# smdogroup/paropt

Hardware: AMD Instinct MI355X
Metric: IP iterations/sec (KKT solve+line search), n=50M vars m=32, 1/2/4/8 GPUs (higher is better)
Workload: dtype f64

## Files before the change

### paropt_amd/csrc/context.cpp

```cpp
#include <dlfcn.h>
#include <math.h>
#include <stdarg.h>
#include <execinfo.h>
#include <stdio.h>
#include <stdlib.h>
#include <string.h>
#include <time.h>

#include <algorithm>
#include <mutex>
#include <unordered_map>

#include "core.hpp"

namespace po {

static thread_local char g_err[1024] = "";
thread_local int g_last_code = 0;

void set_error(const char *fmt, ...) {
  va_list ap;
  va_start(ap, fmt);
  vsnprintf(g_err, sizeof(g_err), fmt, ap);
  va_end(ap);
  fprintf(stderr, "paropt_amd: %s\n", g_err);
}
const char *last_error() { return g_err; }

double host_now() {
  struct timespec t;
  clock_gettime(CLOCK_MONOTONIC, &t);
  return (double)t.tv_sec + 1e-9 * (double)t.tv_nsec;
}

struct SwitchDef {
  DbgSwitch id;
  const char *env;
  int dflt;
  bool presence;
};
static const SwitchDef kSwitches[] = {
    {SW_PERTURB_W, nullptr, 0, false},
    {SW_MPC_FUSE, "PAROPT_AMD_MPC_FUSE", 1, false},
    {SW_MPC_POLY, "PAROPT_AMD_MPC_POLY", 1, false},
    {SW_SPEC_DT, "PAROPT_AMD_SPEC_DT", 1, false},
    {SW_UNIFORM_BOUNDS, nullptr, 1, false},
    {SW_WGRAM_PRIO, "PAROPT_AMD_WGRAM_PRIO", 2, false},
    {SW_WGRAM_ABLATE, "PAROPT_AMD_WGRAM_ABLATE", 0, false},
    {SW_EXPLICIT_DOTS, "PAROPT_AMD_EXPLICIT_DOTS", 0, true},
    {SW_NO_RECOMPUTE, "PAROPT_AMD_NO_RECOMPUTE", 0, true},
    {SW_NO_RECOMPUTE_RHS, "PAROPT_AMD_NO_RECOMPUTE_RHS", 0, true},
    {SW_NO_FUSED_MERIT, "PAROPT_AMD_NO_FUSED_MERIT", 0, true},
    {SW_NO_LEAN_STEP, "PAROPT_AMD_NO_LEAN_STEP", 0, true},
    {SW_NO_RECOMPUTE_DT, "PAROPT_AMD_NO_RECOMPUTE_DT", 0, true},
    {SW_NO_FUSED_UPDATE, "PAROPT_AMD_NO_FUSED_UPDATE", 0, true},
    {SW_NO_CSR_GROUPS, "PAROPT_AMD_NO_CSR_GROUPS", 0, true},
    {SW_NO_FRONTS, "PAROPT_AMD_NO_FRONTS", 0, false},
    {SW_FORCE_RCCL, "PAROPT_AMD_FORCE_RCCL", 0, true},
    {SW_RCCL_ALLGATHER, "PAROPT_AMD_RCCL_ALLGATHER", 0, true},
    {SW_NO_DIRECT_RED, "PAROPT_AMD_NO_DIRECT_RED", 0, true},
    {SW_NO_FLAG_POLL, "PAROPT_AMD_NO_FLAG_POLL", 0, true},
    {SW_NO_BATCH, "PAROPT_AMD_NO_BATCH", 0, true},
    {SW_HOST_TRACE, "PAROPT_AMD_HOST_TRACE", 0, true},
    {SW_SYNC_TRACE, "PAROPT_AMD_SYNC_TRACE", 0, true},
    {SW_USER_TIMING, "PAROPT_AMD_USER_TIMING", 0, true},
    {SW_DUMP_LONG_SOLVES, "PAROPT_AMD_DUMP_LONG_SOLVES", -1, false},
};
static struct {
  int value = -1;
} g_dbg_switch[SW_COUNT];

int dbg_switch(DbgSwitch id) {
  if (g_dbg_switch[id].value >= 0) return g_dbg_switch[id].value;
  for (const SwitchDef &s : kSwitches) {
    if (s.id != id) continue;
    const char *e = s.env ? getenv(s.env) : nullptr;
    return e ? (s.presence ? 1 : atoi(e)) : s.dflt;
  }
  return 0;
}
void dbg_switch_set(int id, int value) {
  if (id >= 0 && id < SW_COUNT) g_dbg_switch[id].value = value;
}

int launch_reduce_final(Ctx *c, int nblocks, int nslots, int nsum, int nmin, int dst_off);
int launch_reduce_final_multi(Ctx *c, const Ctx::PendingRed *pend, int count);
int launch_red_publish(Ctx *c, const double *src, int count);
static int alloc_h_red(Ctx *c, size_t doubles) {
  if (c->h_red) (void)hipHostFree(c->h_red);
  c->h_red = nullptr;
  c->h_red_dev = nullptr;
  if (hipHostMalloc((void **)&c->h_red, sizeof(double) * doubles, hipHostMallocMapped | hipHostMallocCoherent) !=
      hipSuccess) {
    (void)hipGetLastError();
    c->h_red = nullptr;
    PO_HIP(hipHostMalloc((void **)&c->h_red, sizeof(double) * doubles, hipHostMallocDefault));
    c->h_red_coherent = 0;
  } else {
    c->h_red_coherent = 1;
  }
  if (dbg_switch(SW_NO_DIRECT_RED) ||
      hipHostGetDevicePointer((void **)&c->h_red_dev, c->h_red, 0) != hipSuccess) {
    (void)hipGetLastError();
    c->h_red_dev = nullptr;
  }
  if (c->h_flag && (!c->h_red_coherent || !c->h_red_dev)) {
    (void)hipHostFree(c->h_flag);
    c->h_flag = c->h_flag_dev = nullptr;
    if (c->d_ticket) (void)hipFree(c->d_ticket);
    c->d_ticket = nullptr;
  }
  if (c->h_red_dev && !c->h_flag && c->h_red_coherent && !dbg_switch(SW_NO_FLAG_POLL)) {
    if (hipHostMalloc((void **)&c->h_flag, 64, hipHostMallocMapped | hipHostMallocCoherent) == hipSuccess &&
        hipHostGetDevicePointer((void **)&c->h_flag_dev, c->h_flag, 0) == hipSuccess &&
        hipMalloc((void **)&c->d_ticket, sizeof(unsigned)) == hipSuccess &&
        hipMemset(c->d_ticket, 0, sizeof(unsigned)) == hipSuccess) {
      *c->h_flag = 0;
    } else {
      (void)hipGetLastError();
      if (c->h_flag) (void)hipHostFree(c->h_flag);
      if (c->d_ticket) (void)hipFree(c->d_ticket);
      c->h_flag = c->h_flag_dev = nullptr;
      c->d_ticket = nullptr;
    }
  }
  return PO_OK;
}


static int comm_self_test(Ctx *c);
static void free_overflow(Ctx *c, const double *keep);

struct Id128 {
  char b[PO_RCCL_ID_BYTES];
};
struct RcclApi {
  void *handle = nullptr;
  int (*GetUniqueId)(void *) = nullptr;
  int (*CommInitRank)(void **, int, Id128, int) = nullptr;
  int (*AllGather)(const void *, void *, size_t, int, void *, hipStream_t) = nullptr;
  int (*AllReduce)(const void *, void *, size_t, int, int, void *, hipStream_t) = nullptr;
  int (*CommDestroy)(void *) = nullptr;
  const char *(*GetErrorString)(int) = nullptr;
  int (*GetVersion)(int *) = nullptr;
  int version = 0;
};
static RcclApi g_rccl;

static int load_rccl() {
// ... 578 lines not shown
```

### paropt_amd/csrc/core.hpp

```cpp
#pragma once
#include <hip/hip_runtime.h>
#include <stdint.h>

#include <functional>
#include <string>
#include <vector>

#include "../../include/paropt_amd.h"

namespace po {

void set_error(const char *fmt, ...);
extern thread_local int g_last_code;

#define PO_HIP(expr)                                                                     \
  do {                                                                                   \
    hipError_t _e = (expr);                                                              \
    if (_e != hipSuccess) {                                                              \
      po::set_error("%s failed: %s (%s:%d)", #expr, hipGetErrorString(_e), __FILE__,     \
                    __LINE__);                                                           \
      return PO_ERR_HIP;                                                                 \
    }                                                                                    \
  } while (0)

// ... 75 lines not shown
};

struct Vec {
  Ctx *ctx;
  int64_t n;
  double *d;
  int ref;
  double *h;
  int h_live = 0;
};

struct PtrTable {
  const double *p[kMaxPanel];
};
struct CoefTable {
  double a[kMaxPanel];
};
int reduce_finish(Ctx *c, int nblocks, int nsum, int nmin, int nmax, double *host_out, bool now = false,
                  double *local_out = nullptr);
bool red_direct(const Ctx *c);
int batch_flush(Ctx *c, const double *keep_partials = nullptr, size_t keep_len = 0);
void batch_abort(Ctx *c);
template <class F>
inline void after_reduce(Ctx *c, F &&f) {
  if (c->batch_depth > 0 && !c->batch_pend.empty()) {
    c->batch_after.emplace_back(std::forward<F>(f));
  } else {
    f();
  }
}
struct BatchScope {
  Ctx *c;
  bool open;
  explicit BatchScope(Ctx *c_, bool on = true) : c(c_), open(on && c_->batch_enabled) {
    if (open) c->batch_depth++;
  }
  void begin() {
    if (!open && c->batch_enabled) {
      open = true;
      c->batch_depth++;
    }
  }
  int end() {
    if (!open) return PO_OK;
    open = false;
    c->batch_depth--;
    return batch_flush(c);
  }
  int end_nested() {
    if (!open) return PO_OK;
    open = false;
    c->batch_depth--;
    return c->batch_depth > 0 ? PO_OK : batch_flush(c);
  }
  template <class F>
  int end_then(F &&post) {
    if (open) {
      open = false;
      c->batch_depth--;
      if (c->batch_depth > 0) {
        after_reduce(c, std::forward<F>(post));
        return PO_OK;
      }
      PO_TRY(batch_flush(c));
    }
    post();
    return PO_OK;
  }
  ~BatchScope() {
    if (open) {
      c->batch_depth--;
      batch_abort(c);
    }
  }
  BatchScope(const BatchScope &) = delete;
  BatchScope &operator=(const BatchScope &) = delete;
};
enum DbgSwitch {
  SW_PERTURB_W = 11, SW_MPC_FUSE = 14, SW_MPC_POLY = 15, SW_SPEC_DT = 16, SW_UNIFORM_BOUNDS = 17,
  SW_WGRAM_PRIO = 18, SW_WGRAM_ABLATE = 19, SW_EXPLICIT_DOTS = 20, SW_NO_RECOMPUTE = 21, SW_NO_RECOMPUTE_RHS = 22,
  SW_NO_FUSED_MERIT = 23, SW_NO_LEAN_STEP = 24, SW_NO_RECOMPUTE_DT = 25, SW_NO_FUSED_UPDATE = 26,
  SW_NO_CSR_GROUPS = 27, SW_NO_FRONTS = 28, SW_FORCE_RCCL = 29, SW_RCCL_ALLGATHER = 30, SW_NO_DIRECT_RED = 31,
  SW_NO_FLAG_POLL = 32, SW_NO_BATCH = 33, SW_HOST_TRACE = 34, SW_SYNC_TRACE = 35, SW_USER_TIMING = 36,
  SW_DUMP_LONG_SOLVES = 37, SW_COUNT = 38
};
int dbg_switch(DbgSwitch id);
void dbg_switch_set(int id, int value);
double host_now();
inline double host_trace_begin(Ctx *c);
inline void host_trace_end(Ctx *c, double t0);
int ensure_partials(Ctx *c, size_t doubles);
bool ctx_alive(const Ctx *c, unsigned long long serial);
inline double host_trace_begin(Ctx *c) {
  if (!c->host_trace) return 0.0;
  const double t = host_now();
  if (!c->host_gap_open && c->host_t_launch_end > 0.0) {
    const double g = t - c->host_t_launch_end;
    if (g < 500e-6) {
      c->host_inter_s += g;
      c->host_inter_n++;
      if (g > 30e-6) {
        c->host_inter_n30++;
        c->host_inter_s30 += g;
      }
    }
  }
  if (c->host_gap_open) {
    const double g = t - c->host_t_sync;
    if (g < 500e-6) {
      c->host_gap_s += g;
      c->host_gap_n++;
      if (g > 20e-6) c->host_gap_n20++;
    } else {
      c->host_gap_long_s += g;
      c->host_gap_long_n++;
    }
    c->host_gap_open = false;
  }
  return t;
}
inline void host_trace_end(Ctx *c, double t0) {
  if (!c->host_trace) return;
  c->host_t_launch_end = host_now();
  c->host_launch_s += c->host_t_launch_end - t0;
  c->host_launch_n++;
}
inline void count_bytes(Ctx *c, double streams, int64_t n) {
  const double b = 8.0 * streams * (double)n;
  c->alg_bytes += b;
  if (c->in_user) c->alg_bytes_user += b;
}
constexpr int kBpcPanel = 2;
constexpr int kBpcStream = 4;
int grid_for(Ctx *c, int64_t n);
int grid_for(Ctx *c, int64_t n, int bpc);

struct GroupCol {
  const double *w = nullptr;
  double scale = 0.0;
  unsigned period = 1, nw = 0;
  long long nwcon = 0;
};

struct GroupCols2 {
  GroupCol g[2];
  double ca[2] = {0.0, 0.0}, cb[2] = {0.0, 0.0};
  int count = 0;
};

int k_fill(Ctx *c, double *y, int64_t n, double alpha);
int k_fill_hash(Ctx *c, double *y, int64_t n, uint64_t seed, uint64_t aid, int64_t offset,
                double scale, double shift);
int k_copy(Ctx *c, double *y, const double *x, int64_t n);
int k_sign(Ctx *c, double *y, const double *x, int64_t n);
int k_scale(Ctx *c, double *y, int64_t n, double alpha);
int k_axpy(Ctx *c, double *y, double alpha, const double *x, int64_t n);
int k_panel_axpy(Ctx *c, double *y, double a, const double *x, double b, const double *alpha,
                 const double *const *V, int nv, int64_t n, const GroupCol *ybase = nullptr);
int k_panel_axpy2(Ctx *c, double *y1, double a1, const double *x1, const double *c1, double *y2, double a2,
                  const double *x2, const double *c2, const double *const *V, int nv, int64_t n);
int k_panel_lincomb(Ctx *c, double *const *dst, double a, const double *const *X, double b,
                    const double *const *Y, int nv, int64_t n);
enum Red1 { RED_DOT = 0, RED_SUMSQ = 1, RED_ASUM = 2, RED_AMAX = 3 };
int k_reduce1(Ctx *c, int kind, const double *x, const double *y, int64_t n, double *out);
int k_mdot(Ctx *c, const double *x, const double *const *V, int nv, int64_t n, double *out);
int k_minmax(Ctx *c, const double *x, int64_t n, double out[2]);
int k_stream_launch(Ctx *c, int kind, double *x, double *y, int64_t n);
int k_mdot_launch(Ctx *c, const double *x, const double *const *V, int nv, int64_t n, int *nblocks);
struct GramGroups {
  int64_t nwcon = 0, start = 0;
  int nw = 0, skip = 0;
  double alpha = 1.0;
  int ncols = 0;
  double *const *U = nullptr;
};
int k_wgram(Ctx *c, const double *d, const double *const *V, int nv, int64_t n, double *W,
            const double *const *S = nullptr, double *const *Zout = nullptr, int kpend = 0,
            double b0 = 0.0, int preweighted_last = 0, bool may_defer = false,
            const GramGroups *groups = nullptr, bool *groups_done = nullptr);
int wgram_debug_stamps(double out[8]);
int k_xgram(Ctx *c, const double *const *U, const double *const *Z, int m, int64_t w, double *out,
            bool may_defer = false);
int k_wgram_launch(Ctx *c, const double *d, const double *const *V, int nv, int64_t n,
                   int *nblocks, int *nslots, const double *const *S = nullptr,
                   double *const *Zout = nullptr, int kpend = 0, double b0 = 0.0,
                   int preweighted_last = 0, const GramGroups *groups = nullptr, bool *groups_done = nullptr);

struct Bounds {
  const double *x, *lb, *ub, *zl, *zu;
  double max_bound;
  int use_lower, use_upper;
  int lb_uni = 0, ub_uni = 0;
  double lb_c = 0.0, ub_c = 0.0;
};
inline int uniform_bound_streams(const Bounds &b) { return (b.lb_uni ? 1 : 0) + (b.ub_uni ? 1 : 0); }
int k_kkt_res(Ctx *c, const Bounds &b, const double *g, const double *const *A, const double *z,
              int nc, double beta_mu, int64_t n, double *rx, double *out, double *yqn = nullptr,
              double beta_mu2 = -1.0, const GroupCol *gcol = nullptr, double gcoef = 0.0);
int k_kkt_res_update(Ctx *c, const Bounds &b, const double *g, const double *const *A, const double *z, int nc,
                     double beta_mu, int64_t n, double *rx, double *out, double *yqn, double *zl,
                     const double *pzl, double *zu, const double *pzu, double a, double eps, const double *va,
                     double az, double *acz, double az_acz,
                     const double *pxs = nullptr, const double *xold = nullptr, double beta_mu_step = 0.0,
                     double beta_mu2 = -1.0,
                     const GroupCol *gcol = nullptr, double gcoef = 0.0,
                     double *dinv_out = nullptr, double *t_out = nullptr, double spec_diag = 0.0,
                     double spec_beta_mu = 0.0);
int k_res_norms(Ctx *c, const Bounds &b, double beta_mu, int64_t n, double out[11]);
int k_dinv(Ctx *c, const Bounds &b, double diag, int64_t n, double *dinv,
           const double *hdiag = nullptr);
int k_d1s(Ctx *c, const Bounds &b, const double *bx, const double *dinv, double alpha, double beta_mu,
          int64_t n, double *t);
int k_solve2s(Ctx *c, const Bounds &b, const double *t, const double *dinv, const double *coef,
              const double *const *P, int nv, double alpha, double beta_mu, int full, double tau, int64_t n,
              double *px, double *pzl, double *pzu, double out[2]);
int k_d1(Ctx *c, const Bounds &b, const double *rx, const double *dinv, double beta_mu, int64_t n,
         double *t, const double *cl = nullptr, const double *cu = nullptr);
int k_dinv_d1(Ctx *c, const Bounds &b, double diag, const double *hdiag, const double *rx, double beta_mu,
              int64_t n, double *dinv, double *t, int raw = 0);
int k_corrector(Ctx *c, const Bounds &b, const double *px, const double *pzl, const double *pzu,
                int64_t n, double *cl, double *cu);
constexpr int kCorrDotsMax = 15;
int k_corr_d1_dots(Ctx *c, const Bounds &b, const double *px, const double *pzl, const double *pzu, const double *rx,
                   const double *dinv, double beta_mu, const double *const *V, int nv, int64_t n, double *t,
                   double *out);
int k_solve2c(Ctx *c, const Bounds &b, const double *t, const double *dinv, const double *alpha,
              const double *const *P, int nv, double beta_mu, double tau, int64_t n, double *px, double *pzl,
              double *pzu, double *va, int nca, const double *g, int want_logs, double out[12]);
int k_solve2(Ctx *c, const Bounds &b, const double *t, const double *dinv, const double *alpha,
             const double *const *P, int nv, double beta_mu, int refine, double tau, int64_t n,
             double *px, double *pzl, double *pzu, double out[2], const double *coef2 = nullptr,
             const double *rx = nullptr, double diag = 0.0, double *tout = nullptr,
             double *va = nullptr, int nca = 0, const double *cl = nullptr,
             const double *cu = nullptr);
int k_solve2_dots(Ctx *c, const Bounds &b, const double *t, const double *dinv, const double *alpha,
                  const double *coef2, const double *const *P, int nv, double beta_mu, double tau,
                  const double *rx, double diag, int64_t n, double *px, double *pzl, double *pzu,
                  double *tout, double *va, int nca, double *out, double *traw = nullptr,
                  int store_step = 1,
                  int ca0 = 0,
                  double dinv_diag = 0.0,
                  const GroupCols2 *gcols = nullptr);
int k_solve2r(Ctx *c, const Bounds &b, const double *t1, const double *t2, const double *dinv, const double *a1,
              const double *a2, const double *const *P, int nv, double beta_mu, double tau, int64_t n, double *px,
              double *pzl, double *pzu, double *va, int nca, double out[2], const double *ar = nullptr,
              const double *rx = nullptr, double diag = 0.0,
              int ca0 = 0,
              const double *g = nullptr, double *merit_out = nullptr,
              double dinv_diag = 0.0,
              const GroupCol *gcol = nullptr, double gc1 = 0.0, double gc2 = 0.0);
int k_form_pz(Ctx *c, const Bounds &b, const double *px, double beta_mu, int64_t n, double *pzl, double *pzu);
int k_update_mult_yqn(Ctx *c, double *zl, const double *pzl, double *zu, const double *pzu, double a,
                      double eps, int use_lower, int use_upper, const double *rx, const double *va,
                      double az, int64_t n, double *yqn, double *acz = nullptr);
int k_res_step(Ctx *c, const Bounds &b, const double *rx, const double *px, const double *pzl,
               const double *pzu, const double *dinv, const double *coef, const double *const *P,
               int nv, double diag, double beta_mu, int64_t n, double *tprime);
int k_step_check(Ctx *c, const Bounds &b, const double *rx, const double *px, const double *pzl, const double *pzu,
                 const double *coef, const double *const *P, int nv, double diag, double beta_mu, int64_t n,
                 double out[3]);
int k_comp_step(Ctx *c, const Bounds &b, const double *px, const double *pzl, const double *pzu,
                double ax, double az, int64_t n, double out[2]);
int k_comp_merit(Ctx *c, const Bounds &b, const double *px, const double *pzl, const double *pzu, double ax,
                 double az, const double *g, int64_t n, double out[9]);
int k_merit0(Ctx *c, const Bounds &b, const double *px, double sx, const double *g, int64_t n,
             double out[6]);
int k_trial(Ctx *c, const Bounds &b, const double *px, double a, double eps, int64_t n, double *xt,
            double out[2], double *sout = nullptr);
int k_update_mult(Ctx *c, double *zl, const double *pzl, double *zu, const double *pzu, double a,
                  double eps, int use_lower, int use_upper, int64_t n);
int k_affine_mult(Ctx *c, const Bounds &b, double *zl, const double *pzl, double *zu,
                  const double *pzu, double amin, int64_t n);
int k_check_bounds(Ctx *c, double *x, double *lb, double *ub, double *zl, double *zu,
                   double max_bound, double rel_bound, int both, int64_t n, int *flag, int uni[2] = nullptr,
                   double val[2] = nullptr);
int k_bounds_mode(Ctx *c, double *x, double *lb, double *ub, int mode, int64_t offset, int64_t n);
int k_clamp_count(Ctx *c, const double *x, const double *lb, const double *ub, const double *zl, const double *zu,
                  double eps, int64_t n, double out[4]);
// ... 24 lines not shown
```

### paropt_amd/csrc/ip.cpp

```cpp
#include "ip.hpp"

#include <math.h>
#include <stdio.h>
#include <stdlib.h>
#include <string.h>

#include <algorithm>
#include <chrono>

namespace po {

static const int LS_SUCCESS = 1, LS_FAILURE = 2, LS_MIN_STEP = 4, LS_MAX_ITERS = 8,
                 LS_NO_IMPROVEMENT = 16, LS_SHORT_STEP = 32;

InteriorPoint::InteriorPoint(Problem *p)
    : prob(p), ctx(p->ctx), n(p->nlocal), c(p->ncon), qn(nullptr), x(nullptr), zl(nullptr),
      zu(nullptr), lb(nullptr), ub(nullptr), g(nullptr), fobj(0.0), barrier_param(0.1),
      rho_penalty_search(0.0), niter(0), neval(0), ngeval(0),
      iter_cb(nullptr),
      iter_cb_user(nullptr), px(nullptr), pzl(nullptr), pzu(nullptr), Dinv(nullptr), rx(nullptr),
      tvec(nullptr), xt(nullptr), y_qn(nullptr), s_qn(nullptr), vA(nullptr), qn_created(false), qn_owned(true),
      comp_prod(0), comp_count(0), max_rx(0), max_rzl(0), max_rzu(0), sx(1.0), sz(1.0),
      corrector_active(false), norm_type(0), phase_t0(0) {
  qn_handle.qn = nullptr;
// ... 247 lines not shown
  (void)hipEventRecord(user_ev[2 * user_pending], ctx->stream);
}
void InteriorPoint::userEnd() {
  ctx->in_user = 0;
  if (!user_timing || !user_events_ready) return;
  (void)hipEventRecord(user_ev[2 * user_pending + 1], ctx->stream);
  user_pending++;
}
void InteriorPoint::userHarvest() {
  for (int i = 0; i < user_pending; i++) {
    float ms = 0.0f;
    if (hipEventSynchronize(user_ev[2 * i + 1]) == hipSuccess &&
        hipEventElapsedTime(&ms, user_ev[2 * i], user_ev[2 * i + 1]) == hipSuccess)
      user_seconds += 1e-3 * ms;
  }
  user_pending = 0;
}

int InteriorPoint::initAndCheckDesignAndBounds() {
  bounds_uni[0] = bounds_uni[1] = 0;
  int rc = prob->getVarsAndBounds(x, lb, ub);
  if (rc != 0) {
    set_error("getVarsAndBounds failed with code %d", rc);
    return PO_ERR_USER;
  }
  const double rel_bound = 0.001 * barrier_param;
  int flag = 0;
  PO_TRY(k_check_bounds(ctx, x->d, lb->d, ub->d, zl->d, zu->d, options.real("max_bound_value"),
                        rel_bound, use_lower && use_upper, n, &flag, bounds_uni, bounds_val));
  check_flag |= flag;
  if (ctx->rank == 0) {
    if (flag & 1) history += "ParOpt Warning: Variable bounds are inconsistent\n";
    if (flag & 2) history += "ParOpt Warning: Variables may be too close to lower bound\n";
    if (flag & 4) history += "ParOpt Warning: Variables may be too close to upper bound\n";
  }
  return PO_OK;
}

int InteriorPoint::clampCounts(double out[8]) {
  const double eps = options.real("design_precision");
  PO_TRY(k_clamp_count(ctx, x->d, lb->d, ub->d, use_lower ? zl->d : nullptr, use_upper ? zu->d : nullptr, eps, n,
                       out));
  for (int j = 4; j < 8; j++) out[j] = 0.0;
  for (int i = 0; i < c; i++) {
    if (vars.s[i] == eps) out[4] += 1.0;
    if (vars.t[i] == eps) out[5] += 1.0;
    if (vars.zs[i] == eps) out[6] += 1.0;
    if (vars.zt[i] == eps) out[7] += 1.0;
  }
  return PO_OK;
}

static int refreshLiveMirror(Vec *v) {
  if (!v || !v->h_live || !v->h || v->n <= 0) return PO_OK;
  PO_HIP(hipMemcpyAsync(v->h, v->d, sizeof(double) * (size_t)v->n, hipMemcpyDeviceToHost, v->ctx->stream));
  PO_HIP(hipStreamSynchronize(v->ctx->stream));
  return PO_OK;
}

int InteriorPoint::resetDesignAndBounds() {
  stateReplaced();
  bounds_uni[0] = bounds_uni[1] = 0;
  int rc = prob->getVarsAndBounds(x, lb, ub);
  if (rc != 0) return PO_ERR_USER;
  PO_TRY(refreshLiveMirror(x));
  PO_TRY(refreshLiveMirror(lb));
  return refreshLiveMirror(ub);
}

void InteriorPoint::resetQuasiNewtonHessian() {
  if (qn) qn->reset();
}

int InteriorPoint::initLeastSquaresMultipliers() {
  iterate_flags.acz_valid = false;
  const double mu0 = options.real("init_barrier_param");
  PO_TRY(k_fill(ctx, zl->d, n, mu0));
  PO_TRY(k_fill(ctx, zu->d, n, mu0));
  for (int i = 0; i < c; i++) vars.z[i] = vars.s[i] = vars.t[i] = vars.zs[i] = vars.zt[i] = mu0;
  PO_TRY(k_zero_inactive(ctx, lb->d, ub->d, zl->d, zu->d, options.real("max_bound_value"), n));
  if (has_w) return initLeastSquaresMultipliersW();
  if (c == 0) return PO_OK;
  const double small = 1e-4;
  PO_TRY(k_fill(ctx, Dinv->d, n, 1.0));
  int k = 0;
  std::vector<const double *> A = panel(false, &k);
  std::vector<double> G((size_t)c * c, 0.0);
  PO_TRY(k_wgram(ctx, Dinv->d, A.data(), c, n, G.data()));
  for (int i = 0; i < c; i++) G[(size_t)i * (c + 1)] += small;
  std::vector<int> piv(c);
  lu_factor(c, G.data(), c, piv.data());
  const double al[2] = {1.0, -1.0};
  const double *vv[2] = {zl->d, zu->d};
  PO_TRY(k_panel_axpy(ctx, tvec->d, -1.0, g->d, 0.0, al, vv, 2, n));
  std::vector<double> z(c, 0.0);
  PO_TRY(k_mdot(ctx, tvec->d, A.data(), c, n, z.data()));
  for (int i = 0; i < c; i++) z[i] = -z[i];
  lu_solve(c, G.data(), c, piv.data(), z.data());
  for (int i = 0; i < c; i++) {
    const double gam = 10.0 * std::max(gamma_s[i], gamma_t[i]);
    vars.z[i] = (z[i] < -gam || z[i] > gam) ? 0.0 : z[i];
  }
  return PO_OK;
}

int InteriorPoint::initAffineStepMultipliers() {
  const double amin = options.real("start_affine_multiplier_min");
  PO_TRY(initLeastSquaresMultipliers());
  PO_TRY(k_zero_inactive(ctx, lb->d, ub->d, zl->d, zu->d, options.real("max_bound_value"), n));
  PO_TRY(computeResidual(0.0, true));
  bool use_qn = !(options.integer("sequential_linear_method") ||
                  !options.integer("use_qn_gmres_precon") || options.integer("use_diag_hessian"));
  if (options.integer("use_diag_hessian")) PO_TRY(ensureHdiag());
  PO_TRY(setUpKKTSystem(use_qn));
  denseResidual(0.0, res);
  if (has_w) {
    PO_TRY(solveKKTW(res, 0.0, use_qn, false, 1.0, step));
    PO_TRY(k_w_affine(ctx, wv(), wp(), amin, nw));
  } else {
    PO_TRY(solveKKT(res, 0.0, use_qn, false, 1.0, step));
  }
  iterate_flags.acz_valid = false;
  for (int i = 0; i < c; i++) {
    vars.z[i] = vars.z[i] + step.z[i];
    vars.s[i] = std::max(amin, fabs(vars.s[i] + step.s[i]));
    vars.t[i] = std::max(amin, fabs(vars.t[i] + step.t[i]));
    vars.zs[i] = std::max(amin, fabs(vars.zs[i] + step.zs[i]));
    vars.zt[i] = std::max(amin, fabs(vars.zt[i] + step.zt[i]));
  }
  PO_TRY(k_affine_mult(ctx, bounds(), zl->d, pzl->d, zu->d, pzu->d, amin, n));
  double comp = 0.0;
  PO_TRY(getComplementarity(&comp));
  barrier_param = comp;
  return PO_OK;
}

void InteriorPoint::denseResidual(double mu, Dense &r) const {
  for (int i = 0; i < c; i++) {
    r.z[i] = -(cvals[i] - vars.s[i] + vars.t[i]);
    r.s[i] = -(gamma_s[i] - vars.zs[i] + vars.z[i]);
    r.t[i] = -(gamma_t[i] - vars.zt[i] - vars.z[i]);
    r.zs[i] = -(vars.s[i] * vars.zs[i] - mu);
    r.zt[i] = -(vars.t[i] * vars.zt[i] - mu);
  }
}

double InteriorPoint::nextMonotoneMu() const {
  const double abs_res_tol = options.real("abs_res_tol");
  const double mu_frac = options.real("monotone_barrier_fraction") * barrier_param;
  const double mu_pow = pow(barrier_param, options.real("monotone_barrier_power"));
  double new_mu = mu_frac;
  if (mu_pow < mu_frac) new_mu = mu_pow;
  if (new_mu < 0.1 * abs_res_tol) new_mu = 0.09999 * abs_res_tol;
  return new_mu;
}

int InteriorPoint::computeResidual(double mu, bool vectors, Vec *yqn_complete, const MultUpdate *upd) {
  const double beta_mu = options.real("rel_bound_barrier") * mu;
  double *out = res_out;
  const bool spec = vectors && spec_enabled && !has_w && mu == barrier_param;
  const double mu2 = spec ? nextMonotoneMu() : 0.0;
  const double beta_mu2 = spec ? options.real("rel_bound_barrier") * mu2 : -1.0;
  iterate_flags.spec_valid = false;
  scratch_flags.spec_dt_valid = false;
  BatchScope wbatch(ctx, has_w && prob->reductionsBatchable());
  if (has_w) PO_TRY(computeResidualW(mu));
  bool acz_mode = false, acz_rebuilt = false;
  if (vectors) {
    std::vector<const double *> A;
    std::vector<double> zc;
    if (prob->linear_constraints && iterate_flags.ac_valid && c > 0) {
      if (!acz) acz = vec_new(ctx, n);
      if (!acz) return PO_ERR_HIP;
      if (!iterate_flags.acz_valid || acz_age >= kAczRefresh) {
        std::vector<const double *> Ap;
        for (Vec *a : Ac) Ap.push_back(a->d);
        PO_TRY(k_panel_axpy(ctx, acz->d, 0.0, nullptr, 0.0, vars.z.data(), Ap.data(), c, n));
        iterate_flags.acz_valid = true;
        acz_age = 0;
        acz_rebuilt = true;
      }
      acz_age++;
      A.push_back(acz->d);
      zc.push_back(1.0);
      acz_mode = true;
    } else {
      for (Vec *a : Ac) A.push_back(a->d);
      zc = vars.z;
    }
    GroupCol gcol;
    const bool have_gcol = has_w && !acz_mode && prob->sparseTransposeColumn(1.0, x, wvar[0], &gcol);
    if (has_w && !have_gcol) {
      if (prob->setSparseJacobianTranspose(1.0, x, wvar[0], tvec) != 0) return PO_ERR_USER;
      A.push_back(tvec->d);
      zc.push_back(1.0);
    }
    if (upd) {
      const double az_acz = (acz_mode && upd->acz_follow && !acz_rebuilt) ? upd->az : 0.0;
      const bool spec_dt = spec_dt_want && !has_w && !options.integer("use_diag_hessian") &&
                           dbg_switch(SW_SPEC_DT) != 0;
      const double sdiag = spec_dt ? options.real("qn_sigma") + ((qn && !options.integer("sequential_linear_method"))
                                                                    ? qn->diag() : 0.0) : 0.0;
      const double sbmu = spec_dt ? options.real("rel_bound_barrier") * spec_dt_mu : 0.0;
      PO_TRY(k_kkt_res_update(ctx, bounds(), g->d, A.data(), zc.data(), acz_mode ? 0 : (int)A.size(), beta_mu, n,
                              rx->d, out, yqn_complete ? yqn_complete->d : nullptr, zl->d, pzl->d, zu->d, pzu->d,
                              upd->a, upd->eps, (yqn_complete || az_acz != 0.0) ? vA->d : nullptr,
                              upd->az, acz_mode ? acz->d : nullptr, az_acz, step_flags.pz_stored ? nullptr : px->d,
                              step_flags.pz_stored ? nullptr : xt->d, step_beta_mu, beta_mu2,
                              have_gcol ? &gcol : nullptr, 1.0,
                              spec_dt ? Dinv->d : nullptr, spec_dt ? tvec->d : nullptr, sdiag, sbmu));
      if (spec_dt) {
        scratch_flags.spec_dt_valid = true;
        spec_dt_diag = sdiag;
        spec_dt_bmu = sbmu;
      }
    } else {
      PO_TRY(k_kkt_res(ctx, bounds(), g->d, A.data(), zc.data(), (int)A.size(), beta_mu, n, rx->d, out,
                       yqn_complete ? yqn_complete->d : nullptr, beta_mu2, have_gcol ? &gcol : nullptr, 1.0));
    }
  } else {
    PO_TRY(k_res_norms(ctx, bounds(), beta_mu, n, out));
  }
  after_reduce(ctx, [this, vectors, spec, mu2] {
    const double *o = res_out;
    if (vectors) {
      l1_rx = o[2];
      l2_rx = o[5];
      max_rx = o[8];
    }
    if (spec) {
      spec_mu = mu2;
      spec_max[0] = o[11];
      spec_max[1] = o[12];
      iterate_flags.spec_valid = true;
    }
    comp_prod = o[0];
    comp_count = o[1];
    l1_rzl = o[3];
    l1_rzu = o[4];
    l2_rzl = o[6];
    l2_rzu = o[7];
    max_rzl = o[9];
    max_rzu = o[10];
  });
  return wbatch.end_nested();
}

void InteriorPoint::resNorms(const Dense &r, double *max_prime, double *max_dual,
                             double *max_infeas, double *res_norm) const {
  double mp = 0.0, md = 0.0, mi = 0.0;
  if (norm_type == 0) {
    mp = max_rx;
    for (int i = 0; i < c; i++) {
      mp = std::max(mp, std::max(fabs(r.s[i]), fabs(r.t[i])));
      mi = std::max(mi, fabs(r.z[i]));
      md = std::max(md, std::max(fabs(r.zs[i]), fabs(r.zt[i])));
    }
    if (use_lower) md = std::max(md, max_rzl);
    if (use_upper) md = std::max(md, max_rzu);
    if (has_w) {
      mi = std::max(mi, w_maxs[0]);
      md = std::max(md, std::max(std::max(w_maxs[1], w_maxs[2]), std::max(w_maxs[3], w_maxs[4])));
    }
  } else if (norm_type == 1) {
    mp = l1_rx;
    for (int i = 0; i < c; i++) {
      mp += fabs(r.s[i]);
      mp += fabs(r.t[i]);
      mi += fabs(r.z[i]);
      md += fabs(r.zs[i]);
      md += fabs(r.zt[i]);
    }
    if (use_lower) md += l1_rzl;
    if (use_upper) md += l1_rzu;
    if (has_w) {
      mi += w_sums[1];
      md += w_sums[3] + w_sums[4] + w_sums[5] + w_sums[6];
    }
  } else {
    double prime = 0.0, infeas = 0.0, dual = 0.0;
    for (int i = 0; i < c; i++) {
      prime += r.s[i] * r.s[i] + r.t[i] * r.t[i];
      infeas += r.z[i] * r.z[i];
      dual += r.zs[i] * r.zs[i] + r.zt[i] * r.zt[i];
    }
    mp = l2_rx + prime;
    mi = infeas;
    md = dual;
    if (use_lower) md += l2_rzl;
    if (use_upper) md += l2_rzu;
    if (has_w) {
      mi += w_sums[2];
      md += w_sums[3] * w_sums[3] + w_sums[4] * w_sums[4] + w_sums[5] * w_sums[5] +
            w_sums[6] * w_sums[6];
    }
    mp = sqrt(mp);
    mi = sqrt(mi);
    md = sqrt(md);
  }
  *max_prime = mp;
  *max_dual = md;
  *max_infeas = mi;
  *res_norm = std::max(mp, std::max(md, mi));
}

double InteriorPoint::compFromSums(double prod, double count, const Dense &v,
                                   double wprod) const {
  prod = prod / options.real("rel_bound_barrier");
  if (has_w) {
    prod += wprod;
    count += 2.0 * nw_global;
  }
  for (int i = 0; i < c; i++) {
    prod += v.s[i] * v.zs[i] + v.t[i] * v.zt[i];
    count += 2.0;
  }
  return count != 0.0 ? prod / count : 0.0;
}

int InteriorPoint::getComplementarity(double *comp) {
  double out[11];
  PO_TRY(k_res_norms(ctx, bounds(), 0.0, n, out));
  double wprod = 0.0;
  if (has_w) PO_TRY(wCompStep(0.0, 0.0, &wprod));
  *comp = compFromSums(out[0], out[1], vars, wprod);
  return PO_OK;
}

int InteriorPoint::setUpKKTSystem(bool use_qn, bool diag_only, const double *rhs_mu) {
  if (qn) PO_TRY(refreshQuasiNewton());
  step_flags.ptpx_valid = false;
  scratch_flags.t0_valid = false;
  const double sigma = options.real("qn_sigma");
  const bool use_hdiag = options.integer("use_diag_hessian") && hdiag;
  const double b0 = (!use_hdiag && qn && (use_qn || diag_only)) ? qn->diag() : 0.0;
  const bool fuse_t = rhs_mu && !has_w && c + (qn && use_qn && !diag_only ? qn->size() : 0) > 0;
  scratch_flags.t_is_plain_dinv_d1 = false;
  const bool raw_d1_w = has_w && rhs_mu && !corrector_active;
  const bool have_spec_dt = scratch_flags.spec_dt_valid;
  scratch_flags.spec_dt_valid = false;
  if (fuse_t && have_spec_dt && !use_hdiag && spec_dt_diag == b0 + sigma &&
      spec_dt_bmu == options.real("rel_bound_barrier") * (*rhs_mu)) {
    scratch_flags.t_is_plain_dinv_d1 = true;
    t0_diag = b0 + sigma;
  } else if (fuse_t) {
    PO_TRY(k_dinv_d1(ctx, bounds(), b0 + sigma, use_hdiag ? hdiag->d : nullptr, rx->d,
                     options.real("rel_bound_barrier") * (*rhs_mu), n, Dinv->d, tvec->d));
    scratch_flags.t_is_plain_dinv_d1 = !use_hdiag;
    t0_diag = b0 + sigma;
  } else if (raw_d1_w) {
    PO_TRY(k_dinv_d1(ctx, bounds(), b0 + sigma, use_hdiag ? hdiag->d : nullptr, rx->d,
                     options.real("rel_bound_barrier") * (*rhs_mu), n, Dinv->d, d1v->d, 1));
  } else {
    PO_TRY(k_dinv(ctx, bounds(), b0 + sigma, n, Dinv->d, use_hdiag ? hdiag->d : nullptr));
  }
  int k = 0;
  std::vector<const double *> Yp, Sp;
  std::vector<double *> Zo;
  double b0z = 0.0;
  const bool fuse_z = qn && use_qn && !diag_only && !has_w && qn->pendingZ(&Yp, &Sp, &Zo, &b0z) &&
                      !Yp.empty() && Yp.size() <= 12 && c + (int)Yp.size() + (fuse_t ? 1 : 0) <= kWgramMaxVecs;
  if (fuse_z) {
    k = (int)Yp.size();
    const int m2 = c + k, mt = m2 + (fuse_t ? 1 : 0);
    std::vector<const double *> P2(Yp);
    for (Vec *a : Ac) P2.push_back(a->d);
    if (fuse_t) P2.push_back(tvec->d);
    std::vector<double> W2((size_t)mt * mt, 0.0);
    PO_TRY(k_wgram(ctx, Dinv->d, P2.data(), mt, n, W2.data(), Sp.data(), Zo.data(), k, b0z, fuse_t ? 1 : 0));
    qn->pendingZDone();
    kkt.W.assign((size_t)m2 * m2, 0.0);
    auto perm = [&](int i) { return i < c ? k + i : i - c; };
    for (int j = 0; j < m2; j++)
      for (int i = 0; i < m2; i++) kkt.W[i + (size_t)m2 * j] = W2[perm(i) + (size_t)mt * perm(j)];
    if (fuse_t) {
      t0dots.assign(m2, 0.0);
      for (int i = 0; i < m2; i++) t0dots[i] = W2[perm(i) + (size_t)mt * m2];
    }
  }
  std::vector<const double *> P;
  if (!fuse_z) {
    P = panel(use_qn && !diag_only, &k);
  } else if (has_w) {
    int k2 = 0;
    P = panel(use_qn && !diag_only, &k2);
  }
  const int m = c + k;
  kkt.k = k;
  bool fuse_tw = false;
  BatchScope wbatch(ctx, has_w && prob->reductionsBatchable());
  bool t0_ready = fuse_z && fuse_t;
  if (has_w) {
    PO_TRY(prob->sparseFactorFromSlacks(x, Dinv, wv(), Cw));
    fuse_tw = rhs_mu && m > 0 && m + 1 <= kWgramMaxVecs && !corrector_active;
    if (fuse_tw) {
      PO_TRY(computeResidualW(*rhs_mu, true, true));
      if (!raw_d1_w)
        PO_TRY(k_d1(ctx, bounds(), rx->d, nullptr, options.real("rel_bound_barrier") * (*rhs_mu), n, d1v->d));
      PO_TRY(applyK0(d1v->d, wd2->d, tvec, wyw));
    }
  }
  GramGroups gram_groups;
  std::vector<double *> Ugs;
  const GramGroups *ggp = nullptr;
  bool panel_done = false;
  if (has_w && !fuse_z && m > 0 && prob->sparseGramGroups(x, &gram_groups)) {
    PO_TRY(panelImageVectors(m, Ugs));
    gram_groups.ncols = m;
    gram_groups.U = Ugs.data();
    ggp = &gram_groups;
  }
  if (!fuse_z) {
    kkt.W.assign((size_t)m * m, 0.0);
    if (m > 0 && (fuse_t || fuse_tw) && m + 1 <= kWgramMaxVecs) {
      std::vector<const double *> Pt(P);
      Pt.push_back(tvec->d);
      const int mt = m + 1;
      Wt_buf.assign((size_t)mt * mt, 0.0);
      PO_TRY(k_wgram(ctx, Dinv->d, Pt.data(), mt, n, Wt_buf.data(), nullptr, nullptr, 0, 0.0, 1, wbatch.open, ggp,
                     &panel_done));
      t0dots.assign(m, 0.0);
      after_reduce(ctx, [this, m, mt] {
        for (int j = 0; j < m; j++)
          for (int i = 0; i < m; i++) kkt.W[i + (size_t)m * j] = Wt_buf[i + (size_t)mt * j];
        for (int i = 0; i < m; i++) t0dots[i] = Wt_buf[i + (size_t)mt * m];
      });
      t0_ready = true;
    } else {
      if (m > 0)
        PO_TRY(k_wgram(ctx, Dinv->d, P.data(), m, n, kkt.W.data(), nullptr, nullptr, 0, 0.0, 0, wbatch.open, ggp,
                       &panel_done));
      t0dots.clear();
    }
  }
  if ((fuse_t || fuse_tw) && m > 0 && t0_ready && (int)t0dots.size() == m) {
    scratch_flags.t0_valid = true;
    t0_mu = *rhs_mu;
  }
  if (has_w) PO_TRY(sparseGramCorrection(P, m, fuse_tw ? d1v : tvec, wbatch.open, panel_done));
  PO_TRY(wbatch.end());
  if (m > 1 && debug_keep_schur && dbg_switch(SW_PERTURB_W) != 0) {
    kkt.W[1] *= 1.0 + 1e-9;
    kkt.W[m] = kkt.W[1];
  }
  const double *d0 = nullptr, *M = nullptr;
  if (k > 0) {
    double b0_;
    qn->getCompactMat(&b0_, &d0, &M, nullptr);
  }
  kkt.factor(vars, d0, M, debug_keep_schur ? &Gmat0 : nullptr, debug_keep_schur ? &Ce0 : nullptr);
  if (k == 0) Ce0.clear();
  return PO_OK;
}

int InteriorPoint::solveKKT(const Dense &b, double mu, bool use_qn, bool refine_pass, double tau,
                            Dense &out, bool fuse_residual) {
  const double beta_mu = options.real("rel_bound_barrier") * mu;
  const int k = (qn && use_qn) ? qn->size() : 0;
  PO_TRY(kkt.checkWidth(k));
  const int m = c + k;
  std::vector<const double *> P;
  bool have_panel = false;
  auto need_panel = [&]() {
    if (!have_panel) {
      int k2 = 0;
      P = panel(use_qn, &k2);
      have_panel = true;
    }
  };
  const bool corr = corrector_active && !refine_pass;
  const bool corr_fused = corr && corrector_fused && m >= 1 && m <= kCorrDotsMax;
  const double *cl = (corr && !corr_fused) ? s_qn->d : nullptr;
  const double *cu = (corr && !corr_fused) ? y_qn->d : nullptr;
  if (corr && corrector_fused && !corr_fused) {
    set_error("internal: fused corrector solve with a panel of %d columns", m);
    return PO_ERR_ARG;
  }
  const bool have_t0 = !refine_pass && scratch_flags.t0_valid && t0_mu == mu && !corr && (int)t0dots.size() == m;
  std::vector<double> dots(m > 0 ? m : 1, 0.0);
  if (corr_fused) {
    need_panel();
    PO_TRY(k_corr_d1_dots(ctx, bounds(), px->d, pzl->d, pzu->d, rx->d, Dinv->d, beta_mu, P.data(), m, n, tvec->d,
                          dots.data()));
  } else {
    if (!refine_pass && !have_t0) PO_TRY(k_d1(ctx, bounds(), rx->d, Dinv->d, beta_mu, n, tvec->d, cl, cu));
    if (have_t0) {
      for (int i = 0; i < m; i++) dots[i] = t0dots[i];
    } else if (refine_pass && step_flags.tdots_valid && (int)tdots.size() == m) {
      dots = tdots;
    } else if (m > 0) {
      need_panel();
      PO_TRY(k_mdot(ctx, tvec->d, P.data(), m, n, dots.data()));
    }
  }
  if (!refine_pass) scratch_flags.first_t_recomputable = have_t0 && scratch_flags.t_is_plain_dinv_d1;
  if (!refine_pass) scratch_flags.t0_valid = false;
  const bool deferred = refine_pass && step_flags.step_deferred;
  stepWillChange();
  Bordered::Sol sol;
  kkt.solve(1.0, b, vars, dots.data(), &sol);
  const std::vector<double> &alpha = sol.coef;
  kkt.panelDots(dots.data(), sol, refine_pass, &ptpx);
  step_flags.ptpx_valid = true;
  const bool seq_lin = options.integer("sequential_linear_method");
  const int kq = (qn && !seq_lin) ? qn->size() : 0;
  const bool fuse = fuse_residual && !refine_pass && forms.analytic_panel_dots && kq == k &&
                    !options.integer("use_diag_hessian") && !inexact_newton_step && m <= kMaxPanel;
  step_flags.vA_valid = true;
  std::vector<double> coef(m > 0 ? m : 1, 0.0);
  double diag = options.real("qn_sigma");
  if (fuse) PO_TRY(residualCoefs(qn && !seq_lin ? RES_QN : RES_SIGMA, alpha.data(), ptpx.data() + c, k, coef, &diag));
  const bool first_fused = fuse && m > 0 && !corr;
  need_panel();
  if (first_fused) {
    std::vector<double> out(m + 2, 0.0);
    const bool defer = forms.recompute_first_step;
    double *tp_out = !defer ? tvec->d : (forms.recompute_rhs ? nullptr : xt->d);
    const bool redo_dt1 = forms.recompute_dt && defer && forms.recompute_rhs && scratch_flags.first_t_recomputable;
    const double *t_in = redo_dt1 ? nullptr : tvec->d;
    PO_TRY(k_solve2_dots(ctx, bounds(), t_in, Dinv->d, alpha.data(), coef.data(), P.data(), m, beta_mu, tau, rx->d,
                         diag, n, px->d, pzl->d, pzu->d, tp_out, vA->d, c, out.data(), nullptr, defer ? 0 : 1, 0,
                         t0_diag));
    tdots.assign(out.begin(), out.begin() + m);
    step_flags.tdots_valid = true;
    step_mins[0] = out[m];
    step_mins[1] = out[m + 1];
    step_flags.step_deferred = defer;
    if (defer) {
      alpha_first = alpha;
      coef_first = coef;
      diag_first = diag;
    }
  } else if (deferred) {
    const bool take_merit = forms.fuse_merit && forms.recompute_rhs && !corr;
    const double *gm = take_merit ? g->d : nullptr;
    double *mo = take_merit ? fused_merit : nullptr;
    const bool lean = forms.lean_step && lean_step_allowed && take_merit && iterate_flags.iterate_logs_valid;
    double *pzl_out = lean ? nullptr : pzl->d, *pzu_out = lean ? nullptr : pzu->d;
    const bool redo_dt = forms.recompute_dt && forms.recompute_rhs && scratch_flags.first_t_recomputable;
    const double *t1p = redo_dt ? nullptr : tvec->d;
    if (lean) {
      step_flags.pz_stored = false;
      step_beta_mu = beta_mu;
    }
    PO_TRY(k_solve2r(ctx, bounds(), t1p, forms.recompute_rhs ? nullptr : xt->d, Dinv->d, alpha_first.data(),
                     alpha.data(), P.data(), m, beta_mu, tau, n, px->d, pzl_out, pzu_out, vA->d, c, step_mins,
                     coef_first.data(), rx->d, diag_first, 0, gm, mo, t0_diag));
    if (take_merit) {
      after_reduce(ctx, [this] {
        step_mins[0] = fused_merit[7];
        step_mins[1] = fused_merit[8];
        step_flags.fused_merit_valid = true;
      });
    }
  } else if (corr_fused) {
    const bool want_logs = !iterate_flags.iterate_logs_valid;
    PO_TRY(k_solve2c(ctx, bounds(), tvec->d, Dinv->d, alpha.data(), P.data(), m, beta_mu, tau, n, px->d, pzl->d,
                     pzu->d, vA->d, c, g->d, want_logs ? 1 : 0, corr_out));
    after_reduce(ctx, [this, want_logs] {
      for (int i = 0; i < 7; i++) fused_merit[i] = corr_out[i];
      fused_merit[7] = step_mins[0] = corr_out[9];
      fused_merit[8] = step_mins[1] = corr_out[10];
      fused_merit[9] = corr_out[11];
      if (want_logs) {
        iterate_logs[0] = corr_out[7];
        iterate_logs[1] = corr_out[8];
        iterate_flags.iterate_logs_valid = true;
      }
      step_flags.fused_merit_valid = true;
    });
  } else {
    PO_TRY(k_solve2(ctx, bounds(), tvec->d, Dinv->d, alpha.data(), P.data(), m, beta_mu,
                    refine_pass ? 1 : 0, tau, n, px->d, pzl->d, pzu->d, step_mins,
                    fuse ? coef.data() : nullptr, rx->d, diag, tvec->d, vA->d, c, cl, cu));
  }
  step_flags.residual_fused = fuse;
  kkt.backSubstitute(1.0, b, vars, sol, true, out);
  return PO_OK;
}

int InteriorPoint::computeKKTStepWithRefinement(double mu, bool use_qn, double tau) {
  const int nref = options.integer("iterative_refinement_steps");
  const double beta_mu = options.real("rel_bound_barrier") * mu;
  const bool with_qn = qn && !options.integer("sequential_linear_method");
  const int mq = c + (with_qn ? qn->size() : 0);
  const bool diag_hess = options.integer("use_diag_hessian") && (!has_w || hdiag);
  const ResTerm term = (!has_w && inexact_newton_step) ? RES_HVEC
                       : diag_hess                     ? RES_HDIAG
                       : with_qn                       ? RES_QN
                                                       : RES_SIGMA;
  if (has_w && !(scratch_flags.t0_valid && t0_mu == mu)) PO_TRY(computeResidualW(mu));
  denseResidual(mu, res);
  PO_TRY(has_w ? solveKKTW(res, mu, use_qn, false, tau, step, nref > 0)
               : solveKKT(res, mu, use_qn, false, tau, step, nref > 0));
  for (int it = 0; it < nref; it++) {
    LazyPanel Pq{this, with_qn};
    if (has_w) Pq.get();
    std::vector<double> dots;
    PO_TRY(stepPanelDots(Pq, dots));
    std::vector<double> coef(mq + 2, 0.0);
    double diag = 0.0;
    PO_TRY(residualCoefs(term, step.z.data(), dots.data() + c, mq - c, coef, &diag));
    int mres = mq;
    if (term == RES_HVEC || term == RES_HDIAG) {
      Pq.get().push_back(xt->d);
      mres++;
    }
    if (!(it == 0 && step_flags.residual_fused)) {
      if (has_w) {
        if (prob->setSparseJacobianTranspose(1.0, x, wstepv[0], tvec) != 0) return PO_ERR_USER;
        Pq.get().push_back(tvec->d);
        coef[mres++] = 1.0;
      }
      PO_TRY(k_res_step(ctx, bounds(), rx->d, px->d, pzl->d, pzu->d, has_w ? nullptr : Dinv->d, coef.data(),
                        Pq.get().data(), mres, diag, beta_mu, n, has_w ? d1v->d : tvec->d));
    }
    if (has_w) {
      PO_TRY(computeResidualW(mu, false));
      if (prob->addSparseJacobian(-1.0, x, px, wresv[0]) != 0) return PO_ERR_USER;
      PO_TRY(k_w_res_step(ctx, wv(), wp(), wr(), nw, wd2->d));
      scratch_flags.wd2_ready = true;
    }
    Dense r2;
    r2.resize(c);
    denseResidual(mu, r2);
    denseResStep(vars, step, dots.data(), r2);
    PO_TRY(has_w ? solveKKTW(r2, mu, use_qn, true, tau, refine) : solveKKT(r2, mu, use_qn, true, tau, refine));
    for (int i = 0; i < c; i++) {
      step.z[i] += refine.z[i];
      step.s[i] += refine.s[i];
      step.t[i] += refine.t[i];
      step.zs[i] += refine.zs[i];
      step.zt[i] += refine.zt[i];
    }
  }
  sx = sz = 1.0;
  return PO_OK;
}

int InteriorPoint::checkKKTStep(int iteration, double mu) {
  const double beta_mu = options.real("rel_bound_barrier") * mu;
  if (!step_flags.pz_stored) {
    PO_TRY(k_form_pz(ctx, bounds(), px->d, step_beta_mu, n, pzl->d, pzu->d));
    step_flags.pz_stored = true;
  }
  const bool seq_lin = options.integer("sequential_linear_method");
  int kq = 0;
  std::vector<const double *> Pq = panel(qn && !seq_lin, &kq);
  const int mq = c + kq;
  std::vector<double> dots(mq > 0 ? mq : 1, 0.0), coef(mq > 0 ? mq : 1, 0.0);
  if (mq > 0) PO_TRY(k_mdot(ctx, px->d, Pq.data(), mq, n, dots.data()));
  double diag = 0.0;
  const bool with_qn = qn && !seq_lin && !options.integer("use_diag_hessian");
  PO_TRY(residualCoefs(with_qn ? RES_QN : RES_SIGMA, step.z.data(), dots.data() + c, kq, coef, &diag));
  if (has_w) {
    if (prob->setSparseJacobianTranspose(1.0, x, wstepv[0], xt) != 0) return PO_ERR_USER;
    Pq.push_back(xt->d);
    coef.push_back(1.0);
  }
  double mx[3];
  PO_TRY(computeResidual(mu, true));
  PO_TRY(k_step_check(ctx, bounds(), rx->d, px->d, pzl->d, pzu->d, coef.data(), Pq.data(), (int)Pq.size(), diag,
                      beta_mu, n, mx));
  Dense r;
  r.resize(c);
  denseResidual(mu, r);
  denseResStep(vars, step, dots.data(), r);
  double mz = 0.0, ms = 0.0, mt = 0.0, mzs = 0.0, mzt = 0.0;
  for (int i = 0; i < c; i++) {
    mz = std::max(mz, fabs(r.z[i]));
    ms = std::max(ms, fabs(r.s[i]));
    mt = std::max(mt, fabs(r.t[i]));
    mzs = std::max(mzs, fabs(r.zs[i]));
    mzt = std::max(mzt, fabs(r.zt[i]));
  }
  if (ctx->rank == 0) {
    char line[640];
    snprintf(line, sizeof(line),
             "\nResidual step check for iteration %d:\n"
             "max |stationarity (x block)|:             %10.4e\n"
             "max |dense constraints (z block)|:        %10.4e\n"
             "max |slack duals (s block)|:              %10.4e\n"
             "max |slack duals (t block)|:              %10.4e\n"
             "max |slack complementarity (zs block)|:   %10.4e\n"
             "max |slack complementarity (zt block)|:   %10.4e\n"
             "max |lower-bound complementarity (zl)|:   %10.4e\n"
             "max |upper-bound complementarity (zu)|:   %10.4e\n",
             iteration, mx[0], mz, ms, mt, mzs, mzt, mx[1], mx[2]);
    history += line;
  }
  return PO_OK;
}

int InteriorPoint::checkGradients(double dh, std::string *report) {
  scratchLent();
  return prob->checkGradients(dh, x, options.integer("use_hvec_product"), xt, tvec, report);
}

int InteriorPoint::checkMeritFuncGradient(Vec *xpt, double dh, double out[2]) {
  if (xpt) PO_TRY(k_copy(ctx, x->d, xpt->d, n));
  iterateReplaced();
  if (prob->evalObjCon(x, &fobj, cvals.data()) != 0) {
    fprintf(stderr, "ParOpt: Function and constraint evaluation failed\n");
    return PO_ERR_USER;
  }
  neval++;
  if (prob->evalObjConGradient(x, g, Ac.data()) != 0) {
    fprintf(stderr, "ParOpt: Gradient evaluation failed\n");
    return PO_ERR_USER;
  }
  ngeval++;
  iterate_flags.ac_valid = true;
  if (xpt) {
    double g2 = 0.0;
    PO_TRY(k_reduce1(ctx, RED_SUMSQ, g->d, nullptr, n, &g2));
    PO_TRY(k_panel_axpy(ctx, px->d, g2 > 0.0 ? -1.0 / sqrt(g2) : 0.0, g->d, 0.0, nullptr, nullptr, 0, n));
    for (int i = 0; i < c; i++) {
      step.s[i] = -0.259 * (1 + (i % 3));
      step.t[i] = -0.349 * (4 - (i % 2));
    }
    if (has_w && nw > 0) {
      std::vector<double> hs((size_t)nw), ht((size_t)nw);
      for (int64_t i = 0; i < nw; i++) {
        hs[i] = -0.419 * (1 + (i % 5));
        ht[i] = -0.7513 * (1 + (i % 19));
      }
      PO_HIP(hipMemcpyAsync(wstepv[1]->d, hs.data(), sizeof(double) * (size_t)nw, hipMemcpyHostToDevice, ctx->stream));
      PO_HIP(hipMemcpyAsync(wstepv[2]->d, ht.data(), sizeof(double) * (size_t)nw, hipMemcpyHostToDevice, ctx->stream));
      PO_HIP(hipStreamSynchronize(ctx->stream));
    }
  }
  sx = sz = 1.0;
  stepWillChange();
  double m0 = 0.0, dm0 = 0.0;
  PO_TRY(evalMeritInitDeriv(1.0, &m0, &dm0));
  const double eps = 0.0;
  double sums[2], wsums[5];
  std::vector<double> rs(c), rt(c), cs(cvals);
  for (int i = 0; i < c; i++) {
    rs[i] = vars.s[i] + dh * step.s[i];
    rt[i] = vars.t[i] + dh * step.t[i];
  }
  {
    PO_TRY(k_trial(ctx, bounds(), px->d, dh, eps, n, xt->d, sums));
  }
  double ftemp = 0.0;
  if (prob->evalObjCon(xt, &ftemp, cs.data()) != 0) {
    fprintf(stderr, "ParOpt: Function and constraint evaluation failed\n");
    return PO_ERR_USER;
  }
  neval++;
  if (has_w) {
    if (prob->evalSparseCon(xt, wtmp) != 0) return PO_ERR_USER;
    PO_TRY(k_w_trial(ctx, wv(), wp(), dh, eps, gsw->d, gtw->d, wtmp->d, nw, wsums));
  }
  const double m1 = evalMeritFromSums(ftemp, cs.data(), rs.data(), rt.data(), sums[0], sums[1], has_w ? wsums : nullptr);
  const double fd = (m1 - m0) / dh;
  if (ctx->rank == 0) {
    fprintf(stdout, "Merit function test\n");
    fprintf(stdout, "dm FD: %15.8e  Actual: %15.8e  Err: %8.2e  Rel err: %8.2e\n", fd, dm0, fabs(fd - dm0),
            fabs((fd - dm0) / fd));
    fflush(stdout);
  }
  if (out) {
    out[0] = fd;
    out[1] = dm0;
  }
  return PO_OK;
}

int InteriorPoint::debugKKTStep(double mu) {
  PO_TRY(createQuasiNewton());
  PO_TRY(computeResidual(mu, true));
  PO_TRY(setUpKKTSystem(true));
  denseResidual(mu, res);
  if (has_w) {
    PO_TRY(solveKKTW(res, mu, true, false, 0.95, step));
  } else {
    PO_TRY(solveKKT(res, mu, true, false, 0.95, step));
  }
  sx = sz = 1.0;
  return PO_OK;
}

int InteriorPoint::debugSetState(const double *z, const double *s, const double *t, const double *zs,
                                 const double *zt, double mu) {
  PO_TRY(createQuasiNewton());
  for (int i = 0; i < c; i++) {
    vars.z[i] = z[i];
    vars.s[i] = s[i];
    vars.t[i] = t[i];
    vars.zs[i] = zs[i];
    vars.zt[i] = zt[i];
  }
  barrier_param = mu;
  {
    const std::string nt = options.str("norm_type");
    norm_type = nt == "infinity" ? 0 : (nt == "l1" ? 1 : 2);
  }
  stateReplaced();
  spec_enabled = false;
  corrector_active = false;
  inexact_newton_step = false;
  if (prob->evalObjCon(x, &fobj, cvals.data()) != 0) return PO_ERR_USER;
  if (prob->evalObjConGradient(x, g, Ac.data()) != 0) return PO_ERR_USER;
  iterate_flags.ac_valid = true;
  return PO_OK;
}

int InteriorPoint::debugKKT(double mu, int mode, double tau) {
  struct KeepSchur {
    bool &f;
    explicit KeepSchur(bool &f_) : f(f_) { f = true; }
    ~KeepSchur() { f = false; }
  } keep(debug_keep_schur);
  if (mode == 0) {
    PO_TRY(debugKKTStep(mu));
  } else if (mode == 2) {
    PO_TRY(createQuasiNewton());
    const bool use_qn = !options.integer("sequential_linear_method");
    barrier_param = mu;
    PO_TRY(computeResidual(mu, true));
    const double comp = compFromSums(comp_prod, comp_count, vars, w_sums[0]);
    const double rhs_mu = 0.0;
    PO_TRY(setUpKKTSystem(use_qn, false, &rhs_mu));
    double tau_new = tau;
    PO_TRY(mehrotraStep(use_qn, comp, true, options.real("min_fraction_to_boundary"), options.real("abs_res_tol"),
                        &tau_new));
    (void)tau_new;
    PO_TRY(batch_flush(ctx));
  } else {
    PO_TRY(createQuasiNewton());
    PO_TRY(computeResidual(mu, true));
    PO_TRY(setUpKKTSystem(true, false, &mu));
    lean_step_allowed = false;
    PO_TRY(computeKKTStepWithRefinement(mu, true, tau));
    PO_TRY(batch_flush(ctx));
  }
  denseResidual(mu, res);
  resNorms(res, &debug_norms[0], &debug_norms[1], &debug_norms[2], &debug_norms[3]);
  return PO_OK;
}

int InteriorPoint::mehrotraStep(bool use_qn, double comp, bool corrector, double min_frac, double abs_res_tol,
                                double *tau_out) {
  PO_TRY(computeKKTStepWithRefinement(0.0, use_qn, 1.0));
  double max_x = std::min(1.0, step_mins[0]), max_z = std::min(1.0, step_mins[1]);
  for (int i = 0; i < c; i++) {
    if (step.s[i] < 0.0) max_x = std::min(max_x, -vars.s[i] / step.s[i]);
    if (step.t[i] < 0.0) max_x = std::min(max_x, -vars.t[i] / step.t[i]);
    if (step.zs[i] < 0.0) max_z = std::min(max_z, -vars.zs[i] / step.zs[i]);
    if (step.zt[i] < 0.0) max_z = std::min(max_z, -vars.zt[i] / step.zt[i]);
  }
  double cs[2];
  if (step_flags.fused_merit_valid && !has_w && dbg_switch(SW_MPC_POLY) != 0) {
    cs[0] = comp_prod + max_x * fused_merit[0] + max_z * fused_merit[1] + max_x * max_z * fused_merit[2];
    cs[1] = comp_count;
  } else {
    PO_TRY(k_comp_step(ctx, bounds(), px->d, pzl->d, pzu->d, max_x, max_z, n, cs));
  }
  double prod = cs[0] / options.real("rel_bound_barrier"), count = cs[1];
  if (has_w) {
    double wprod = 0.0;
    PO_TRY(wCompStep(max_x, max_z, &wprod));
    prod += wprod;
    count += 2.0 * nw_global;
  }
  for (int i = 0; i < c; i++) {
    prod += ((vars.s[i] + max_x * step.s[i]) * (vars.zs[i] + max_z * step.zs[i]) +
             (vars.t[i] + max_x * step.t[i]) * (vars.zt[i] + max_z * step.zt[i]));
    count += 2.0;
  }
  const double comp_affine = count != 0.0 ? prod / count : 0.0;
  const double s1 = comp_affine / comp;
  double sigma = s1 * s1 * s1;
  if (sigma < 0.01) sigma = 0.01;
  barrier_param = sigma * comp;
  if (barrier_param < 0.09999 * abs_res_tol) barrier_param = 0.09999 * abs_res_tol;
  double tau = min_frac;
  if (1.0 - barrier_param >= tau) tau = 1.0 - barrier_param;
  *tau_out = tau;
  if (corrector) {
    corrector_fused = !has_w && c + kkt.k >= 1 && c + kkt.k <= kCorrDotsMax &&
                      dbg_switch(SW_MPC_FUSE) != 0;
    if (!corrector_fused) PO_TRY(k_corrector(ctx, bounds(), px->d, pzl->d, pzu->d, n, s_qn->d, y_qn->d));
    denseResidual(barrier_param, res);
    for (int i = 0; i < c; i++) {
      res.zs[i] -= step.s[i] * step.zs[i];
      res.zt[i] -= step.t[i] * step.zt[i];
    }
    if (has_w) {
      PO_TRY(computeResidualW(barrier_param));
      PO_TRY(k_w_corrector(ctx, wp(), wr(), nw));
    }
    corrector_active = true;
    int rcs = has_w ? solveKKTW(res, barrier_param, use_qn, false, tau, step)
                    : solveKKT(res, barrier_param, use_qn, false, tau, step);
    corrector_active = false;
    corrector_fused = false;
    PO_TRY(rcs);
    sx = sz = 1.0;
  } else {
    PO_TRY(computeKKTStepWithRefinement(barrier_param, use_qn, tau));
  }
  return PO_OK;
}

int InteriorPoint::scaleKKTStep(double tau, double comp, double *alpha_x, double *alpha_z, int *ceq,
// ... 743 lines not shown
                 "nobj", "ngrd", "nhvc", "alpha", "alphx", "alphz", "fobj", "|opt|", "|infes|",
                 "|dual|", "mu", "comp", "dmerit", "rho");
        history += line;
      }
      if (k == 0) {
        snprintf(line, sizeof(line),
                 "%4d %4d %4d %4d %7s %7s %7s %12.5e %7.1e %7.1e %7.1e %7.1e %7.1e %8s %7s %s\n", k,
                 neval, ngeval, nhvec, "--", "--", "--", fobj, max_prime, max_infeas, max_dual,
                 barrier_param, comp, "--", "--", info);
      } else {
        snprintf(line, sizeof(line),
                 "%4d %4d %4d %4d %7.1e %7.1e %7.1e %12.5e %7.1e %7.1e %7.1e %7.1e %7.1e %8.1e %7.1e %s\n",
                 k, neval, ngeval, nhvec, alpha_prev, alpha_xprev, alpha_zprev, fobj, max_prime,
                 max_infeas, max_dual, barrier_param, comp, dm0_prev, rho_penalty_search, info);
      }
      history += line;
    }

    int converged = 0;
    if (k > 0 && (barrier_param <= 0.1 * abs_res_tol) &&
        (res_norm < abs_res_tol || rel_function_test || (line_search_test >= 2))) {
      if (ctx->rank == 0) {
        if (rel_function_test) {
          history += "\nParOpt: Successfully converged on relative function test\n";
        } else if (line_search_test >= 2) {
          history +=
              "\nParOpt Warning: Current design point could not be improved. No barrier function "
              "decrease in previous two iterations\n";
        } else {
          history += "\nParOpt: Successfully converged to requested tolerance\n";
        }
      }
      converged = 1;
    }
    if (converged) {
      flushHistory();
      return 0;
    }

    const bool mehrotra = (barrier_strategy == B_MEHROTRA || barrier_strategy == B_MPC);
    spec_dt_mu = mehrotra ? 0.0 : barrier_param;
    double tau = min_frac;
    if (1.0 - barrier_param >= tau) tau = 1.0 - barrier_param;

    int gmres_iters = 0;
    inexact_newton_step = false;
    if (use_hvec_product) {
      const double gmres_rtol =
          res_norm_prev == 0.0 ? 1e300
                               : options.real("eisenstat_walker_gamma") *
                                     pow(res_norm / res_norm_prev, options.real("eisenstat_walker_alpha"));
      const double nk = options.real("nk_switch_tol");
      if (max_prime < nk && max_dual < nk && max_infeas < nk && gmres_rtol < options.real("max_gmres_rtol")) {
        const bool precon_qn = !(seq_lin || !options.integer("use_qn_gmres_precon"));
        PO_TRY(setUpKKTSystem(precon_qn));
        PO_TRY(computeKKTGMRESStep(gmres_rtol, options.real("gmres_atol"), precon_qn, tau, &gmres_iters));
        phaseEnd("gmres_step");
        if (gmres_iters > 0) inexact_newton_step = true;
      }
    }
    fobj_prev = fobj;
    res_norm_prev = res_norm;
    int seq_linear_step = 0, diagonal_quasi_newton_step = 0;
    bool use_qn = !seq_lin;
    if (inexact_newton_step) {
    } else if (!seq_lin && line_search_failed && !use_qnu) {
      use_qn = false;
      seq_linear_step = 1;
      if (qn && qn->diag() > 0.0) {
        seq_linear_step = 0;
        diagonal_quasi_newton_step = 1;
      }
    } else if (use_diag_hessian && !seq_lin) {
      use_qn = false;
      if (prob->evalHessianDiag(x, vars.z.data(), has_w ? wvar[0] : nullptr, hdiag) != 0) {
        fprintf(stderr, "ParOpt: Hessian diagonal evaluation failed\n");
        return PO_ERR_USER;
      }
    }

    if (inexact_newton_step) {
    } else {
    const double rhs_mu = mehrotra ? 0.0 : barrier_param;
    PO_TRY(setUpKKTSystem(use_qn, diagonal_quasi_newton_step != 0, &rhs_mu));
    phaseEnd("setup_kkt");
    if (!mehrotra) {
      lean_step_allowed = qn && use_qnu && use_qn && !diagonal_quasi_newton_step && forms.analytic_panel_dots &&
                          forms.fuse_mult_update && !use_hvec_product && !use_diag_hessian && !seq_lin;
      const int step_rc = computeKKTStepWithRefinement(barrier_param, use_qn, tau);
      lean_step_allowed = false;
      PO_TRY(step_rc);
    } else {
      PO_TRY(mehrotraStep(use_qn, comp, barrier_strategy == B_MPC, min_frac, abs_res_tol, &tau));
    }
    }
    phaseEnd("kkt_step");
    if (step_verification_frequency > 0 && (k % step_verification_frequency) == 0 && !inexact_newton_step) {
      if (barrier_strategy == B_MPC && ctx->rank == 0)
        history += "Note: the step check is inconsistent with the predictor-corrector step (corrector terms)\n";
      PO_TRY(checkKKTStep(k, barrier_param));
    }

    double alpha_x = 1.0, alpha_z = 1.0;
    int ceq_step = 0;
    PO_TRY(scaleKKTStep(tau, comp, &alpha_x, &alpha_z, &ceq_step, inexact_newton_step));
    phaseEnd("scale_step");

    double alpha = 1.0;
    int line_fail = LS_FAILURE;
    int update_type = 0;
    int line_search_skipped = 0;
    no_merit_function_improvement = 0;

    if (use_line_search) {
      double m0 = 0.0, dm0 = 0.0;
      PO_TRY(evalMeritInitDeriv(alpha_x, &m0, &dm0));
      phaseEnd("merit_deriv");
      dm0_prev = dm0;
      if (dm0 >= 0.0 && dm0 <= fprec) {
        line_search_skipped = 1;
        PO_TRY(computeStepAndUpdate(alpha, 1, 1, &update_type));
        phaseEnd("step_update");
        if ((fobj_prev + fprec <= fobj) && (fobj + fprec <= fobj_prev)) line_fail = LS_NO_IMPROVEMENT;
      } else {
        if (dm0 >= 0.0) {
          if (qn) {
            qn_hessian_reset = 1;
            qn->reset();
          }
          diagonal_quasi_newton_step = 1;
          PO_TRY(computeResidual(barrier_param, true));
          denseResidual(barrier_param, res);
          resNorms(res, &max_prime, &max_dual, &max_infeas, &res_norm);
          PO_TRY(setUpKKTSystem(true, false, &barrier_param));
          PO_TRY(computeKKTStepWithRefinement(barrier_param, true, tau));
          PO_TRY(scaleKKTStep(tau, comp, &alpha_x, &alpha_z, &ceq_step));
          PO_TRY(evalMeritInitDeriv(alpha_x, &m0, &dm0));
          dm0_prev = dm0;
          phaseEnd("qn_reset_step");
        }
        if (dm0 >= 0.0) {
          line_fail = LS_FAILURE;
        } else {
          double px_norm = 0.0;
          if (step_flags.merit_cache_valid) {
            px_norm = merit_cache[6];
          } else if (step_flags.px_amax_valid) {
            px_norm = px_amax_w;
          } else {
            PO_TRY(k_reduce1(ctx, RED_AMAX, px->d, nullptr, n, &px_norm));
          }
          px_norm *= fabs(sx);
          double alpha_min = 1.0;
          if (px_norm != 0.0) alpha_min = fprec / px_norm;
          if (alpha_min > 0.5) alpha_min = 0.5;
          PO_TRY(lineSearch(alpha_min, &alpha, m0, dm0, &line_fail));
          phaseEnd("line_search");
          if (px_norm < design_precision) line_fail |= LS_SHORT_STEP;
          if (!(line_fail & LS_FAILURE)) {
            PO_TRY(computeStepAndUpdate(alpha, 0, 1, &update_type));
            phaseEnd("step_update");
          }
        }
      }
    } else {
      double m0 = 0.0, dm0 = 0.0;
      PO_TRY(evalMeritInitDeriv(alpha_x, &m0, &dm0));
// ... 231 lines not shown
```

### paropt_amd/csrc/ip.hpp

```cpp
#pragma once
#include <stdlib.h>
#include <map>
#include <string>
#include <vector>

#include "bordered.hpp"
#include "problem.hpp"
#include "qn.hpp"

namespace po {

class Options {
 public:
  enum Type { STR = 1, BOOL = 2, INT = 3, FLOAT = 4, ENUM = 5 };
  struct Entry {
    Type type;
    std::string s;
    int i = 0, ilo = 0, ihi = 0;
    double f = 0, flo = 0, fhi = 0;
    std::vector<std::string> choices;
  };
  Options();
  void addTrustRegionDefaults();
  void addMMADefaults();
  int set(const char *name, const char *value);
  int set(const char *name, int value);
  int set(const char *name, double value);
  const char *str(const char *name) const;
  int integer(const char *name) const;
  double real(const char *name) const;
  bool has(const char *name) const { return e.count(name) > 0; }
  int visit(const Options *skip, po_option_visitor fn, void *user) const;
  void adoptExtras(const Options &src, const Options &base);

 private:
  std::map<std::string, Entry> e;
};

class InteriorPoint {
 public:
  InteriorPoint(Problem *prob);
  ~InteriorPoint();
  int allocate();
  const std::vector<int> &gPivots() const { return kkt.gpiv; }
  Vec *lowerBounds() { return lb; }
  Vec *upperBounds() { return ub; }
  void clearUniformBounds() { bounds_uni[0] = bounds_uni[1] = 0; }
  int checkFlag() const { return check_flag; }
  int clampCounts(double out[8]);
  int checkKKTStep(int iteration, double mu);

  Options options;
  int optimize(const char *checkpoint);
  void getOptimizedPoint(Vec **x, const double **z, Vec **zl, Vec **zu);
  void getOptimizedSlacks(const double **s, const double **t, const double **zs, const double **zt);
  void getOptimizedSparse(Vec *v[5]);
  void getIterationCounters(int *niter_, int *neval_, int *ngeval_);
  double getBarrierParameter() const { return barrier_param; }
  int getComplementarity(double *comp);
  void setPenaltyGamma(double gamma);
  void setPenaltyGammaArray(const double *gamma);
  int resetDesignAndBounds();
  void resetQuasiNewtonHessian();
  int setQuasiNewton(CompactQuasiNewton *qn_);
  int resetProblemInstance(Problem *p);
  int writeSolutionFile(const char *filename);
  int readSolutionFile(const char *filename);
  int debugKKTStep(double mu);
  int debugSetState(const double *z, const double *s, const double *t, const double *zs, const double *zt, double mu);
  int debugKKT(double mu, int mode, double tau);
  std::vector<double> Gmat0, Ce0;
  bool debug_keep_schur = false;
  double debug_norms[4] = {0, 0, 0, 0};
  const std::vector<double> &gramMatrix() const { return kkt.W; }
  const std::vector<int> &cPivots() const { return kkt.cpiv; }
  const double *stepMins() const { return step_mins; }
  Vec *dinvVec() { return Dinv; }
  Vec *rxVec() { return rx; }
  void flushHistory();
  int checkGradients(double dh, std::string *report);
  int checkMeritFuncGradient(Vec *xpt, double dh, double out[2]);
  int setHvecFiniteDifference(int mode, int central, double rel_step);
  void getHvecFiniteDifferenceCount(int *products, int *evaluations) const;
  double hvecFiniteDifferenceStep() const { return hvec_fd_h; }
  int evalHvec(const double *z, Vec *zw, Vec *p, Vec *hvec);

  Problem *prob;
  Ctx *ctx;
  int64_t n;
  int c;
  CompactQuasiNewton *qn;
  po_qn_s qn_handle;

  Vec *x, *zl, *zu, *lb, *ub, *g;
  std::vector<Vec *> Ac;
  Dense vars, res, step, refine;
  double fobj, barrier_param, rho_penalty_search;
  std::vector<double> cvals;
  int niter, neval, ngeval, nhvec;

  po_ip_iteration_fn iter_cb;
  void *iter_cb_user;
  std::string history;
  std::vector<std::string> phase_names;
  std::vector<double> phase_seconds;
  std::string phase_names_joined;
  bool user_timing = dbg_switch(SW_USER_TIMING) != 0;

  Vec *px, *pzl, *pzu;

  int64_t nw;
  bool has_w;
  double nw_global;
  Vec *wvar[5], *wresv[5], *wstepv[5];

 private:
  Vec *Dinv, *rx, *tvec, *xt, *y_qn, *s_qn;
  Vec *vA;
  std::vector<double> gamma_s, gamma_t;
  int use_lower, use_upper;
  bool qn_created;
  bool qn_owned;

  Bordered kkt;

  struct StepFlags {
    bool ptpx_valid = false;
    bool tdots_valid = false;
    bool merit_cache_valid = false;
    bool fused_merit_valid = false;
    bool px_amax_valid = false;
    bool w_comp_valid = false;
    bool w_merit_cache_valid = false;
    bool vA_valid = false;
    bool residual_fused = false;
    bool pz_stored = true;
    bool step_deferred = false;
    bool px_first_only = false;
  } step_flags;
  struct ScratchFlags {
    bool spec_dt_valid = false;
    bool t0_valid = false;
    bool t_is_plain_dinv_d1 = false;
    bool first_t_recomputable = false;
    bool wd2_ready = false;
    bool panel_valid = false;
  } scratch_flags;
  struct IterateFlags {
    bool ac_valid = false;
    bool acz_valid = false;
    bool cwx_valid = false;
    bool trial_cw_valid = false;
    bool iterate_logs_valid = false;
    bool trial_logs_valid = false;
    bool residual_cached = false;
    bool spec_valid = false;
    bool s_qn_from_trial = false;
  } iterate_flags;
  void stepWillChange() { step_flags = {}; }
  void scratchLent() { scratch_flags = {}; }
  void iterateReplaced() { iterate_flags = {}; }
  void stateReplaced() {
    stepWillChange();
    scratchLent();
    iterateReplaced();
  }
  double comp_prod, comp_count, max_rx, max_rzl, max_rzu;
  double l1_rx = 0, l1_rzl = 0, l1_rzu = 0, l2_rx = 0, l2_rzl = 0, l2_rzu = 0;
  double sx, sz;
  double step_mins[2];
  std::vector<double> ptpx;
  bool corrector_active;
  bool corrector_fused = false;
  bool spec_dt_want = false;
  double spec_dt_diag = 0.0, spec_dt_bmu = 0.0, spec_dt_mu = 0.0;
  double corr_out[12] = {0};
  int norm_type;
  std::vector<double> tdots;

  Vec *hdiag;
  std::vector<Vec *> gmresW;
  bool inexact_newton_step;
  double merit_cache[7];
  double px_amax_w = 0.0;
  std::vector<double> Wt_buf, W2_buf;
  double fused_merit[10] = {0};
  double t0_diag = 0.0;
  bool lean_step_allowed = false;
  double step_beta_mu = 0.0;
  double trial_logs[2] = {0, 0}, iterate_logs[2] = {0, 0};
  int gatherCounts(int64_t mine, std::vector<int64_t> *all);
  int solutionFileOffsets(int64_t *nvars_total, int64_t *var_off, int64_t *nw_total, int64_t *w_off);
  int ensureHdiag();
  int solveKKTAlpha(const double *bx, double alpha, const Dense &b, double mu, bool use_qn, bool full,
                    double tau, Dense &out);
  int evalObjBarrierDeriv(const Dense &p, double *pmerit);
  int solveKKTAlphaW(const double *bx, double alpha, const Dense &b, double mu, bool use_qn, bool full,
                     double tau, Dense &out);
  Vec *wscalev[5];
  double w_merit_last[10];
  int computeKKTGMRESStep(double rtol, double atol, bool use_qn, double tau, int *gmres_iters);

  int hvec_mode = PO_HVEC_EXACT, hvec_central = 0;
  double hvec_rel = 0.0;
  bool hvec_fd_active = false;
  int hvec_fd_products = 0, hvec_fd_evals = 0;
  double hvec_fd_h = 0.0;
  Vec *hvec_xp = nullptr;
  std::vector<Vec *> hvec_work[2];
  Vec *hvec_csr_data = nullptr, *hvec_csr_cw = nullptr;
  int64_t hvec_csr_nnz = 0;
  int hvecProduct(const double *z, Vec *zw, Vec *p, Vec *hvec);
  int hvecFiniteDifference(const double *z, Vec *zw, Vec *p, Vec *hvec);
  int hvecScratch(int sides, int nc);
  int hvecEvalAt(double a, Vec *p, int side, bool with_jac);

  Vec *gsw, *gtw, *Cw, *wd2, *wyw, *wtmp, *wtmp2;
  Vec *cwx = nullptr;
  int sparseConAtIterate(const double **cw);
  Vec *d1v;
  std::vector<Vec *> Uw;
  bool panel_plain = false;
  std::vector<Vec *> Yw;
  bool panel_solved = false;
  std::vector<const double *> correctionPanel(int m) const;
  double w_sums[7], w_maxs[5];
  double res_out[13] = {0}, wres_out[12] = {0};
  bool spec_enabled = false;
  double spec_mu = 0.0, spec_max[2] = {0.0, 0.0};
  double nextMonotoneMu() const;
  WVars wv() const;
  WVars wr() const;
  WVars wp() const;
  int allocateW();
  int applyK0(const double *bx, const double *bw, Vec *yx, Vec *yw);
  int computeResidualW(double mu, bool norms = true, bool with_d2 = false);
  int sparseGramCorrection(const std::vector<const double *> &P, int m, Vec *work = nullptr, bool may_defer = false,
                           bool panel_done = false);
  int panelImageVectors(int m, std::vector<double *> &U);
  int solveKKTW(const Dense &b, double mu, bool use_qn, bool refine_pass, double tau, Dense &out,
                bool fuse_residual = false);
  int initLeastSquaresMultipliersW();
  int wCompStep(double ax, double az, double *prod);

  Bounds bounds() const;
  std::vector<const double *> panel(bool use_qn, int *k) const;
  struct LazyPanel {
    const InteriorPoint *ip;
    bool use_qn;
    bool asked = false;
    std::vector<const double *> P;
    std::vector<const double *> &get();
  };
  int stepPanelDots(LazyPanel &P, std::vector<double> &dots);
  std::vector<double> compactInverse(const double *ztp, int kq) const;
  enum ResTerm { RES_SIGMA, RES_QN, RES_HVEC, RES_HDIAG };
  int residualCoefs(ResTerm term, const double *z, const double *ztpx, int kq, std::vector<double> &coef,
                    double *diag);

  int createQuasiNewton();
  int refreshQuasiNewton();
  int initAndCheckDesignAndBounds();
  int initLeastSquaresMultipliers();
  int initAffineStepMultipliers();
  void denseResidual(double mu, Dense &r) const;
  struct MultUpdate {
    double a = 0.0, az = 0.0, eps = 0.0;
    bool acz_follow = false;
  };
  int computeResidual(double mu, bool vectors, Vec *yqn_complete = nullptr, const MultUpdate *upd = nullptr);
  void resNorms(const Dense &r, double *max_prime, double *max_dual, double *max_infeas,
                double *res_norm) const;
  double compFromSums(double prod, double count, const Dense &v, double wprod = 0.0) const;
  int setUpKKTSystem(bool use_qn, bool diag_only = false, const double *rhs_mu = nullptr);
  int solveKKT(const Dense &b, double mu, bool use_qn, bool refine_pass, double tau, Dense &out,
               bool fuse_residual = false);
  int computeKKTStepWithRefinement(double mu, bool use_qn, double tau);
  int mehrotraStep(bool use_qn, double comp, bool corrector, double min_frac, double abs_res_tol, double *tau_out);
  int scaleKKTStep(double tau, double comp, double *alpha_x, double *alpha_z, int *ceq,
                   bool inexact = false);
  int evalMeritInitDeriv(double max_x, double *merit, double *pmerit);
  double evalMeritFromSums(double fk, const double *ck, const double *sk, const double *tk,
                           double pos, double neg, const double *wsums = nullptr) const;
  int lineSearch(double alpha_min, double *alpha, double m0, double dm0, int *fail);
  int computeStepAndUpdate(double alpha, int eval_obj_con, int perform_qn_update, int *update_type);
  void phaseBegin();
  void phaseEnd(const char *name);
  double phase_t0;
  static const int kUserRing = 16;
  hipEvent_t user_ev[2 * kUserRing];
  int user_pending = 0;
  bool user_events_ready = false;
  double user_seconds = 0.0;
  void userBegin();
  void userEnd();
  void userHarvest();
  struct Forms {
    bool analytic_panel_dots;
    bool fuse_merit;
    bool lean_step;
    bool recompute_dt;
    bool recompute_first_step;
    bool recompute_rhs;
    bool fuse_mult_update;
  };
  static Forms readForms();
  const Forms forms = readForms();
  int check_flag = 0;
  int bounds_uni[2] = {0, 0};
  double bounds_val[2] = {0.0, 0.0};
  static const int kAczRefresh = 16;
  Vec *acz = nullptr;
  int acz_age = 0;
  double w_step_out[5] = {0, 0, 0, 0, 0}, w_comp_poly[3] = {0, 0, 0}, w_merit_cache[10] = {0};
  double s_qn_a = 0.0;
  std::vector<double> alpha_first, coef_first;
  double diag_first = 0.0;
  double t0_mu = 0.0;
  std::vector<double> t0dots;
};

}

struct po_ip_s {
  po::InteriorPoint *ip;
};
```

### paropt_amd/csrc/ip_gmres.cpp

```cpp
#include <math.h>

#include <algorithm>

#include "ip.hpp"

namespace po {

int InteriorPoint::ensureHdiag() {
  if (hdiag) return PO_OK;
  hdiag = vec_new(ctx, n);
  return hdiag ? PO_OK : PO_ERR_HIP;
}

int InteriorPoint::solveKKTAlpha(const double *bx, double alpha, const Dense &b, double mu, bool use_qn,
                                 bool full, double tau, Dense &out) {
  const double beta_mu = options.real("rel_bound_barrier") * mu;
  int k = 0;
  std::vector<const double *> P = panel(use_qn, &k);
  PO_TRY(kkt.checkWidth(k));
  const int m = c + k;
  PO_TRY(k_d1s(ctx, bounds(), bx, Dinv->d, alpha, beta_mu, n, tvec->d));
  std::vector<double> dots(m > 0 ? m : 1, 0.0);
  if (m > 0) PO_TRY(k_mdot(ctx, tvec->d, P.data(), m, n, dots.data()));
  Bordered::Sol sol;
  kkt.solve(alpha, b, vars, dots.data(), &sol);
  const std::vector<double> &coef = sol.coef;
  stepWillChange();
  kkt.panelDots(dots.data(), sol, false, &ptpx);
  step_flags.ptpx_valid = true;
  PO_TRY(k_solve2s(ctx, bounds(), tvec->d, Dinv->d, coef.data(), P.data(), m, alpha, beta_mu, full ? 1 : 0, tau,
                   n, px->d, pzl->d, pzu->d, step_mins));
  kkt.backSubstitute(alpha, b, vars, sol, full, out);
  return PO_OK;
}

int InteriorPoint::solveKKTAlphaW(const double *bx, double alpha, const Dense &b, double mu, bool use_qn,
                                  bool full, double tau, Dense &out) {
  const double beta_mu = options.real("rel_bound_barrier") * mu;
  int k = 0;
  std::vector<const double *> P = panel(use_qn, &k);
  PO_TRY(kkt.checkWidth(k));
  const int m = c + k;
  WVars ws{wscalev[0]->d, wscalev[1]->d, wscalev[2]->d, wscalev[3]->d, wscalev[4]->d};
  PO_TRY(k_d1s(ctx, bounds(), bx, nullptr, alpha, beta_mu, n, d1v->d));
  PO_TRY(k_w_scale5(ctx, ws, wr(), alpha, nw));
  PO_TRY(k_w_d2(ctx, wv(), ws, nw, wd2->d));
  PO_TRY(applyK0(d1v->d, wd2->d, tvec, wyw));
  std::vector<double> dots(m > 0 ? m : 1, 0.0);
  if (m > 0) PO_TRY(k_mdot(ctx, tvec->d, P.data(), m, n, dots.data()));
  Bordered::Sol sol;
  kkt.solve(alpha, b, vars, dots.data(), &sol);
  const std::vector<double> &coef = sol.coef;
  stepWillChange();
  kkt.panelDots(dots.data(), sol, false, &ptpx);
  step_flags.ptpx_valid = true;
  double mins_w[2] = {1.0, 1.0};
  if (!full && k > 0) {
    if (c > 0) {
      PO_TRY(k_panel_axpy(ctx, xt->d, 1.0, d1v->d, 0.0, sol.yz.data(), P.data(), c, n));
      PO_TRY(applyK0(xt->d, wd2->d, tvec, wyw));
    }
    PO_TRY(k_w_step(ctx, wv(), ws, wyw->d, 0, tau, wp(), nw, mins_w));
    PO_TRY(k_panel_axpy(ctx, d1v->d, 0.0, nullptr, 1.0, coef.data(), P.data(), m, n));
    PO_TRY(applyK0(d1v->d, wd2->d, tvec, wtmp2));
  } else {
    if (m > 0) PO_TRY(k_panel_axpy(ctx, d1v->d, 0.0, nullptr, 1.0, coef.data(), P.data(), m, n));
    PO_TRY(applyK0(d1v->d, wd2->d, tvec, wyw));
    PO_TRY(k_w_step(ctx, wv(), ws, wyw->d, 0, tau, wp(), nw, mins_w));
  }
  double mins_x[2] = {1.0, 1.0};
  PO_TRY(k_solve2s(ctx, bounds(), tvec->d, Dinv->d, coef.data(), P.data(), 0, alpha, beta_mu, full ? 1 : 0, tau,
                   n, px->d, pzl->d, pzu->d, mins_x));
  step_mins[0] = std::min(mins_x[0], mins_w[0]);
  step_mins[1] = std::min(mins_x[1], mins_w[1]);
  kkt.backSubstitute(alpha, b, vars, sol, full, out);
  return PO_OK;
}

int InteriorPoint::evalObjBarrierDeriv(const Dense &p, double *pmerit_) {
  const double beta = options.real("rel_bound_barrier");
  double out[6];
  PO_TRY(k_merit0(ctx, bounds(), px->d, 1.0, g->d, n, out));
  double ppos = out[2] * beta, pneg = out[3] * beta;
  if (has_w) {
    const double *cw = nullptr;
    PO_TRY(sparseConAtIterate(&cw));
    PO_TRY(k_fill(ctx, wtmp2->d, nw, 0.0));
    if (prob->addSparseJacobian(1.0, x, px, wtmp2) != 0) return PO_ERR_USER;
    PO_TRY(k_w_merit(ctx, wv(), wp(), 1.0, gsw->d, gtw->d, cw, wtmp2->d, nw, w_merit_last));
    ppos += w_merit_last[2];
    pneg += w_merit_last[3];
  }
  for (int i = 0; i < c; i++) {
    if (p.s[i] > 0.0) ppos += p.s[i] / vars.s[i]; else pneg += p.s[i] / vars.s[i];
    if (p.t[i] > 0.0) ppos += p.t[i] / vars.t[i]; else pneg += p.t[i] / vars.t[i];
  }
  double pmerit = out[4] - barrier_param * (ppos + pneg);
  for (int i = 0; i < c; i++) pmerit += gamma_s[i] * p.s[i] + gamma_t[i] * p.t[i];
  if (has_w) pmerit += w_merit_last[6] + w_merit_last[7];
  *pmerit_ = pmerit;
  return PO_OK;
}

// ... 172 lines not shown
```

### paropt_amd/csrc/kernels.hip

```cpp
#include "core.hpp"

#include <math.h>
#include <stdlib.h>
#include <string.h>

namespace po {

#define PO_PAIR_LOOP(q, n)                                                                 \
  const int64_t _npairs = ((n) + 1) >> 1;                                                  \
  for (int64_t q = (int64_t)blockIdx.x * blockDim.x + threadIdx.x; q < _npairs;            \
       q += (int64_t)gridDim.x * blockDim.x)

typedef double f64x2l __attribute__((ext_vector_type(2)));
__device__ __forceinline__ double2 ld2(const double *__restrict__ p, int64_t q, int64_t n) {
#ifndef PO_LD2_PLAIN
  const f64x2l v = __builtin_nontemporal_load(reinterpret_cast<const f64x2l *>(p + 2 * q));
  return make_double2(v.x, v.y);
#else
  return *reinterpret_cast<const double2 *>(p + 2 * q);
#endif
}
#ifndef PO_ST2_PLAIN
#define PO_ST2_NT 1
#endif
typedef double f64x2s __attribute__((ext_vector_type(2)));
__device__ __forceinline__ void st2(double *__restrict__ p, int64_t q, int64_t n, double2 v) {
  if (2 * q + 1 >= n) v.y = 0.0;
#ifdef PO_ST2_NT
  __builtin_nontemporal_store((f64x2s){v.x, v.y}, reinterpret_cast<f64x2s *>(p + 2 * q));
#else
  *reinterpret_cast<double2 *>(p + 2 * q) = v;
#endif
}

typedef double f64x4 __attribute__((ext_vector_type(4)));
typedef double f64x2 __attribute__((ext_vector_type(2)));

__device__ __forceinline__ f64x2 ld_stream(const double *p) {
  return __builtin_nontemporal_load(reinterpret_cast<const f64x2 *>(p));
}

enum { OP_SUM = 0, OP_MIN = 1, OP_MAX = 2 };

template <int OP>
__device__ __forceinline__ double combine(double a, double b) {
  if (OP == OP_SUM) return a + b;
  if (OP == OP_MIN) return fmin(a, b);
  return fmax(a, b);
}

template <int OP>
__device__ __forceinline__ double wave_reduce(double v) {
#pragma unroll
  for (int o = 32; o > 0; o >>= 1) v = combine<OP>(v, __shfl_xor(v, o, 64));
  return v;
}

template <int N, int OP>
__device__ __forceinline__ void block_reduce_store(double (&a)[N], double *__restrict__ partials,
                                                   int slot0, double *sm) {
  const int lane = threadIdx.x & 63, wave = threadIdx.x >> 6;
#pragma unroll
  for (int j = 0; j < N; j++) {
    double v = wave_reduce<OP>(a[j]);
    if (lane == 0) sm[wave * N + j] = v;
  }
  __syncthreads();
  if (threadIdx.x < N) {
    const int j = threadIdx.x;
    double v = combine<OP>(combine<OP>(sm[j], sm[N + j]), combine<OP>(sm[2 * N + j], sm[3 * N + j]));
    partials[(size_t)(slot0 + j) * gridDim.x + blockIdx.x] = v;
  }
  __syncthreads();
}

__device__ __forceinline__ void red_raise_flag(volatile unsigned long long *flag, unsigned long long seq,
                                               unsigned *ticket) {
  if (!flag) return;
  __threadfence_system();
  __syncthreads();
  if (threadIdx.x == 0) {
    const unsigned t = atomicAdd(ticket, 1u);
    if (t == gridDim.x - 1) {
// ... 623 lines not shown
  __shared__ double sm[4 * NVB];
  double acc[NVB];
  const double *vp[NVB];
#pragma unroll
  for (int j = 0; j < NVB; j++) {
    acc[j] = 0.0;
    vp[j] = V.p[j0 + j];
  }
  PO_PAIR_LOOP(q, n) {
    const f64x2 xv = *reinterpret_cast<const f64x2 *>(x + 2 * q);
#pragma unroll
    for (int j = 0; j < NVB; j++) {
      const f64x2 w = ld_stream(vp[j] + 2 * q);
      acc[j] = fma(xv.x, w.x, fma(xv.y, w.y, acc[j]));
    }
  }
  block_reduce_store<NVB, OP_SUM>(acc, partials, j0, sm);
}

#define PO_MDOT_CASE(NVB)                                                          \
  case NVB:                                                                        \
    PO_LAUNCH(mdot_kernel<NVB>, grid, x, pt, j0, n, c->d_partials);                \
    break;

int k_mdot_launch(Ctx *c, const double *x, const double *const *V, int nv, int64_t n, int *nblocks) {
  count_bytes(c, nv + 1, n);
  if (nv > kMaxPanel) {
    set_error("mdot of %d vectors exceeds kMaxPanel=%d", nv, kMaxPanel);
    return PO_ERR_ARG;
  }
  const int grid = grid_for(c, n, 5);
  PO_TRY(ensure_partials(c, (size_t)grid * (nv + 32)));
  PtrTable pt;
  CoefTable ct;
  fill_tables(nullptr, V, nv, &ct, &pt);
  int j0 = 0;
  while (j0 < nv) {
    const int rem = nv - j0;
    const int w = rem >= 32 ? 32 : (rem >= 24 ? 24 : (rem >= 16 ? 16 : rem));
    switch (w) {
      PO_MDOT_CASE(1) PO_MDOT_CASE(2) PO_MDOT_CASE(3) PO_MDOT_CASE(4) PO_MDOT_CASE(5)
      PO_MDOT_CASE(6) PO_MDOT_CASE(7) PO_MDOT_CASE(8) PO_MDOT_CASE(9) PO_MDOT_CASE(10)
      PO_MDOT_CASE(11) PO_MDOT_CASE(12) PO_MDOT_CASE(13) PO_MDOT_CASE(14) PO_MDOT_CASE(15)
      PO_MDOT_CASE(16) PO_MDOT_CASE(24) PO_MDOT_CASE(32)
    }
    j0 += w;
  }
  *nblocks = grid;
  return PO_OK;
}

int k_mdot(Ctx *c, const double *x, const double *const *V, int nv, int64_t n, double *out) {
  if (nv <= 0) return PO_OK;
  if (nv > kMaxPanel) {
    for (int j0 = 0; j0 < nv; j0 += kMaxPanel)
      PO_TRY(k_mdot(c, x, V + j0, nv - j0 > kMaxPanel ? kMaxPanel : nv - j0, n, out + j0));
    return PO_OK;
  }
  int grid = 0;
  const bool timed = c->time_mdot_nv == nv;
  if (timed && c->mdot_timing_pending) PO_TRY(batch_flush(c));
  if (timed) PO_HIP(hipEventRecord(c->ev_mdot0, c->stream));
  PO_TRY(k_mdot_launch(c, x, V, nv, n, &grid));
  if (timed) PO_HIP(hipEventRecord(c->ev_mdot1, c->stream));
  const bool defer = timed && c->batch_depth > 0;
  PO_TRY(reduce_finish(c, grid, nv, 0, 0, out, timed && !defer));
  if (timed) {
    auto harvest = [c] {
      float ms = 0.0f;
      if (hipEventSynchronize(c->ev_mdot1) == hipSuccess &&
          hipEventElapsedTime(&ms, c->ev_mdot0, c->ev_mdot1) == hipSuccess) {
        c->mdot_ms += ms;
        c->mdot_count++;
      }
      c->mdot_timing_pending = false;
    };
    if (defer) c->mdot_timing_pending = true;
    after_reduce(c, harvest);
  }
  return PO_OK;
}


struct BE {
  bool L, U;
  double xl, xu, zl, zu;
};
__device__ __forceinline__ BE bound_elem(double x, double lb, double ub, double zl, double zu,
                                         double maxb, int use_lower, int use_upper) {
  BE e;
  e.L = use_lower && (lb > -maxb);
  e.U = use_upper && (ub < maxb);
  e.xl = e.L ? (x - lb) : 1.0;
  e.xu = e.U ? (ub - x) : 1.0;
  e.zl = zl;
  e.zu = zu;
  return e;
}
#define PO_MAKE_BOUNDS(b, q, n)                                                          \
  const bool _has2 = (2 * q + 1 < n);                                                    \
  const BE e0 = bound_elem(_x.x, _lb.x, _ub.x, _zl.x, _zu.x, (b).max_bound, (b).use_lower, \
                           (b).use_upper);                                               \
  BE e1 = bound_elem(_x.y, _lb.y, _ub.y, _zl.y, _zu.y, (b).max_bound, (b).use_lower,     \
                     (b).use_upper);                                                     \
  if (!_has2) {                                                                          \
    e1.L = false;                                                                        \
    e1.U = false;                                                                        \
    e1.xl = 1.0;                                                                         \
    e1.xu = 1.0;                                                                         \
  }
__device__ __forceinline__ double2 ld2_bound(const double *__restrict__ p, int uni, double v, int64_t q, int64_t n) {
  return uni ? make_double2(v, v) : ld2(p, q, n);
}
#define PO_LD2_LB(b, q, n) ld2_bound((b).lb, (b).lb_uni, (b).lb_c, q, n)
#define PO_LD2_UB(b, q, n) ld2_bound((b).ub, (b).ub_uni, (b).ub_c, q, n)
#define PO_LOAD_BOUNDS(b, q, n)                                                         \
  const double2 _x = ld2((b).x, q, n), _lb = PO_LD2_LB(b, q, n), _ub = PO_LD2_UB(b, q, n), \
                _zl = ld2((b).zl, q, n), _zu = ld2((b).zu, q, n);                        \
  PO_MAKE_BOUNDS(b, q, n)

__device__ __forceinline__ void res_bound_acc(const BE &e, double beta_mu, double *sums, double *maxs,
                                              int il1, int il2, int imax) {
  if (e.L) {
    sums[0] += e.zl * e.xl;
    sums[1] += 1.0;
    const double r = fabs(-(e.xl * e.zl - beta_mu));
    sums[il1] += r;
    sums[il2] += r * r;
    maxs[imax] = fmax(maxs[imax], r);
  }
  if (e.U) {
    sums[0] += e.zu * e.xu;
    sums[1] += 1.0;
    const double r = fabs(-(e.xu * e.zu - beta_mu));
    sums[il1 + 1] += r;
    sums[il2 + 1] += r * r;
    maxs[imax + 1] = fmax(maxs[imax + 1], r);
  }
}
__device__ __forceinline__ void res_bound_max2(const BE &e, double beta_mu2, double *m2) {
  if (e.L) m2[0] = fmax(m2[0], fabs(-(e.xl * e.zl - beta_mu2)));
  if (e.U) m2[1] = fmax(m2[1], fabs(-(e.xu * e.zu - beta_mu2)));
}
__global__ void __launch_bounds__(kBlock)
    kkt_res_kernel(Bounds b, const double *__restrict__ g, PtrTable A, CoefTable z, int nc,
                   double beta_mu, int64_t n, double *__restrict__ rx, double *__restrict__ yqn,
                   double beta_mu2, GroupCol gcol, double gcoef, double *__restrict__ partials) {
  __shared__ double sm[4 * 8];
  double sums[8] = {0.0, 0.0, 0.0, 0.0, 0.0, 0.0, 0.0, 0.0};
  double maxs[5] = {0.0, 0.0, 0.0, 0.0, 0.0};
  PO_PAIR_LOOP(q, n) {
    PO_LOAD_BOUNDS(b, q, n);
    const double2 gv = ld2(g, q, n);
    double2 yv = make_double2(0.0, 0.0);
    if (yqn) yv = ld2(yqn, q, n);
    double2 r;
    r.x = (b.use_lower ? _zl.x : 0.0);
    r.y = (b.use_lower ? _zl.y : 0.0);
    if (b.use_upper) {
      r.x += -1.0 * _zu.x;
      r.y += -1.0 * _zu.y;
    }
    r.x += -1.0 * gv.x;
    r.y += -1.0 * gv.y;
    GRaw graw;
    if (gcol.w) graw = gcol_request(gcol, q, n);
    double2 ps = panel_sum(A, z, nc, q);
    if (gcol.w) {
      const f64x2 gcv = gcol_value(gcol, graw);
      ps.x += gcoef * gcv.x;
      ps.y += gcoef * gcv.y;
    }
    r.x += ps.x;
    r.y += ps.y;
    if (!_has2) r.y = 0.0;
    st2(rx, q, n, r);
    if (yqn) {
      const double cl = b.use_lower ? 1.0 : 0.0, cu = b.use_upper ? -1.0 : 0.0;
      yv.x = __dadd_rn(yv.x, __fma_rn(-1.0, r.x, __fma_rn(cu, _zu.x, __fma_rn(cl, _zl.x, 0.0))));
      yv.y = __dadd_rn(yv.y, __fma_rn(-1.0, r.y, __fma_rn(cu, _zu.y, __fma_rn(cl, _zl.y, 0.0))));
      st2(yqn, q, n, yv);
    }
    maxs[0] = fmax(maxs[0], fmax(fabs(r.x), fabs(r.y)));
    sums[2] += fabs(r.x) + fabs(r.y);
    sums[5] += r.x * r.x + r.y * r.y;
    res_bound_acc(e0, beta_mu, sums, maxs, 3, 6, 1);
    res_bound_acc(e1, beta_mu, sums, maxs, 3, 6, 1);
    if (beta_mu2 >= 0.0) {
      res_bound_max2(e0, beta_mu2, maxs + 3);
      res_bound_max2(e1, beta_mu2, maxs + 3);
    }
  }
  block_reduce_store<8, OP_SUM>(sums, partials, 0, sm);
  if (beta_mu2 >= 0.0) {
    block_reduce_store<5, OP_MAX>(maxs, partials, 8, sm);
  } else {
    double m3[3] = {maxs[0], maxs[1], maxs[2]};
    block_reduce_store<3, OP_MAX>(m3, partials, 8, sm);
  }
}

int k_kkt_res(Ctx *c, const Bounds &b, const double *g, const double *const *A, const double *z,
              int nc, double beta_mu, int64_t n, double *rx, double *out, double *yqn, double beta_mu2,
              const GroupCol *gcol, double gcoef) {
  PO_TRY(gcol_check(gcol, n, "k_kkt_res"));
  if (nc > kMaxPanel) {
    const double *w = nullptr, one = 1.0;
    PO_TRY(collapse_range(c, 0, z, A, 0, nc, n, &w));
    return k_kkt_res(c, b, g, &w, &one, 1, beta_mu, n, rx, out, yqn, beta_mu2, gcol, gcoef);
  }
  count_bytes(c, 7 + nc + (yqn ? 2 : 0) - uniform_bound_streams(b), n);
  const int grid = grid_for(c, n, kBpcPanel);
  PO_TRY(ensure_partials(c, (size_t)grid * 13));
  PtrTable pt;
  CoefTable ct;
  fill_tables(z, A, nc, &ct, &pt);
  if (gcol) count_bytes(c, 1.0, gcol->nwcon);
  PO_LAUNCH(kkt_res_kernel, grid, b, g, pt, ct, nc, beta_mu, n, rx, yqn, beta_mu2, gcol ? *gcol : GroupCol(), gcoef,
            c->d_partials);
  return reduce_finish(c, grid, 8, 0, beta_mu2 >= 0.0 ? 5 : 3, out);
}

__global__ void __launch_bounds__(kBlock)
    res_norms_kernel(Bounds b, double beta_mu, int64_t n, double *__restrict__ partials) {
  __shared__ double sm[4 * 8];
  double sums[8] = {0.0, 0.0, 0.0, 0.0, 0.0, 0.0, 0.0, 0.0};
  double maxs[3] = {0.0, 0.0, 0.0};
  PO_PAIR_LOOP(q, n) {
    PO_LOAD_BOUNDS(b, q, n);
    res_bound_acc(e0, beta_mu, sums, maxs, 3, 6, 1);
    res_bound_acc(e1, beta_mu, sums, maxs, 3, 6, 1);
  }
  block_reduce_store<8, OP_SUM>(sums, partials, 0, sm);
  block_reduce_store<3, OP_MAX>(maxs, partials, 8, sm);
}

int k_res_norms(Ctx *c, const Bounds &b, double beta_mu, int64_t n, double out[11]) {
  count_bytes(c, 5 - uniform_bound_streams(b), n);
  const int grid = grid_for(c, n);
  PO_TRY(ensure_partials(c, (size_t)grid * 11));
  PO_LAUNCH(res_norms_kernel, grid, b, beta_mu, n, c->d_partials);
  return reduce_finish(c, grid, 8, 0, 3, out);
}

__device__ __forceinline__ double dinv_elem(const BE &e, double diag) {
  double v = diag;
  if (e.L) v += e.zl / e.xl;
  if (e.U) v += e.zu / e.xu;
  return 1.0 / v;
}
__global__ void __launch_bounds__(kBlock)
    dinv_kernel(Bounds b, double diag, const double *__restrict__ hdiag, int64_t n,
                double *__restrict__ dinv) {
  PO_PAIR_LOOP(q, n) {
    PO_LOAD_BOUNDS(b, q, n);
    double2 h = make_double2(0.0, 0.0);
    if (hdiag) h = ld2(hdiag, q, n);
    st2(dinv, q, n, make_double2(dinv_elem(e0, diag + h.x), dinv_elem(e1, diag + h.y)));
  }
}
int k_dinv(Ctx *c, const Bounds &b, double diag, int64_t n, double *dinv, const double *hdiag) {
  count_bytes(c, 6 + (hdiag ? 1 : 0) - uniform_bound_streams(b), n);
  if (n <= 0) return PO_OK;
  PO_LAUNCH(dinv_kernel, grid_for(c, n), b, diag, hdiag, n, dinv);
  return PO_OK;
}

__device__ __forceinline__ double d1_elem(const BE &e, double rx, double beta_mu, double cl = 0.0,
                                          double cu = 0.0) {
  double d1 = rx;
  if (e.L) d1 += (-(e.xl * e.zl - beta_mu) - cl) / e.xl;
  if (e.U) d1 -= (-(e.xu * e.zu - beta_mu) + cu) / e.xu;
  return d1;
}
__global__ void __launch_bounds__(kBlock)
    d1_kernel(Bounds b, const double *__restrict__ rx, const double *__restrict__ dinv,
              double beta_mu, const double *__restrict__ cl, const double *__restrict__ cu, int64_t n,
              double *__restrict__ t) {
  PO_PAIR_LOOP(q, n) {
    PO_LOAD_BOUNDS(b, q, n);
    const double2 r = ld2(rx, q, n);
    const double2 dv = dinv ? ld2(dinv, q, n) : make_double2(1.0, 1.0);
    double2 c0 = make_double2(0.0, 0.0), c1 = c0;
    if (cl) {
      c0 = ld2(cl, q, n);
      c1 = ld2(cu, q, n);
    }
    st2(t, q, n,
        make_double2(dv.x * d1_elem(e0, r.x, beta_mu, c0.x, c1.x),
                     dv.y * d1_elem(e1, r.y, beta_mu, c0.y, c1.y)));
  }
}
int k_d1(Ctx *c, const Bounds &b, const double *rx, const double *dinv, double beta_mu, int64_t n,
         double *t, const double *cl, const double *cu) {
  count_bytes(c, 7 + (dinv ? 1 : 0) + (cl ? 2 : 0) - uniform_bound_streams(b), n);
  if (n <= 0) return PO_OK;
  PO_LAUNCH(d1_kernel, grid_for(c, n), b, rx, dinv, beta_mu, cl, cu, n, t);
  return PO_OK;
}

__global__ void __launch_bounds__(kBlock)
    dinv_d1_kernel(Bounds b, double diag, const double *__restrict__ hdiag, const double *__restrict__ rx,
                   double beta_mu, int64_t n, double *__restrict__ dinv, double *__restrict__ t, int raw) {
  PO_PAIR_LOOP(q, n) {
    PO_LOAD_BOUNDS(b, q, n);
    double2 h = make_double2(0.0, 0.0);
    if (hdiag) h = ld2(hdiag, q, n);
    const double2 r = ld2(rx, q, n);
    const double2 dv = make_double2(dinv_elem(e0, diag + h.x), dinv_elem(e1, diag + h.y));
    st2(dinv, q, n, dv);
    const double w0 = raw ? 1.0 : dv.x, w1 = raw ? 1.0 : dv.y;
    st2(t, q, n, make_double2(w0 * d1_elem(e0, r.x, beta_mu), w1 * d1_elem(e1, r.y, beta_mu)));
  }
}
int k_dinv_d1(Ctx *c, const Bounds &b, double diag, const double *hdiag, const double *rx, double beta_mu,
              int64_t n, double *dinv, double *t, int raw) {
  count_bytes(c, 8 + (hdiag ? 1 : 0) - uniform_bound_streams(b), n);
  if (n <= 0) return PO_OK;
  PO_LAUNCH(dinv_d1_kernel, grid_for(c, n), b, diag, hdiag, rx, beta_mu, n, dinv, t, raw);
  return PO_OK;
}

__global__ void __launch_bounds__(kBlock)
    corrector_kernel(Bounds b, const double *__restrict__ px, const double *__restrict__ pzl,
                     const double *__restrict__ pzu, int64_t n, double *__restrict__ cl,
                     double *__restrict__ cu) {
  PO_PAIR_LOOP(q, n) {
    PO_LOAD_BOUNDS(b, q, n);
    const double2 p = ld2(px, q, n), l = ld2(pzl, q, n), u = ld2(pzu, q, n);
    st2(cl, q, n, make_double2(e0.L ? p.x * l.x : 0.0, e1.L ? p.y * l.y : 0.0));
    st2(cu, q, n, make_double2(e0.U ? p.x * u.x : 0.0, e1.U ? p.y * u.y : 0.0));
  }
}
int k_corrector(Ctx *c, const Bounds &b, const double *px, const double *pzl, const double *pzu,
                int64_t n, double *cl, double *cu) {
  count_bytes(c, 8 - uniform_bound_streams(b), n);
  if (n <= 0) return PO_OK;
  PO_LAUNCH(corrector_kernel, grid_for(c, n), b, px, pzl, pzu, n, cl, cu);
  return PO_OK;
}

template <int NVB>
__global__ void __launch_bounds__(kBlock)
    corr_d1_dots_kernel(Bounds b, const double *__restrict__ px, const double *__restrict__ pzl,
                        const double *__restrict__ pzu, const double *__restrict__ rx,
                        const double *__restrict__ dinv, double beta_mu, PtrTable V, int64_t n,
                        double *__restrict__ t, double *__restrict__ partials) {
  __shared__ double sm[4 * NVB];
  double acc[NVB];
  const double *vp[NVB];
#pragma unroll
  for (int j = 0; j < NVB; j++) {
    acc[j] = 0.0;
    vp[j] = V.p[j];
  }
  PO_PAIR_LOOP(q, n) {
    PO_LOAD_BOUNDS(b, q, n);
// ... 1701 lines not shown
```

### paropt_amd/csrc/wgram.hip

```cpp
#include "core.hpp"

#include <math.h>
#include <stdlib.h>

#include <memory>
#include <vector>

namespace po {

typedef double f64x2 __attribute__((ext_vector_type(2)));

constexpr int kGramTile = 128;
constexpr int kGramLd = kGramTile + 8;

struct PtrTableW {
  double *p[kMaxPanel];
};

__device__ __forceinline__ f64x2 ld_nt(const double *p) {
  return __builtin_nontemporal_load(reinterpret_cast<const f64x2 *>(p));
}

template <int NG>
struct GramPlan {
  int owner[NG];
  int load[4];
  constexpr GramPlan() : owner{}, load{0, 0, 0, 0} {
    for (int J = NG - 1; J >= 0; J--) {
      int best = 0;
      for (int w = 1; w < 4; w++)
        if (load[w] < load[best]) best = w;
      owner[J] = best;
      load[best] += J + 1;
    }
  }
  constexpr int max_load() const {
    int m = load[0];
    for (int w = 1; w < 4; w++)
      if (load[w] > m) m = load[w];
    return m;
  }
};
template <int NG>
struct GramPlanHolder {
  static constexpr GramPlan<NG> plan = GramPlan<NG>();
  static constexpr int NQ = plan.max_load();
};

template <int NG, int LD = kGramLd>
__device__ __forceinline__ void gram_fetch(const double *__restrict__ base, const double *__restrict__ dwl, int s,
                                           double (&a)[NG], double &w) {
  w = dwl[16 * s];
#pragma unroll
  for (int g = 0; g < NG; g++) a[g] = base[(4 * g) * LD + 16 * s];
}

template <int NG, int W>
__device__ __forceinline__ void gram_step(const double (&a)[NG], double w, bool tsel,
                                          double (&acc)[GramPlanHolder<NG>::NQ]) {
  constexpr GramPlan<NG> plan = GramPlanHolder<NG>::plan;
  int q = 0;
#pragma unroll
  for (int J = 0; J < NG; J++) {
    if (plan.owner[J] == W) {
      const double bw = a[J] * ((J == NG - 1 && tsel) ? 1.0 : w);
#pragma unroll
      for (int I = 0; I <= J; I++) {
        acc[q] = __builtin_amdgcn_mfma_f64_4x4x4f64(a[I], bw, acc[q], 0, 0, 0);
        q++;
      }
    }
  }
}

template <int NG, int W, int TR = kGramTile, int LD = kGramLd>
__device__ __forceinline__ void gram_tile(const double *__restrict__ pt, const double *__restrict__ dw, int lane,
                                          int tcol, double (&acc)[GramPlanHolder<NG>::NQ]) {
  const int ci = lane & 3;
  const int rowoff = ((lane >> 2) & 3) + 4 * (lane >> 4);
  const double *base = pt + ci * LD + rowoff;
  const double *dwl = dw + rowoff;
  const bool tsel = (4 * (NG - 1) + ci == tcol);
  double a0[NG], a1[NG], w0, w1;
// ... 178 lines not shown
      case 2: gram_tile<NG, 2>(pt, dw, lane, tcol, acc); break;
      default: gram_tile<NG, 3>(pt, dw, lane, tcol, acc); break;
    }
  }
#undef PO_GRAM_PREFETCH
  switch (wave) {
    case 0: gram_store<NG, 0>(acc, lane, partials); break;
    case 1: gram_store<NG, 1>(acc, lane, partials); break;
    case 2: gram_store<NG, 2>(acc, lane, partials); break;
    default: gram_store<NG, 3>(acc, lane, partials); break;
  }
}

constexpr int kGramDepth = 3;
#ifdef PO_WGRAM_NO_FULL_STAGE
#define PO_WGRAM_FULL_STAGE 0
#else
#define PO_WGRAM_FULL_STAGE 1
#endif

__device__ unsigned long long g_wgram_stamp[8];

struct GramGeom {
  int64_t ngt = 0;
  int64_t rg = 0;
  int64_t nwcon = 0;
  int trows = kGramTile, G = 0, period = 0, nw = 0, ncols = 0;
  double alpha = 0.0;
};
__device__ __forceinline__ void gram_tile_geom(const GramGeom &gg, int64_t tile, int64_t &row0, int &nrows) {
  const bool grp = tile < gg.ngt;
  const int64_t rowg = tile * gg.trows, rowp = gg.rg + (tile - gg.ngt) * kGramTile;
  const int64_t left = gg.rg - rowg;
  const int nrg = left < gg.trows ? (int)left : gg.trows;
  row0 = grp ? rowg : rowp;
  nrows = grp ? nrg : kGramTile;
}
constexpr int kGramGroupNw = 24;
struct GramGroupOps {
  double p[kGramGroupNw], w[kGramGroupNw];
};
__device__ __forceinline__ void gram_groups_request(const double *__restrict__ pt, const double *__restrict__ dw,
                                                    const GramGeom &gg, int u, int gi, GramGroupOps &o) {
  const double *row = pt + u * kGramLd + gi * gg.period;
  const double *wr = dw + gi * gg.period;
#pragma unroll
  for (int k = 0; k < kGramGroupNw; k++) {
    if (k < gg.nw) {
      o.p[k] = row[k];
      o.w[k] = wr[k];
    }
  }
}
__device__ __forceinline__ double gram_groups_sum(const GramGeom &gg, const GramGroupOps &o) {
#pragma clang fp contract(off)
  double sacc = 0.0;
#pragma unroll
  for (int k = 0; k < kGramGroupNw; k++) {
    if (k < gg.nw) {
      const double prod = o.w[k] * o.p[k];
      sacc = sacc + prod;
    }
  }
  return gg.alpha * sacc;
}
__device__ __forceinline__ void gram_groups_rest(const double *__restrict__ pt, const double *__restrict__ dw,
                                                 const GramGeom &gg, double *const *Utab, int64_t g0, int ng, int ctid) {
#pragma clang fp contract(off)
  typedef __attribute__((address_space(1))) double gdouble;
  for (int pair = ctid + 256; pair < ng * gg.ncols; pair += 256) {
    const int u = pair / ng, gi = pair - u * ng;
    const double *row = pt + u * kGramLd + gi * gg.period;
    const double *wr = dw + gi * gg.period;
    double sacc = 0.0;
    for (int k = 0; k < gg.nw; k++) {
      const double prod = wr[k] * row[k];
      sacc = sacc + prod;
    }
    gdouble *up = (gdouble *)Utab[u];
    up[g0 + gi] = gg.alpha * sacc;
  }
}

template <int NG, int ZP>
struct GramProducer {
  f64x2 buf[kGramDepth][NG];
  f64x2 sbuf[kGramDepth][ZP > 0 ? ZP : 1];
  f64x2 dbuf[kGramDepth];
  int64_t row[kGramDepth];
  bool in[kGramDepth];
};

template <int NG, int ZP, int R>
__device__ __forceinline__ void gram_pc_load(GramProducer<NG, ZP> &P, const double *const (&colp)[NG],
                                             const double *const (&scol)[ZP > 0 ? ZP : 1], const double *d,
                                             int64_t tile, int64_t ntiles, int64_t n, int64_t ilast, int lane,
                                             const GramGeom &gg) {
  if (tile >= ntiles) {
    P.in[R] = false;
    return;
  }
  int64_t row0;
  int nrows;
  gram_tile_geom(gg, tile, row0, nrows);
  int64_t i = row0 + 2 * lane;
  const bool in = (2 * lane < nrows) && (i < n);
  int64_t alt = row0 + 2 * (lane & 3);
  alt = alt > ilast ? ilast : alt;
  if (!in) i = gg.ngt > 0 ? alt : ilast;
  P.in[R] = in;
  P.row[R] = i;
#pragma unroll
  for (int it = 0; it < NG; it++) P.buf[R][it] = ld_nt(colp[it] + i);
  if (ZP > 0) {
#pragma unroll
    for (int it = 0; it < ZP; it++) P.sbuf[R][it] = ld_nt(scol[it] + i);
  }
  P.dbuf[R] = *reinterpret_cast<const f64x2 *>(d + i);
}

template <int NG, int ZP, int R, bool FULL = false>
__device__ __forceinline__ void gram_pc_stage(GramProducer<NG, ZP> &P, double *__restrict__ pt,
                                              double *__restrict__ dw, double *const (&zcol)[ZP > 0 ? ZP : 1], int pw,
                                              int nv, int kpend, double b0, int lane) {
  const bool in = FULL ? true : P.in[R];
#pragma unroll
  for (int it = 0; it < NG; it++) {
    const int j = pw + 4 * it;
    f64x2 v = P.buf[R][it];
    if (ZP > 0 && it < ZP && j < kpend) {
      v.x -= b0 * P.sbuf[R][it].x;
      v.y -= b0 * P.sbuf[R][it].y;
      if (in && zcol[it]) __builtin_nontemporal_store(v, reinterpret_cast<f64x2 *>(zcol[it] + P.row[R]));
    }
    if (!FULL && !in) v = (f64x2){0.0, 0.0};
    if (j < nv) *reinterpret_cast<f64x2 *>(pt + j * kGramLd + 2 * lane) = v;
  }
  if (pw == 0) *reinterpret_cast<f64x2 *>(dw + 2 * lane) = in ? P.dbuf[R] : (f64x2){0.0, 0.0};
}

template <int NG, int ZP, int RS, int GS>
__global__ void __launch_bounds__(512, 1)
    wgram_pc_kernel(const double *__restrict__ d, PtrTable V, int nv, int64_t n, int64_t ntiles,
                    double *__restrict__ partials, PtrTable S, PtrTableW Zout, int kpend, double b0, int tcol,
                    int ablate, int prio, GramGeom gg, PtrTableW Ugs) {
  constexpr int M = 4 * NG;
  constexpr int NQ = GramPlanHolder<NG>::NQ;
  const bool want_stamps = (ablate & 16) != 0;
  ablate &= 15;
  if constexpr (GS == 0) gg = GramGeom();
  constexpr int kBufDoubles = M * kGramLd + kGramTile;
  extern __shared__ double lds[];
  const int tid = threadIdx.x, lane = tid & 63;
  const int wave = __builtin_amdgcn_readfirstlane(tid >> 6);
  for (int b2 = 0; b2 < 2; b2++)
    for (int idx = tid; idx < (M - nv) * kGramLd; idx += 512) lds[b2 * kBufDoubles + nv * kGramLd + idx] = 0.0;
  double **utab = reinterpret_cast<double **>(lds + 2 * kBufDoubles);
  if constexpr (GS != 0) {
    if (tid < kMaxPanel) utab[tid] = Ugs.p[tid];
  }
  int64_t first = blockIdx.x, stride = gridDim.x;
  int64_t nt = first < ntiles ? (ntiles - first + stride - 1) / stride : 0;
  if constexpr (GS != 0) {
    const int64_t per = (ntiles + gridDim.x - 1) / gridDim.x;
    first = blockIdx.x * per;
    stride = 1;
    nt = ntiles - first;
    nt = nt < 0 ? 0 : (nt < per ? nt : per);
  }
  __syncthreads();
  if (wave >= 4) {
    if (prio == 1) __builtin_amdgcn_s_setprio(1);
    if (prio == 2) __builtin_amdgcn_s_setprio(2);
    if (prio == 3) __builtin_amdgcn_s_setprio(3);
    const int pw = wave - 4;
    const double *colp[NG];
#pragma unroll
    for (int it = 0; it < NG; it++) {
      const int j = pw + 4 * it;
      colp[it] = V.p[j < nv ? j : nv - 1];
    }
    const double *scol[ZP > 0 ? ZP : 1];
    double *zcol[ZP > 0 ? ZP : 1];
#pragma unroll
    for (int it = 0; it < (ZP > 0 ? ZP : 1); it++) {
      const int j = pw + 4 * it;
      scol[it] = (ZP > 0 && kpend > 0) ? S.p[j < kpend ? j : kpend - 1] : nullptr;
      zcol[it] = (ZP > 0 && j < kpend) ? Zout.p[j] : nullptr;
    }
    const int64_t ilast = ((n - 1) >> 1) << 1;
    GramProducer<NG, ZP> P;
    gram_pc_load<NG, ZP, 0>(P, colp, scol, d, first, ntiles, n, ilast, lane, gg);
    gram_pc_load<NG, ZP, 1>(P, colp, scol, d, first + stride, ntiles, n, ilast, lane, gg);
    gram_pc_load<NG, ZP, 2>(P, colp, scol, d, first + 2 * stride, ntiles, n, ilast, lane, gg);
    unsigned long long st_stage = 0, st_load = 0, st_wait = 0;
    const bool stamp = want_stamps && blockIdx.x == 0 && wave == 4;
    const unsigned long long st_c0 = stamp ? __builtin_amdgcn_s_memtime() : 0;
    const unsigned long long st_r0 = stamp ? __builtin_amdgcn_s_memrealtime() : 0;
#define PO_PC_STEP(R)                                                                                         \
  if (it + (R) < nt) {                                                                                        \
    double *bt = lds + (size_t)((it + (R)) & 1) * kBufDoubles;                                                \
    const unsigned long long _t0 = stamp ? __builtin_amdgcn_s_memtime() : 0;                                  \
    if (ablate == 2) {                                                                                        \
      if (P.buf[R][0].x == 1.2345e301) bt[0] = P.buf[R][NG - 1].y;                                            \
    } else if (PO_WGRAM_FULL_STAGE && __all(P.in[R])) {                                                       \
      gram_pc_stage<NG, ZP, (R), true>(P, bt, bt + M * kGramLd, zcol, pw, nv, kpend, b0, lane);               \
    } else {                                                                                                  \
      gram_pc_stage<NG, ZP, (R), false>(P, bt, bt + M * kGramLd, zcol, pw, nv, kpend, b0, lane);              \
    }                                                                                                         \
    if (stamp) __builtin_amdgcn_s_waitcnt(0);                                                                 \
    const unsigned long long _t1 = stamp ? __builtin_amdgcn_s_memtime() : 0;                                  \
    if (ablate != 3) gram_pc_load<NG, ZP, (R)>(P, colp, scol, d, first + (it + (R) + kGramDepth) * stride, ntiles, n, ilast, lane, gg); \
    const unsigned long long _t2 = stamp ? __builtin_amdgcn_s_memtime() : 0;                                  \
    __syncthreads();                                                                                          \
    if (stamp) {                                                                                              \
      const unsigned long long _t3 = __builtin_amdgcn_s_memtime();                                            \
      st_stage += _t1 - _t0;                                                                                  \
      st_load += _t2 - _t1;                                                                                   \
      st_wait += _t3 - _t2;                                                                                   \
    }                                                                                                         \
  }
    for (int64_t it = 0; it < nt; it += kGramDepth) {
      PO_PC_STEP(0)
      PO_PC_STEP(1)
      PO_PC_STEP(2)
    }
#undef PO_PC_STEP
    if (stamp && lane == 0) {
      g_wgram_stamp[2] = st_stage;
      g_wgram_stamp[3] = st_load;
      g_wgram_stamp[4] = st_wait;
      g_wgram_stamp[5] = (unsigned long long)nt;
      g_wgram_stamp[6] = __builtin_amdgcn_s_memtime() - st_c0;
      g_wgram_stamp[7] = __builtin_amdgcn_s_memrealtime() - st_r0;
    }
    __syncthreads();
    if (RS) __syncthreads();
  } else {
    constexpr int NACC = RS ? NG * (NG + 1) / 2 : NQ;
    double acc[NACC];
#pragma unroll
    for (int q = 0; q < NACC; q++) acc[q] = 0.0;
    unsigned long long sc_wait = 0, sc_work = 0;
    const bool cstamp = want_stamps && blockIdx.x == 0 && wave == 0;
    [[maybe_unused]] int gs_u = 0, gs_gi = 0;
    if constexpr (GS == 1) {
      gs_u = tid / gg.G;
      gs_gi = tid - gs_u * gg.G;
    }
    for (int64_t it = 0; it < nt; it++) {
      const unsigned long long _t0 = cstamp ? __builtin_amdgcn_s_memtime() : 0;
      __syncthreads();
      const unsigned long long _t1 = cstamp ? __builtin_amdgcn_s_memtime() : 0;
      const double *bt = lds + (size_t)(it & 1) * kBufDoubles;
      if (ablate == 1) continue;
      [[maybe_unused]] GramGroupOps gops;
      [[maybe_unused]] bool gs_on = false, gs_mine = false;
      [[maybe_unused]] int gs_ng = 0, pu = 0, pgi = 0;
      [[maybe_unused]] int64_t gs_g0 = 0;
      if constexpr (GS == 1) {
        const int64_t tile = first + it * stride;
        gs_on = tile < gg.ngt;
        if (gs_on) {
          gs_g0 = tile * gg.G;
          gs_ng = (int)((gg.nwcon - gs_g0) < gg.G ? (gg.nwcon - gs_g0) : gg.G);
          pu = gs_u;
          pgi = gs_gi;
          if (gs_ng != gg.G) {
            pu = tid / gs_ng;
            pgi = tid - pu * gs_ng;
          }
          gs_mine = tid < gs_ng * gg.ncols;
          if (!RS && gs_mine && ablate != 5) gram_groups_request(bt, bt + M * kGramLd, gg, pu, pgi, gops);
        }
      }
      if constexpr (RS) {
        if constexpr (GS == 1) {
          auto request = [&]() {
            if (gs_on && gs_mine && ablate != 5) gram_groups_request(bt, bt + M * kGramLd, gg, pu, pgi, gops);
          };
          gram_tile_rows<NG>(bt, bt + M * kGramLd, lane, wave, tcol, acc, request);
        } else {
          gram_tile_rows<NG>(bt, bt + M * kGramLd, lane, wave, tcol, acc);
        }
      } else {
        switch (wave) {
          case 0: gram_tile<NG, 0>(bt, bt + M * kGramLd, lane, tcol, acc); break;
          case 1: gram_tile<NG, 1>(bt, bt + M * kGramLd, lane, tcol, acc); break;
          case 2: gram_tile<NG, 2>(bt, bt + M * kGramLd, lane, tcol, acc); break;
          default: gram_tile<NG, 3>(bt, bt + M * kGramLd, lane, tcol, acc); break;
        }
      }
      if constexpr (GS == 1) {
        if (gs_on) {
          if (gs_mine && ablate != 6) {
// ... 130 lines not shown
    } else {                                                                             \
      _Pragma("unroll") for (int h = 0; h < NH; h++) {                                   \
        f64x2 v = P.buf[R][h];                                                           \
        if (!_in) v = (f64x2){0.0, 0.0};                                                 \
        const int _j = j0 + 8 * h;                                                       \
        if (_j < nv) *reinterpret_cast<f64x2 *>(bt + _j * kG64Ld + 2 * rp) = v;          \
      }                                                                                  \
    }                                                                                    \
    if (pw == 0 && half == 0)                                                            \
      *reinterpret_cast<f64x2 *>(bt + M * kG64Ld + 2 * rp) = _in ? P.dbuf[R] : (f64x2){0.0, 0.0}; \
    if (stamp) __builtin_amdgcn_s_waitcnt(0xc07f);  \
    const unsigned long long _t1 = stamp ? __builtin_amdgcn_s_memtime() : 0;             \
    PO_G64_LOAD(R, first + (it + (R) + D) * stride);                                     \
    const unsigned long long _t2 = stamp ? __builtin_amdgcn_s_memtime() : 0;             \
    __syncthreads();                                                                     \
    if (stamp) {                                                                         \
      const unsigned long long _t3 = __builtin_amdgcn_s_memtime();                       \
      st_stage += _t1 - _t0;                                                             \
      st_load += _t2 - _t1;                                                              \
      st_wait += _t3 - _t2;                                                              \
    }                                                                                    \
  }
    PO_G64_LOAD(0, first);
    PO_G64_LOAD(1, first + stride);
    PO_G64_LOAD(2, first + 2 * stride);
    if constexpr (D == 4) PO_G64_LOAD(3, first + 3 * stride);
    int64_t it = 0;
    for (; it + D <= nt; it += D) {
      PO_G64_STEP(0)
      PO_G64_STEP(1)
      PO_G64_STEP(2)
      if constexpr (D == 4) PO_G64_STEP(3)
    }
    if (it < nt) PO_G64_STEP(0)
    if (it + 1 < nt) PO_G64_STEP(1)
    if constexpr (D == 4) {
      if (it + 2 < nt) PO_G64_STEP(2)
    }
#undef PO_G64_STEP
#undef PO_G64_LOAD
    if (stamp && lane == 0) {
      g_wgram_stamp[2] = st_stage;
      g_wgram_stamp[3] = st_load;
      g_wgram_stamp[4] = st_wait;
      g_wgram_stamp[5] = (unsigned long long)nt;
      g_wgram_stamp[6] = __builtin_amdgcn_s_memtime() - st_c0;
      g_wgram_stamp[7] = __builtin_amdgcn_s_memrealtime() - st_r0;
    }
    __syncthreads();
  } else {
    switch (wave) {
      case 0: gram64_consume<NG, 0>(lds, nt, partials, tcol, lane, want_stamps && blockIdx.x == 0); break;
      case 1: gram64_consume<NG, 1>(lds, nt, partials, tcol, lane, false); break;
      case 2: gram64_consume<NG, 2>(lds, nt, partials, tcol, lane, false); break;
      default: gram64_consume<NG, 3>(lds, nt, partials, tcol, lane, false); break;
    }
  }
}

template <int NG>
static int wgram_pc64_launch_t(Ctx *c, const double *d, const PtrTable &pt, int nv, int64_t n, int tcol, int ablate,
                               int prio, int *grid_out) {
  const size_t lds = (size_t)2 * (4 * NG * kG64Ld + kG64Tile) * sizeof(double);
  static bool attr_set = false;
  if (!attr_set) {
    PO_HIP(hipFuncSetAttribute(reinterpret_cast<const void *>(wgram_pc64_kernel<NG>),
                               hipFuncAttributeMaxDynamicSharedMemorySize, (int)lds));
    attr_set = true;
  }
  const int64_t ntiles = (n + kG64Tile - 1) / kG64Tile;
  int64_t g = (int64_t)c->num_cu;
  if (g > ntiles) g = ntiles;
  if (g < 1) g = 1;
  PO_TRY(ensure_partials(c, (size_t)g * (NG * (NG + 1) / 2) * 16));
  const int stamps = (ablate & 16) != 0;
  hipLaunchKernelGGL((wgram_pc64_kernel<NG>), dim3((int)g), dim3(512), lds, c->stream, d, pt, nv, n, ntiles,
                     c->d_partials, tcol, prio, stamps);
  c->n_launches++;
  PO_HIP(hipGetLastError());
  *grid_out = (int)g;
  return PO_OK;
}

template <int NG, int ZP, int RS, int GS = 0>
static int wgram_pc_launch_t(Ctx *c, const double *d, const PtrTable &pt, int nv, int64_t n, int64_t ntiles,
                             const PtrTable &st, const PtrTableW &zt, int kpend, double b0, int tcol, int ablate,
                             int prio, int *grid_out, const GramGeom *gg = nullptr, const PtrTableW *ut = nullptr) {
  const size_t lds = (size_t)2 * (4 * NG * kGramLd + kGramTile) * sizeof(double) + (GS ? kMaxPanel * sizeof(double *) : 0);
  static bool attr_set = false;
  if (!attr_set) {
    PO_HIP(hipFuncSetAttribute(reinterpret_cast<const void *>(wgram_pc_kernel<NG, ZP, RS, GS>),
                               hipFuncAttributeMaxDynamicSharedMemorySize, (int)lds));
    attr_set = true;
  }
  int64_t g = (int64_t)c->num_cu;
  if (g > ntiles) g = ntiles;
  if (g < 1) g = 1;
  PO_TRY(ensure_partials(c, (size_t)g * (NG * (NG + 1) / 2) * 16));
  static const PtrTableW no_u = PtrTableW();
  hipLaunchKernelGGL((wgram_pc_kernel<NG, ZP, RS, GS>), dim3((int)g), dim3(512), lds, c->stream, d, pt, nv, n, ntiles,
                     c->d_partials, st, zt, kpend, b0, tcol, ablate, prio, gg ? *gg : GramGeom(), ut ? *ut : no_u);
  c->n_launches++;
  PO_HIP(hipGetLastError());
  *grid_out = (int)g;
  return PO_OK;
}

template <int NG, int ZP, int OCC>
static int wgram_launch_t(Ctx *c, const double *d, const PtrTable &pt, int nv, int64_t n, int64_t ntiles,
                          const PtrTable &st, const PtrTableW &zt, int kpend, double b0, int tcol, int ablate,
                          int *grid_out) {
  const size_t lds = (size_t)(4 * NG * kGramLd + kGramTile) * sizeof(double);
  static bool attr_set = false;
  if (!attr_set) {
    PO_HIP(hipFuncSetAttribute(reinterpret_cast<const void *>(wgram_kernel<NG, ZP, OCC>),
                               hipFuncAttributeMaxDynamicSharedMemorySize, (int)lds));
    attr_set = true;
  }
  int per_cu = (int)((160 * 1024) / lds);
  if (per_cu > OCC) per_cu = OCC;
  if (per_cu < 1) per_cu = 1;
  int64_t g = (int64_t)c->num_cu * per_cu;
  if (g > ntiles) g = ntiles;
  if (g < 1) g = 1;
  PO_TRY(ensure_partials(c, (size_t)g * (NG * (NG + 1) / 2) * 16));
  hipLaunchKernelGGL((wgram_kernel<NG, ZP, OCC>), dim3((int)g), dim3(kBlock), lds, c->stream, d, pt, nv, n, ntiles,
                     c->d_partials, st, zt, kpend, b0, tcol, ablate);
  c->n_launches++;
  PO_HIP(hipGetLastError());
  *grid_out = (int)g;
  return PO_OK;
}

static int wgram_groups(int nv) { return (nv + 3) / 4; }

static bool wgram_groups_geom(const GramGroups *g, int nv, int64_t n, int kpend, GramGeom *gg) {
  if (!g || g->nwcon <= 0 || g->ncols <= 0 || g->ncols > nv || !g->U || kpend > 0) return false;
  const int64_t period = (int64_t)g->nw + g->skip;
  if (g->start != 0 || g->nw <= 0 || g->nw > kGramGroupNw || period > kGramTile) return false;
  if ((g->nwcon - 1) * period + g->nw > n) return false;
  int G = (int)(kGramTile / period);
  if (period & 1) G &= ~1;
  if (G < 1) return false;
  int64_t rg = g->nwcon * period;
  if (rg > n) rg = n;
  if ((rg & 1) && rg != n) return false;
  const int NG = (nv + 3) / 4;
  if (NG > 9 || n < 4 * kGramTile) return false;
  gg->ngt = (g->nwcon + G - 1) / G;
  gg->rg = rg;
  gg->nwcon = g->nwcon;
  gg->trows = G * (int)period;
  gg->G = G;
  gg->period = (int)period;
  gg->nw = g->nw;
  gg->ncols = g->ncols;
  gg->alpha = g->alpha;
  return true;
}

int k_wgram_launch(Ctx *c, const double *d, const double *const *V, int nv, int64_t n, int *nblocks,
                   int *nslots, const double *const *S, double *const *Zout, int kpend, double b0,
                   int preweighted_last, const GramGroups *groups, bool *groups_done) {
  if (groups_done) *groups_done = false;
  if (nv > kWgramMaxVecs || nv < 1) {
    set_error("wgram panel width %d outside 1..%d", nv, kWgramMaxVecs);
    return PO_ERR_ARG;
  }
  if (kpend > 12 || kpend > nv || (kpend > 0 && (!S || !Zout))) {
    set_error("wgram: %d pending columns cannot be materialised in the Gram pass", kpend);
    return PO_ERR_ARG;
  }
  count_bytes(c, nv + 1 + 2 * kpend, n);
  const int tcol = preweighted_last ? nv - 1 : -1;
  const int NG = wgram_groups(nv);
  int64_t ntiles = (n + kGramTile - 1) / kGramTile;
  PtrTable pt, st;
  PtrTableW zt, ut;
  for (int j = 0; j < kMaxPanel; j++) {
    pt.p[j] = j < nv ? V[j] : nullptr;
    st.p[j] = (S && j < kpend) ? S[j] : nullptr;
    zt.p[j] = (Zout && j < kpend) ? Zout[j] : nullptr;
    ut.p[j] = nullptr;
  }
  int grid = 0;
  GramGeom gg;
  const int ablate = dbg_switch(SW_WGRAM_ABLATE), prio = dbg_switch(SW_WGRAM_PRIO);
  if (NG >= kGramPcMinNG && wgram_groups_geom(groups, nv, n, kpend, &gg)) {
    ntiles = gg.ngt + (n - gg.rg + kGramTile - 1) / kGramTile;
    for (int j = 0; j < gg.ncols; j++) ut.p[j] = groups->U[j];
    count_bytes(c, (double)gg.ncols, gg.nwcon);
#define PO_WGG(NGv)                                                                                              \
  case NGv:                                                                                                      \
    PO_TRY((wgram_pc_launch_t<NGv, 0, 1, 1>(c, d, pt, nv, n, ntiles, st, zt, 0, 0.0, tcol, ablate, prio, &grid, &gg, \
                                            &ut)));                                                              \
    break;
    switch (NG) {
      PO_WGG(6) PO_WGG(7) PO_WGG(8) PO_WGG(9)
    }
#undef PO_WGG
    if (groups_done) *groups_done = true;
    *nblocks = grid;
    *nslots = (NG * (NG + 1) / 2) * 16;
    return PO_OK;
  }
#define PO_WG(NGv)                                                                                     \
  case NGv: {                                                                                          \
                         \
            \
    constexpr int OCC0 = NGv <= 8 ? 4 : (NGv <= 10 ? 3 : (NGv <= 14 ? 2 : 1));                         \
    constexpr int OCCZ = NGv <= 7 ? 3 : (NGv <= 13 ? 2 : 1);                                           \
            \
    constexpr int NGc = NGv < kGramPcMinNG ? kGramPcMinNG : (NGv <= 16 ? NGv : 16);                    \
    constexpr int NGr = NGc <= kGramRowSplitMaxNG ? NGc : kGramRowSplitMaxNG;                          \
    constexpr int NGo = NGc > kGramRowSplitMaxNG ? NGc : kGramRowSplitMaxNG + 1;                       \
    if (NGv >= 17 && kpend == 0 && n >= 4 * kGramTile) {                                               \
      constexpr int NGw = NGv >= 17 ? NGv : 17;                                                        \
      PO_TRY((wgram_pc64_launch_t<NGw>(c, d, pt, nv, n, tcol, ablate, prio, &grid)));                  \
    } else if (NGv <= 16 && NGv >= kGramPcMinNG && n >= 4 * kGramTile) {                               \
      if (NGv <= kGramRowSplitMaxNG) {                                                                 \
        if (kpend > 0) PO_TRY((wgram_pc_launch_t<NGr, 3, 1>(c, d, pt, nv, n, ntiles, st, zt, kpend, b0, tcol, ablate, prio, &grid))); \
        else PO_TRY((wgram_pc_launch_t<NGr, 0, 1>(c, d, pt, nv, n, ntiles, st, zt, 0, 0.0, tcol, ablate, prio, &grid)));              \
      } else if (kpend > 0 && NGv == 16)  \
        PO_TRY((wgram_launch_t<NGv, 3, 1>(c, d, pt, nv, n, ntiles, st, zt, kpend, b0, tcol, ablate, &grid)));                   \
      else if (kpend > 0) PO_TRY((wgram_pc_launch_t<(NGo < 16 ? NGo : 15), 3, 0>(c, d, pt, nv, n, ntiles, st, zt, kpend, b0, tcol, ablate, prio, &grid))); \
      else PO_TRY((wgram_pc_launch_t<NGo, 0, 0>(c, d, pt, nv, n, ntiles, st, zt, 0, 0.0, tcol, ablate, prio, &grid)));                \
    } else if (kpend > 0) {                                                                            \
      PO_TRY((wgram_launch_t<NGv, 3, OCCZ>(c, d, pt, nv, n, ntiles, st, zt, kpend, b0, tcol, ablate, &grid))); \
    } else {                                                                                           \
      PO_TRY((wgram_launch_t<NGv, 0, OCC0>(c, d, pt, nv, n, ntiles, st, zt, 0, 0.0, tcol, ablate, &grid)));    \
    }                                                                                                  \
  } break;
  switch (NG) {
    PO_WG(1) PO_WG(2) PO_WG(3) PO_WG(4) PO_WG(5) PO_WG(6) PO_WG(7) PO_WG(8) PO_WG(9) PO_WG(10)
    PO_WG(11) PO_WG(12) PO_WG(13) PO_WG(14) PO_WG(15) PO_WG(16) PO_WG(17) PO_WG(18) PO_WG(19) PO_WG(20)
  }
#undef PO_WG
  *nblocks = grid;
  *nslots = (NG * (NG + 1) / 2) * 16;
  return PO_OK;
}

int wgram_debug_stamps(double out[8]) {
  unsigned long long h[8] = {0, 0, 0, 0, 0, 0, 0, 0};
  PO_HIP(hipMemcpyFromSymbol(h, HIP_SYMBOL(g_wgram_stamp), sizeof(h)));
  for (int i = 0; i < 8; i++) out[i] = (double)h[i];
  return PO_OK;
}

static int wgram_one_launch(Ctx *c, const double *d, const double *const *V, int nv, int64_t n, double *W,
                            const double *const *S, double *const *Zout, int kpend, double b0, int preweighted_last,
                            bool may_defer, const GramGroups *groups = nullptr, bool *groups_done = nullptr);

int k_wgram(Ctx *c, const double *d, const double *const *V, int nv, int64_t n, double *W,
            const double *const *S, double *const *Zout, int kpend, double b0, int preweighted_last, bool may_defer,
            const GramGroups *groups, bool *groups_done) {
  if (groups_done) *groups_done = false;
  if (nv <= 0) return PO_OK;
  if (nv <= kWgramMaxVecs)
    return wgram_one_launch(c, d, V, nv, n, W, S, Zout, kpend, b0, preweighted_last, may_defer, groups, groups_done);
  if (kpend > 0 || preweighted_last) {
    set_error("wgram: a panel of %d columns is processed in blocks, which cannot form L-SR1 columns or carry a "
              "pre-weighted column", nv);
    return PO_ERR_ARG;
  }
  const int half = kWgramMaxVecs / 2;
  const int nb = (nv + half - 1) / half;
  int bw = (nv + nb - 1) / nb;
  bw = ((bw + 3) / 4) * 4;
  std::vector<const double *> V2;
  std::vector<double> W2;
  for (int I = 0; I < nb; I++) {
    const int i0 = I * bw, ni = (nv - i0 < bw) ? nv - i0 : bw;
    if (ni <= 0) continue;
    for (int J = I + 1; J < nb; J++) {
      const int j0 = J * bw, nj = (nv - j0 < bw) ? nv - j0 : bw;
      if (nj <= 0) continue;
      const int m2 = ni + nj;
      V2.assign(V + i0, V + i0 + ni);
      V2.insert(V2.end(), V + j0, V + j0 + nj);
      W2.assign((size_t)m2 * m2, 0.0);
      PO_TRY(wgram_one_launch(c, d, V2.data(), m2, n, W2.data(), nullptr, nullptr, 0, 0.0, 0, false));
      auto col = [&](int q) { return q < ni ? i0 + q : j0 + (q - ni); };
      for (int q = 0; q < m2; q++)
        for (int r = 0; r < m2; r++) W[col(r) + (size_t)nv * col(q)] = W2[r + (size_t)m2 * q];
    }
  }
  return PO_OK;
}

static int wgram_one_launch(Ctx *c, const double *d, const double *const *V, int nv, int64_t n, double *W,
                            const double *const *S, double *const *Zout, int kpend, double b0, int preweighted_last,
                            bool may_defer, const GramGroups *groups, bool *groups_done) {
  if (nv <= 0) return PO_OK;
  int grid = 0, nslots = 0;
  const bool defer = may_defer && c->batch_depth > 0;
  const bool timed = c->time_wgram != 0 && !defer;
  if (timed) PO_HIP(hipEventRecord(c->ev0, c->stream));
  PO_TRY(k_wgram_launch(c, d, V, nv, n, &grid, &nslots, S, Zout, kpend, b0, preweighted_last, groups, groups_done));
  if (timed) PO_HIP(hipEventRecord(c->ev1, c->stream));
  auto blocks = std::make_shared<std::vector<double>>(nslots);
  PO_TRY(reduce_finish(c, grid, nslots, 0, 0, blocks->data(), !defer));
  if (timed) {
    float ms = 0.0f;
    PO_HIP(hipEventSynchronize(c->ev1));
    PO_HIP(hipEventElapsedTime(&ms, c->ev0, c->ev1));
    const int w = kpend > 0 ? 1 : 0;
    c->wgram_ms[w] += ms;
    c->wgram_count[w]++;
    c->wgram_cols[w] = nv;
    c->wgram_bytes[w] += 8.0 * (double)n * (nv + 1 + 2 * kpend);
  }
  auto unpack = [blocks, nv, W] {
    const int NG = wgram_groups(nv);
    int p = 0;
    for (int I = 0; I < NG; I++) {
      for (int J = I; J < NG; J++, p++) {
        for (int i = 0; i < 4; i++) {
          for (int j = 0; j < 4; j++) {
            const int r = 4 * I + i, s = 4 * J + j;
            if (r < nv && s < nv && r <= s) {
              const double v = (*blocks)[(size_t)p * 16 + i * 4 + j];
              W[r + (size_t)nv * s] = v;
              W[s + (size_t)nv * r] = v;
            }
          }
        }
      }
    }
  };
  after_reduce(c, unpack);
  return PO_OK;
}

constexpr int kXgramMaxVecs = 48;

template <int NG, int W>
struct XgramOwn {
  static constexpr int NJ = W < NG ? (NG - W + 3) / 4 : 0;
  static constexpr int NQ = NJ * NG > 0 ? NJ * NG : 1;
};

template <int NG, int NJ>
__device__ __forceinline__ void xgram_fetch(const double *__restrict__ ub, const double *__restrict__ zb, int off,
                                            double (&a)[NG], double (&b)[NJ]) {
#pragma unroll
  for (int g = 0; g < NG; g++) a[g] = ub[(4 * g) * kG64Ld + off];
#pragma unroll
  for (int jj = 0; jj < NJ; jj++) b[jj] = zb[(16 * jj) * kG64Ld + off];
}
template <int NG, int NJ>
__device__ __forceinline__ void xgram_step(const double (&a)[NG], const double (&b)[NJ],
                                           double (&acc)[XgramOwn<NG, 0>::NQ]) {
  int q = 0;
#pragma unroll
  for (int jj = 0; jj < NJ; jj++) {
#pragma unroll
    for (int I = 0; I < NG; I++) {
      acc[q] = __builtin_amdgcn_mfma_f64_4x4x4f64(a[I], b[jj], acc[q], 0, 0, 0);
      q++;
    }
  }
}

template <int NG, int W>
__device__ __forceinline__ void xgram_tile(const double *__restrict__ ut, const double *__restrict__ zt, int lane,
                                           double (&acc)[XgramOwn<NG, 0>::NQ]) {
  constexpr int NJ = XgramOwn<NG, W>::NJ;
  if constexpr (NJ > 0) {
    const int ci = lane & 3;
    const int rowoff = ((lane >> 2) & 3) + 4 * (lane >> 4);
    const double *ub = ut + ci * kG64Ld + rowoff;
    const double *zb = zt + (4 * W + ci) * kG64Ld + rowoff;
    int off1 = 16;
    asm volatile("" : "+v"(off1));
    double a[NG], b[NJ];
#pragma unroll 1
    for (int s = 0; s < kG64Tile / 16; s += 2) {
      xgram_fetch<NG, NJ>(ub, zb, 16 * s, a, b);
      xgram_step<NG, NJ>(a, b, acc);
      xgram_fetch<NG, NJ>(ub, zb, 16 * s + off1, a, b);
      xgram_step<NG, NJ>(a, b, acc);
    }
  }
}

template <int NG, int W>
__device__ __forceinline__ void xgram_store(const double (&acc)[XgramOwn<NG, 0>::NQ], int lane,
                                            double *__restrict__ partials) {
  constexpr int NJ = XgramOwn<NG, W>::NJ;
  int q = 0;
#pragma unroll
  for (int jj = 0; jj < NJ; jj++) {
#pragma unroll
// ... 157 lines not shown
```

Baseline: 44.05.

## Form Dinv and t inside the Gram pass instead of a separate kernel

Adds a Gram-kernel variant that computes Dinv and the t vector on the fly from x, bounds, multipliers and rx, instead of running a separate dinv_d1 kernel before the Gram pass. This is meant to save one full read/write sweep over the 50M-element vectors in KKT setup. The materialised Dinv and t are now formed lazily through ensureDinvT at every later consumer, so they are still written when needed. The path only applies with uniform bounds, moderate panel widths and no Hessian diagonal. It adds a new template instantiation and many lazy-materialisation call sites that must all be correct.

```diff
diff --git a/paropt_amd/csrc/bound_elem.hpp b/paropt_amd/csrc/bound_elem.hpp
--- /dev/null
+++ b/paropt_amd/csrc/bound_elem.hpp
@@ -0,0 +1,37 @@
+#pragma once
+#include <hip/hip_runtime.h>
+
+namespace po {
+
+struct BE {
+  bool L, U;
+  double xl, xu, zl, zu;
+};
+__device__ __forceinline__ BE bound_elem(double x, double lb, double ub, double zl, double zu,
+                                         double maxb, int use_lower, int use_upper) {
+  BE e;
+  e.L = use_lower && (lb > -maxb);
+  e.U = use_upper && (ub < maxb);
+  e.xl = e.L ? (x - lb) : 1.0;
+  e.xu = e.U ? (ub - x) : 1.0;
+  e.zl = zl;
+  e.zu = zu;
+  return e;
+}
+
+__device__ __forceinline__ double dinv_elem(const BE &e, double diag) {
+  double v = diag;
+  if (e.L) v += e.zl / e.xl;
+  if (e.U) v += e.zu / e.xu;
+  return 1.0 / v;
+}
+
+__device__ __forceinline__ double d1_elem(const BE &e, double rx, double beta_mu, double cl = 0.0,
+                                          double cu = 0.0) {
+  double d1 = rx;
+  if (e.L) d1 += (-(e.xl * e.zl - beta_mu) - cl) / e.xl;
+  if (e.U) d1 -= (-(e.xu * e.zu - beta_mu) + cu) / e.xu;
+  return d1;
+}
+
+}
diff --git a/paropt_amd/csrc/context.cpp b/paropt_amd/csrc/context.cpp
--- a/paropt_amd/csrc/context.cpp
+++ b/paropt_amd/csrc/context.cpp
@@ -65,6 +65,7 @@
     {SW_SYNC_TRACE, "PAROPT_AMD_SYNC_TRACE", 0, true},
     {SW_USER_TIMING, "PAROPT_AMD_USER_TIMING", 0, true},
     {SW_DUMP_LONG_SOLVES, "PAROPT_AMD_DUMP_LONG_SOLVES", -1, false},
+    {SW_GRAM_DT, "PAROPT_AMD_GRAM_DT", 1, false},
 };
 static struct {
   int value = -1;
diff --git a/paropt_amd/csrc/core.hpp b/paropt_amd/csrc/core.hpp
--- a/paropt_amd/csrc/core.hpp
+++ b/paropt_amd/csrc/core.hpp
@@ -181,7 +181,7 @@
   SW_NO_FUSED_MERIT = 23, SW_NO_LEAN_STEP = 24, SW_NO_RECOMPUTE_DT = 25, SW_NO_FUSED_UPDATE = 26,
   SW_NO_CSR_GROUPS = 27, SW_NO_FRONTS = 28, SW_FORCE_RCCL = 29, SW_RCCL_ALLGATHER = 30, SW_NO_DIRECT_RED = 31,
   SW_NO_FLAG_POLL = 32, SW_NO_BATCH = 33, SW_HOST_TRACE = 34, SW_SYNC_TRACE = 35, SW_USER_TIMING = 36,
-  SW_DUMP_LONG_SOLVES = 37, SW_COUNT = 38
+  SW_DUMP_LONG_SOLVES = 37, SW_GRAM_DT = 38, SW_COUNT = 39
 };
 int dbg_switch(DbgSwitch id);
 void dbg_switch_set(int id, int value);
@@ -273,17 +273,19 @@
   int ncols = 0;
   double *const *U = nullptr;
 };
+struct GramDT;
 int k_wgram(Ctx *c, const double *d, const double *const *V, int nv, int64_t n, double *W,
             const double *const *S = nullptr, double *const *Zout = nullptr, int kpend = 0,
             double b0 = 0.0, int preweighted_last = 0, bool may_defer = false,
-            const GramGroups *groups = nullptr, bool *groups_done = nullptr);
+            const GramGroups *groups = nullptr, bool *groups_done = nullptr, const GramDT *dt = nullptr);
 int wgram_debug_stamps(double out[8]);
 int k_xgram(Ctx *c, const double *const *U, const double *const *Z, int m, int64_t w, double *out,
             bool may_defer = false);
 int k_wgram_launch(Ctx *c, const double *d, const double *const *V, int nv, int64_t n,
                    int *nblocks, int *nslots, const double *const *S = nullptr,
                    double *const *Zout = nullptr, int kpend = 0, double b0 = 0.0,
-                   int preweighted_last = 0, const GramGroups *groups = nullptr, bool *groups_done = nullptr);
+                   int preweighted_last = 0, const GramGroups *groups = nullptr, bool *groups_done = nullptr,
+                   const GramDT *dt = nullptr);
 
 struct Bounds {
   const double *x, *lb, *ub, *zl, *zu;
@@ -293,6 +295,12 @@
   double lb_c = 0.0, ub_c = 0.0;
 };
 inline int uniform_bound_streams(const Bounds &b) { return (b.lb_uni ? 1 : 0) + (b.ub_uni ? 1 : 0); }
+struct GramDT {
+  Bounds b;
+  const double *rx;
+  double diag, beta_mu;
+};
+bool k_wgram_forms_dt(const Bounds &b, int nv, int64_t n, int kpend);
 int k_kkt_res(Ctx *c, const Bounds &b, const double *g, const double *const *A, const double *z,
               int nc, double beta_mu, int64_t n, double *rx, double *out, double *yqn = nullptr,
               double beta_mu2 = -1.0, const GroupCol *gcol = nullptr, double gcoef = 0.0);
diff --git a/paropt_amd/csrc/ip.cpp b/paropt_amd/csrc/ip.cpp
--- a/paropt_amd/csrc/ip.cpp
+++ b/paropt_amd/csrc/ip.cpp
@@ -353,6 +353,7 @@
   if (has_w) return initLeastSquaresMultipliersW();
   if (c == 0) return PO_OK;
   const double small = 1e-4;
+  scratch_flags.dinv_t_unformed = false;
   PO_TRY(k_fill(ctx, Dinv->d, n, 1.0));
   int k = 0;
   std::vector<const double *> A = panel(false, &k);
@@ -434,6 +435,7 @@
   const double beta_mu2 = spec ? options.real("rel_bound_barrier") * mu2 : -1.0;
   iterate_flags.spec_valid = false;
   scratch_flags.spec_dt_valid = false;
+  if (vectors) scratch_flags.dinv_t_unformed = false;
   BatchScope wbatch(ctx, has_w && prob->reductionsBatchable());
   if (has_w) PO_TRY(computeResidualW(mu));
   bool acz_mode = false, acz_rebuilt = false;
@@ -598,7 +600,14 @@
   return PO_OK;
 }
 
-int InteriorPoint::setUpKKTSystem(bool use_qn, bool diag_only, const double *rhs_mu) {
+int InteriorPoint::ensureDinvT() {
+  if (!scratch_flags.dinv_t_unformed) return PO_OK;
+  scratch_flags.dinv_t_unformed = false;
+  return k_dinv_d1(ctx, bounds(), t0_diag, nullptr, rx->d, unformed_bmu, n, Dinv->d, tvec->d);
+}
+
+int InteriorPoint::setUpKKTSystem(bool use_qn, bool diag_only, const double *rhs_mu,
+                                  bool store_dt) {
   if (qn) PO_TRY(refreshQuasiNewton());
   step_flags.ptpx_valid = false;
   scratch_flags.t0_valid = false;
@@ -610,10 +619,33 @@
   const bool raw_d1_w = has_w && rhs_mu && !corrector_active;
   const bool have_spec_dt = scratch_flags.spec_dt_valid;
   scratch_flags.spec_dt_valid = false;
+  scratch_flags.dinv_t_unformed = false;
+  std::vector<const double *> Yp, Sp;
+  std::vector<double *> Zo;
+  double b0z = 0.0;
+  const bool fuse_z = qn && use_qn && !diag_only && !has_w && qn->pendingZ(&Yp, &Sp, &Zo, &b0z) &&
+                      !Yp.empty() && Yp.size() <= 12 && c + (int)Yp.size() + (fuse_t ? 1 : 0) <= kWgramMaxVecs;
+  GramDT gdt;
+  bool gram_dt = false;
+  int kz = 0;
+  if (fuse_t && !use_hdiag && !store_dt && dbg_switch(SW_GRAM_DT) != 0) {
+    kz = fuse_z ? (int)Yp.size() : ((qn && use_qn && !diag_only) ? qn->size() : 0);
+    gdt.b = bounds();
+    gdt.rx = rx->d;
+    gdt.diag = b0 + sigma;
+    gdt.beta_mu = options.real("rel_bound_barrier") * (*rhs_mu);
+    gram_dt = c + kz > 0 && k_wgram_forms_dt(gdt.b, c + kz + 1, n, fuse_z ? kz : 0);
+  }
   if (fuse_t && have_spec_dt && !use_hdiag && spec_dt_diag == b0 + sigma &&
       spec_dt_bmu == options.real("rel_bound_barrier") * (*rhs_mu)) {
     scratch_flags.t_is_plain_dinv_d1 = true;
     t0_diag = b0 + sigma;
+    gram_dt = false;
+  } else if (gram_dt) {
+    scratch_flags.t_is_plain_dinv_d1 = true;
+    scratch_flags.dinv_t_unformed = true;
+    t0_diag = gdt.diag;
+    unformed_bmu = gdt.beta_mu;
   } else if (fuse_t) {
     PO_TRY(k_dinv_d1(ctx, bounds(), b0 + sigma, use_hdiag ? hdiag->d : nullptr, rx->d,
                      options.real("rel_bound_barrier") * (*rhs_mu), n, Dinv->d, tvec->d));
@@ -626,11 +658,6 @@
     PO_TRY(k_dinv(ctx, bounds(), b0 + sigma, n, Dinv->d, use_hdiag ? hdiag->d : nullptr));
   }
   int k = 0;
-  std::vector<const double *> Yp, Sp;
-  std::vector<double *> Zo;
-  double b0z = 0.0;
-  const bool fuse_z = qn && use_qn && !diag_only && !has_w && qn->pendingZ(&Yp, &Sp, &Zo, &b0z) &&
-                      !Yp.empty() && Yp.size() <= 12 && c + (int)Yp.size() + (fuse_t ? 1 : 0) <= kWgramMaxVecs;
   if (fuse_z) {
     k = (int)Yp.size();
     const int m2 = c + k, mt = m2 + (fuse_t ? 1 : 0);
@@ -638,7 +665,8 @@
     for (Vec *a : Ac) P2.push_back(a->d);
     if (fuse_t) P2.push_back(tvec->d);
     std::vector<double> W2((size_t)mt * mt, 0.0);
-    PO_TRY(k_wgram(ctx, Dinv->d, P2.data(), mt, n, W2.data(), Sp.data(), Zo.data(), k, b0z, fuse_t ? 1 : 0));
+    PO_TRY(k_wgram(ctx, Dinv->d, P2.data(), mt, n, W2.data(), Sp.data(), Zo.data(), k, b0z, fuse_t ? 1 : 0, false,
+                   nullptr, nullptr, gram_dt ? &gdt : nullptr));
     qn->pendingZDone();
     kkt.W.assign((size_t)m2 * m2, 0.0);
     auto perm = [&](int i) { return i < c ? k + i : i - c; };
@@ -658,6 +686,10 @@
   }
   const int m = c + k;
   kkt.k = k;
+  if (gram_dt && !fuse_z && m != c + kz) {
+    PO_TRY(ensureDinvT());
+    gram_dt = false;
+  }
   bool fuse_tw = false;
   BatchScope wbatch(ctx, has_w && prob->reductionsBatchable());
   bool t0_ready = fuse_z && fuse_t;
@@ -689,7 +721,7 @@
       const int mt = m + 1;
       Wt_buf.assign((size_t)mt * mt, 0.0);
       PO_TRY(k_wgram(ctx, Dinv->d, Pt.data(), mt, n, Wt_buf.data(), nullptr, nullptr, 0, 0.0, 1, wbatch.open, ggp,
-                     &panel_done));
+                     &panel_done, gram_dt ? &gdt : nullptr));
       t0dots.assign(m, 0.0);
       after_reduce(ctx, [this, m, mt] {
         for (int j = 0; j < m; j++)
@@ -749,6 +781,7 @@
   }
   const bool have_t0 = !refine_pass && scratch_flags.t0_valid && t0_mu == mu && !corr && (int)t0dots.size() == m;
   std::vector<double> dots(m > 0 ? m : 1, 0.0);
+  if (!have_t0 && !refine_pass) PO_TRY(ensureDinvT());
   if (corr_fused) {
     need_panel();
     PO_TRY(k_corr_d1_dots(ctx, bounds(), px->d, pzl->d, pzu->d, rx->d, Dinv->d, beta_mu, P.data(), m, n, tvec->d,
@@ -788,6 +821,7 @@
     const bool defer = forms.recompute_first_step;
     double *tp_out = !defer ? tvec->d : (forms.recompute_rhs ? nullptr : xt->d);
     const bool redo_dt1 = forms.recompute_dt && defer && forms.recompute_rhs && scratch_flags.first_t_recomputable;
+    if (!redo_dt1) PO_TRY(ensureDinvT());
     const double *t_in = redo_dt1 ? nullptr : tvec->d;
     PO_TRY(k_solve2_dots(ctx, bounds(), t_in, Dinv->d, alpha.data(), coef.data(), P.data(), m, beta_mu, tau, rx->d,
                          diag, n, px->d, pzl->d, pzu->d, tp_out, vA->d, c, out.data(), nullptr, defer ? 0 : 1, 0,
@@ -809,6 +843,7 @@
     const bool lean = forms.lean_step && lean_step_allowed && take_merit && iterate_flags.iterate_logs_valid;
     double *pzl_out = lean ? nullptr : pzl->d, *pzu_out = lean ? nullptr : pzu->d;
     const bool redo_dt = forms.recompute_dt && forms.recompute_rhs && scratch_flags.first_t_recomputable;
+    if (!redo_dt) PO_TRY(ensureDinvT());
     const double *t1p = redo_dt ? nullptr : tvec->d;
     if (lean) {
       step_flags.pz_stored = false;
@@ -825,6 +860,7 @@
       });
     }
   } else if (corr_fused) {
+    PO_TRY(ensureDinvT());
     const bool want_logs = !iterate_flags.iterate_logs_valid;
     PO_TRY(k_solve2c(ctx, bounds(), tvec->d, Dinv->d, alpha.data(), P.data(), m, beta_mu, tau, n, px->d, pzl->d,
                      pzu->d, vA->d, c, g->d, want_logs ? 1 : 0, corr_out));
@@ -841,6 +877,7 @@
       step_flags.fused_merit_valid = true;
     });
   } else {
+    PO_TRY(ensureDinvT());
     PO_TRY(k_solve2(ctx, bounds(), tvec->d, Dinv->d, alpha.data(), P.data(), m, beta_mu,
                     refine_pass ? 1 : 0, tau, n, px->d, pzl->d, pzu->d, step_mins,
                     fuse ? coef.data() : nullptr, rx->d, diag, tvec->d, vA->d, c, cl, cu));
@@ -878,6 +915,7 @@
       mres++;
     }
     if (!(it == 0 && step_flags.residual_fused)) {
+      PO_TRY(ensureDinvT());
       if (has_w) {
         if (prob->setSparseJacobianTranspose(1.0, x, wstepv[0], tvec) != 0) return PO_ERR_USER;
         Pq.get().push_back(tvec->d);
@@ -911,6 +949,7 @@
 
 int InteriorPoint::checkKKTStep(int iteration, double mu) {
   const double beta_mu = options.real("rel_bound_barrier") * mu;
+  PO_TRY(ensureDinvT());
   if (!step_flags.pz_stored) {
     PO_TRY(k_form_pz(ctx, bounds(), px->d, step_beta_mu, n, pzl->d, pzu->d));
     step_flags.pz_stored = true;
@@ -964,6 +1003,7 @@
 }
 
 int InteriorPoint::checkGradients(double dh, std::string *report) {
+  PO_TRY(ensureDinvT());
   scratchLent();
   return prob->checkGradients(dh, x, options.integer("use_hvec_product"), xt, tvec, report);
 }
@@ -1094,7 +1134,7 @@
     PO_TRY(computeResidual(mu, true));
     const double comp = compFromSums(comp_prod, comp_count, vars, w_sums[0]);
     const double rhs_mu = 0.0;
-    PO_TRY(setUpKKTSystem(use_qn, false, &rhs_mu));
+    PO_TRY(setUpKKTSystem(use_qn, false, &rhs_mu, true));
     double tau_new = tau;
     PO_TRY(mehrotraStep(use_qn, comp, true, options.real("min_fraction_to_boundary"), options.real("abs_res_tol"),
                         &tau_new));
@@ -2004,7 +2044,7 @@
     if (inexact_newton_step) {
     } else {
     const double rhs_mu = mehrotra ? 0.0 : barrier_param;
-    PO_TRY(setUpKKTSystem(use_qn, diagonal_quasi_newton_step != 0, &rhs_mu));
+    PO_TRY(setUpKKTSystem(use_qn, diagonal_quasi_newton_step != 0, &rhs_mu, mehrotra));
     phaseEnd("setup_kkt");
     if (!mehrotra) {
       lean_step_allowed = qn && use_qnu && use_qn && !diagonal_quasi_newton_step && forms.analytic_panel_dots &&
diff --git a/paropt_amd/csrc/ip.hpp b/paropt_amd/csrc/ip.hpp
--- a/paropt_amd/csrc/ip.hpp
+++ b/paropt_amd/csrc/ip.hpp
@@ -75,7 +75,7 @@
   const std::vector<double> &gramMatrix() const { return kkt.W; }
   const std::vector<int> &cPivots() const { return kkt.cpiv; }
   const double *stepMins() const { return step_mins; }
-  Vec *dinvVec() { return Dinv; }
+  Vec *dinvVec() { return ensureDinvT() == PO_OK ? Dinv : nullptr; }
   Vec *rxVec() { return rx; }
   void flushHistory();
   int checkGradients(double dh, std::string *report);
@@ -143,6 +143,7 @@
     bool t0_valid = false;
     bool t_is_plain_dinv_d1 = false;
     bool first_t_recomputable = false;
+    bool dinv_t_unformed = false;
     bool wd2_ready = false;
     bool panel_valid = false;
   } scratch_flags;
@@ -186,6 +187,8 @@
   std::vector<double> Wt_buf, W2_buf;
   double fused_merit[10] = {0};
   double t0_diag = 0.0;
+  double unformed_bmu = 0.0;
+  int ensureDinvT();
   bool lean_step_allowed = false;
   double step_beta_mu = 0.0;
   double trial_logs[2] = {0, 0}, iterate_logs[2] = {0, 0};
@@ -272,7 +275,7 @@
   void resNorms(const Dense &r, double *max_prime, double *max_dual, double *max_infeas,
                 double *res_norm) const;
   double compFromSums(double prod, double count, const Dense &v, double wprod = 0.0) const;
-  int setUpKKTSystem(bool use_qn, bool diag_only = false, const double *rhs_mu = nullptr);
+  int setUpKKTSystem(bool use_qn, bool diag_only = false, const double *rhs_mu = nullptr, bool store_dt = false);
   int solveKKT(const Dense &b, double mu, bool use_qn, bool refine_pass, double tau, Dense &out,
                bool fuse_residual = false);
   int computeKKTStepWithRefinement(double mu, bool use_qn, double tau);
diff --git a/paropt_amd/csrc/ip_gmres.cpp b/paropt_amd/csrc/ip_gmres.cpp
--- a/paropt_amd/csrc/ip_gmres.cpp
+++ b/paropt_amd/csrc/ip_gmres.cpp
@@ -19,6 +19,7 @@
   std::vector<const double *> P = panel(use_qn, &k);
   PO_TRY(kkt.checkWidth(k));
   const int m = c + k;
+  PO_TRY(ensureDinvT());
   PO_TRY(k_d1s(ctx, bounds(), bx, Dinv->d, alpha, beta_mu, n, tvec->d));
   std::vector<double> dots(m > 0 ? m : 1, 0.0);
   if (m > 0) PO_TRY(k_mdot(ctx, tvec->d, P.data(), m, n, dots.data()));
diff --git a/paropt_amd/csrc/kernels.hip b/paropt_amd/csrc/kernels.hip
--- a/paropt_amd/csrc/kernels.hip
+++ b/paropt_amd/csrc/kernels.hip
@@ -1,4 +1,5 @@
 #include "core.hpp"
+#include "bound_elem.hpp"
 
 #include <math.h>
 #include <stdlib.h>
@@ -788,21 +789,6 @@
 }
 
 
-struct BE {
-  bool L, U;
-  double xl, xu, zl, zu;
-};
-__device__ __forceinline__ BE bound_elem(double x, double lb, double ub, double zl, double zu,
-                                         double maxb, int use_lower, int use_upper) {
-  BE e;
-  e.L = use_lower && (lb > -maxb);
-  e.U = use_upper && (ub < maxb);
-  e.xl = e.L ? (x - lb) : 1.0;
-  e.xu = e.U ? (ub - x) : 1.0;
-  e.zl = zl;
-  e.zu = zu;
-  return e;
-}
 #define PO_MAKE_BOUNDS(b, q, n)                                                          \
   const bool _has2 = (2 * q + 1 < n);                                                    \
   const BE e0 = bound_elem(_x.x, _lb.x, _ub.x, _zl.x, _zu.x, (b).max_bound, (b).use_lower, \
@@ -949,12 +935,6 @@
   return reduce_finish(c, grid, 8, 0, 3, out);
 }
 
-__device__ __forceinline__ double dinv_elem(const BE &e, double diag) {
-  double v = diag;
-  if (e.L) v += e.zl / e.xl;
-  if (e.U) v += e.zu / e.xu;
-  return 1.0 / v;
-}
 __global__ void __launch_bounds__(kBlock)
     dinv_kernel(Bounds b, double diag, const double *__restrict__ hdiag, int64_t n,
                 double *__restrict__ dinv) {
@@ -972,13 +952,6 @@
   return PO_OK;
 }
 
-__device__ __forceinline__ double d1_elem(const BE &e, double rx, double beta_mu, double cl = 0.0,
-                                          double cu = 0.0) {
-  double d1 = rx;
-  if (e.L) d1 += (-(e.xl * e.zl - beta_mu) - cl) / e.xl;
-  if (e.U) d1 -= (-(e.xu * e.zu - beta_mu) + cu) / e.xu;
-  return d1;
-}
 __global__ void __launch_bounds__(kBlock)
     d1_kernel(Bounds b, const double *__restrict__ rx, const double *__restrict__ dinv,
               double beta_mu, const double *__restrict__ cl, const double *__restrict__ cu, int64_t n,
diff --git a/paropt_amd/csrc/wgram.hip b/paropt_amd/csrc/wgram.hip
--- a/paropt_amd/csrc/wgram.hip
+++ b/paropt_amd/csrc/wgram.hip
@@ -1,4 +1,5 @@
 #include "core.hpp"
+#include "bound_elem.hpp"
 
 #include <math.h>
 #include <stdlib.h>
@@ -343,20 +344,26 @@
   }
 }
 
-template <int NG, int ZP>
+constexpr int gram_dt_slots(int DT) { return DT == 0 ? 1 : 2; }
+struct GramDTArgs {
+  Bounds b;
+  double diag = 0.0, beta_mu = 0.0;
+};
+template <int NG, int ZP, int DT = 0>
 struct GramProducer {
   f64x2 buf[kGramDepth][NG];
   f64x2 sbuf[kGramDepth][ZP > 0 ? ZP : 1];
   f64x2 dbuf[kGramDepth];
+  f64x2 ebuf[kGramDepth][gram_dt_slots(DT)];
   int64_t row[kGramDepth];
   bool in[kGramDepth];
 };
 
-template <int NG, int ZP, int R>
-__device__ __forceinline__ void gram_pc_load(GramProducer<NG, ZP> &P, const double *const (&colp)[NG],
+template <int NG, int ZP, int R, int DT = 0>
+__device__ __forceinline__ void gram_pc_load(GramProducer<NG, ZP, DT> &P, const double *const (&colp)[NG],
                                              const double *const (&scol)[ZP > 0 ? ZP : 1], const double *d,
                                              int64_t tile, int64_t ntiles, int64_t n, int64_t ilast, int lane,
-                                             const GramGeom &gg) {
+                                             const GramGeom &gg, const GramDTArgs &dt, bool owner) {
   if (tile >= ntiles) {
     P.in[R] = false;
     return;
@@ -377,18 +384,40 @@
 #pragma unroll
     for (int it = 0; it < ZP; it++) P.sbuf[R][it] = ld_nt(scol[it] + i);
   }
-  P.dbuf[R] = *reinterpret_cast<const f64x2 *>(d + i);
-}
-
-template <int NG, int ZP, int R, bool FULL = false>
-__device__ __forceinline__ void gram_pc_stage(GramProducer<NG, ZP> &P, double *__restrict__ pt,
+  if constexpr (DT == 0) {
+    P.dbuf[R] = *reinterpret_cast<const f64x2 *>(d + i);
+  } else if (owner) {
+    P.dbuf[R] = ld_nt(d + i);
+    P.ebuf[R][0] = ld_nt(dt.b.zl + i);
+    P.ebuf[R][1] = ld_nt(dt.b.zu + i);
+  }
+}
+
+template <int NG, int ZP, int R, bool FULL = false, int DT = 0>
+__device__ __forceinline__ void gram_pc_stage(GramProducer<NG, ZP, DT> &P, double *__restrict__ pt,
                                               double *__restrict__ dw, double *const (&zcol)[ZP > 0 ? ZP : 1], int pw,
-                                              int nv, int kpend, double b0, int lane) {
+                                              int nv, int kpend, double b0, int lane, int64_t n,
+                                              const GramDTArgs &dt, bool owner) {
   const bool in = FULL ? true : P.in[R];
+  [[maybe_unused]] f64x2 dvv = (f64x2){0.0, 0.0};
 #pragma unroll
   for (int it = 0; it < NG; it++) {
     const int j = pw + 4 * it;
     f64x2 v = P.buf[R][it];
+    if constexpr (DT != 0) {
+      if (it == NG - 1 && owner) {
+        const f64x2 xx = P.dbuf[R], zlv = P.ebuf[R][0], zuv = P.ebuf[R][1];
+        const double lbc = dt.b.lb_c, ubc = dt.b.ub_c;
+        const BE e0 = bound_elem(xx.x, lbc, ubc, zlv.x, zuv.x, dt.b.max_bound, dt.b.use_lower, dt.b.use_upper);
+        const BE e1 = bound_elem(xx.y, lbc, ubc, zlv.y, zuv.y, dt.b.max_bound, dt.b.use_lower, dt.b.use_upper);
+        dvv = (f64x2){dinv_elem(e0, dt.diag), dinv_elem(e1, dt.diag)};
+        v = (f64x2){dvv.x * d1_elem(e0, v.x, dt.beta_mu), dvv.y * d1_elem(e1, v.y, dt.beta_mu)};
+        if (P.row[R] + 1 >= n) {
+          dvv.y = 0.0;
+          v.y = 0.0;
+        }
+      }
+    }
     if (ZP > 0 && it < ZP && j < kpend) {
       v.x -= b0 * P.sbuf[R][it].x;
       v.y -= b0 * P.sbuf[R][it].y;
@@ -397,14 +426,19 @@
     if (!FULL && !in) v = (f64x2){0.0, 0.0};
     if (j < nv) *reinterpret_cast<f64x2 *>(pt + j * kGramLd + 2 * lane) = v;
   }
-  if (pw == 0) *reinterpret_cast<f64x2 *>(dw + 2 * lane) = in ? P.dbuf[R] : (f64x2){0.0, 0.0};
-}
-
-template <int NG, int ZP, int RS, int GS>
+  if constexpr (DT == 0) {
+    if (pw == 0) *reinterpret_cast<f64x2 *>(dw + 2 * lane) = in ? P.dbuf[R] : (f64x2){0.0, 0.0};
+  } else if (owner) {
+    *reinterpret_cast<f64x2 *>(dw + 2 * lane) = in ? dvv : (f64x2){0.0, 0.0};
+  }
+}
+
+template <int NG, int ZP, int RS, int GS, int DT = 0>
 __global__ void __launch_bounds__(512, 1)
     wgram_pc_kernel(const double *__restrict__ d, PtrTable V, int nv, int64_t n, int64_t ntiles,
                     double *__restrict__ partials, PtrTable S, PtrTableW Zout, int kpend, double b0, int tcol,
-                    int ablate, int prio, GramGeom gg, PtrTableW Ugs) {
+                    int ablate, int prio, GramGeom gg, PtrTableW Ugs, GramDTArgs dt) {
+  static_assert(DT == 0 || GS == 0, "Dinv / t are formed in the plain tiling only");
   constexpr int M = 4 * NG;
   constexpr int NQ = GramPlanHolder<NG>::NQ;
   const bool want_stamps = (ablate & 16) != 0;
@@ -450,12 +484,13 @@
       zcol[it] = (ZP > 0 && j < kpend) ? Zout.p[j] : nullptr;
     }
     const int64_t ilast = ((n - 1) >> 1) << 1;
-    GramProducer<NG, ZP> P;
-    gram_pc_load<NG, ZP, 0>(P, colp, scol, d, first, ntiles, n, ilast, lane, gg);
-    gram_pc_load<NG, ZP, 1>(P, colp, scol, d, first + stride, ntiles, n, ilast, lane, gg);
-    gram_pc_load<NG, ZP, 2>(P, colp, scol, d, first + 2 * stride, ntiles, n, ilast, lane, gg);
+    const bool owner = DT != 0 && pw == (tcol & 3);
+    GramProducer<NG, ZP, DT> P;
+    gram_pc_load<NG, ZP, 0, DT>(P, colp, scol, d, first, ntiles, n, ilast, lane, gg, dt, owner);
+    gram_pc_load<NG, ZP, 1, DT>(P, colp, scol, d, first + stride, ntiles, n, ilast, lane, gg, dt, owner);
+    gram_pc_load<NG, ZP, 2, DT>(P, colp, scol, d, first + 2 * stride, ntiles, n, ilast, lane, gg, dt, owner);
     unsigned long long st_stage = 0, st_load = 0, st_wait = 0;
-    const bool stamp = want_stamps && blockIdx.x == 0 && wave == 4;
+    const bool stamp = want_stamps && blockIdx.x == 0 && (DT != 0 ? owner : wave == 4);
     const unsigned long long st_c0 = stamp ? __builtin_amdgcn_s_memtime() : 0;
     const unsigned long long st_r0 = stamp ? __builtin_amdgcn_s_memrealtime() : 0;
 #define PO_PC_STEP(R)                                                                                         \
@@ -465,13 +500,13 @@
     if (ablate == 2) {                                                                                        \
       if (P.buf[R][0].x == 1.2345e301) bt[0] = P.buf[R][NG - 1].y;                                            \
     } else if (PO_WGRAM_FULL_STAGE && __all(P.in[R])) {                                                       \
-      gram_pc_stage<NG, ZP, (R), true>(P, bt, bt + M * kGramLd, zcol, pw, nv, kpend, b0, lane);               \
+      gram_pc_stage<NG, ZP, (R), true, DT>(P, bt, bt + M * kGramLd, zcol, pw, nv, kpend, b0, lane, n, dt, owner);  \
     } else {                                                                                                  \
-      gram_pc_stage<NG, ZP, (R), false>(P, bt, bt + M * kGramLd, zcol, pw, nv, kpend, b0, lane);              \
+      gram_pc_stage<NG, ZP, (R), false, DT>(P, bt, bt + M * kGramLd, zcol, pw, nv, kpend, b0, lane, n, dt, owner); \
     }                                                                                                         \
     if (stamp) __builtin_amdgcn_s_waitcnt(0);                                                                 \
     const unsigned long long _t1 = stamp ? __builtin_amdgcn_s_memtime() : 0;                                  \
-    if (ablate != 3) gram_pc_load<NG, ZP, (R)>(P, colp, scol, d, first + (it + (R) + kGramDepth) * stride, ntiles, n, ilast, lane, gg); \
+    if (ablate != 3) gram_pc_load<NG, ZP, (R), DT>(P, colp, scol, d, first + (it + (R) + kGramDepth) * stride, ntiles, n, ilast, lane, gg, dt, owner); \
     const unsigned long long _t2 = stamp ? __builtin_amdgcn_s_memtime() : 0;                                  \
     __syncthreads();                                                                                          \
     if (stamp) {                                                                                              \
@@ -768,14 +803,15 @@
   return PO_OK;
 }
 
-template <int NG, int ZP, int RS, int GS = 0>
+template <int NG, int ZP, int RS, int GS = 0, int DT = 0>
 static int wgram_pc_launch_t(Ctx *c, const double *d, const PtrTable &pt, int nv, int64_t n, int64_t ntiles,
                              const PtrTable &st, const PtrTableW &zt, int kpend, double b0, int tcol, int ablate,
-                             int prio, int *grid_out, const GramGeom *gg = nullptr, const PtrTableW *ut = nullptr) {
+                             int prio, int *grid_out, const GramGeom *gg = nullptr, const PtrTableW *ut = nullptr,
+                             const GramDT *dt = nullptr) {
   const size_t lds = (size_t)2 * (4 * NG * kGramLd + kGramTile) * sizeof(double) + (GS ? kMaxPanel * sizeof(double *) : 0);
   static bool attr_set = false;
   if (!attr_set) {
-    PO_HIP(hipFuncSetAttribute(reinterpret_cast<const void *>(wgram_pc_kernel<NG, ZP, RS, GS>),
+    PO_HIP(hipFuncSetAttribute(reinterpret_cast<const void *>(wgram_pc_kernel<NG, ZP, RS, GS, DT>),
                                hipFuncAttributeMaxDynamicSharedMemorySize, (int)lds));
     attr_set = true;
   }
@@ -784,8 +820,15 @@
   if (g < 1) g = 1;
   PO_TRY(ensure_partials(c, (size_t)g * (NG * (NG + 1) / 2) * 16));
   static const PtrTableW no_u = PtrTableW();
-  hipLaunchKernelGGL((wgram_pc_kernel<NG, ZP, RS, GS>), dim3((int)g), dim3(512), lds, c->stream, d, pt, nv, n, ntiles,
-                     c->d_partials, st, zt, kpend, b0, tcol, ablate, prio, gg ? *gg : GramGeom(), ut ? *ut : no_u);
+  GramDTArgs da;
+  if (dt) {
+    da.b = dt->b;
+    da.diag = dt->diag;
+    da.beta_mu = dt->beta_mu;
+  }
+  hipLaunchKernelGGL((wgram_pc_kernel<NG, ZP, RS, GS, DT>), dim3((int)g), dim3(512), lds, c->stream, d, pt, nv, n,
+                     ntiles, c->d_partials, st, zt, kpend, b0, tcol, ablate, prio, gg ? *gg : GramGeom(),
+                     ut ? *ut : no_u, da);
   c->n_launches++;
   PO_HIP(hipGetLastError());
   *grid_out = (int)g;
@@ -819,6 +862,8 @@
 }
 
 static int wgram_groups(int nv) { return (nv + 3) / 4; }
+constexpr int kGramDtMaxNG = 12;
+static_assert(kGramDtMaxNG <= kGramRowSplitMaxNG, "Dinv / t are formed in the row-split form only");
 
 static bool wgram_groups_geom(const GramGroups *g, int nv, int64_t n, int kpend, GramGeom *gg) {
   if (!g || g->nwcon <= 0 || g->ncols <= 0 || g->ncols > nv || !g->U || kpend > 0) return false;
@@ -845,10 +890,20 @@
   return true;
 }
 
+bool k_wgram_forms_dt(const Bounds &b, int nv, int64_t n, int kpend) {
+  const int NG = wgram_groups(nv);
+  if (uniform_bound_streams(b) != 2) return false;
+  return nv >= 2 && NG >= kGramPcMinNG && NG <= kGramDtMaxNG && n >= 4 * kGramTile && kpend <= 12;
+}
+
 int k_wgram_launch(Ctx *c, const double *d, const double *const *V, int nv, int64_t n, int *nblocks,
                    int *nslots, const double *const *S, double *const *Zout, int kpend, double b0,
-                   int preweighted_last, const GramGroups *groups, bool *groups_done) {
+                   int preweighted_last, const GramGroups *groups, bool *groups_done, const GramDT *dt) {
   if (groups_done) *groups_done = false;
+  if (dt && (!preweighted_last || groups || !k_wgram_forms_dt(dt->b, nv, n, kpend))) {
+    set_error("wgram: no form of the pass forms Dinv and t for this panel (%d columns, n = %lld)", nv, (long long)n);
+    return PO_ERR_ARG;
+  }
   if (nv > kWgramMaxVecs || nv < 1) {
     set_error("wgram panel width %d outside 1..%d", nv, kWgramMaxVecs);
     return PO_ERR_ARG;
@@ -857,7 +912,8 @@
     set_error("wgram: %d pending columns cannot be materialised in the Gram pass", kpend);
     return PO_ERR_ARG;
   }
-  count_bytes(c, nv + 1 + 2 * kpend, n);
+  count_bytes(c, nv + 1 + 2 * kpend + (dt ? 2 : 0), n);
+  if (dt) d = dt->b.x;
   const int tcol = preweighted_last ? nv - 1 : -1;
   const int NG = wgram_groups(nv);
   int64_t ntiles = (n + kGramTile - 1) / kGramTile;
@@ -865,6 +921,7 @@
   PtrTableW zt, ut;
   for (int j = 0; j < kMaxPanel; j++) {
     pt.p[j] = j < nv ? V[j] : nullptr;
+    if (dt && j == nv - 1) pt.p[j] = dt->rx;
     st.p[j] = (S && j < kpend) ? S[j] : nullptr;
     zt.p[j] = (Zout && j < kpend) ? Zout[j] : nullptr;
     ut.p[j] = nullptr;
@@ -900,11 +957,15 @@
     constexpr int NGc = NGv < kGramPcMinNG ? kGramPcMinNG : (NGv <= 16 ? NGv : 16);                    \
     constexpr int NGr = NGc <= kGramRowSplitMaxNG ? NGc : kGramRowSplitMaxNG;                          \
     constexpr int NGo = NGc > kGramRowSplitMaxNG ? NGc : kGramRowSplitMaxNG + 1;                       \
+    constexpr int NGd = NGc <= kGramDtMaxNG ? NGc : kGramDtMaxNG;                                      \
     if (NGv >= 17 && kpend == 0 && n >= 4 * kGramTile) {                                               \
       constexpr int NGw = NGv >= 17 ? NGv : 17;                                                        \
       PO_TRY((wgram_pc64_launch_t<NGw>(c, d, pt, nv, n, tcol, ablate, prio, &grid)));                  \
     } else if (NGv <= 16 && NGv >= kGramPcMinNG && n >= 4 * kGramTile) {                               \
-      if (NGv <= kGramRowSplitMaxNG) {                                                                 \
+      if (NGv <= kGramDtMaxNG && dt) {                                                                 \
+        if (kpend > 0) PO_TRY((wgram_pc_launch_t<NGd, 3, 1, 0, 1>(c, d, pt, nv, n, ntiles, st, zt, kpend, b0, tcol, ablate, prio, &grid, nullptr, nullptr, dt))); \
+        else PO_TRY((wgram_pc_launch_t<NGd, 0, 1, 0, 1>(c, d, pt, nv, n, ntiles, st, zt, 0, 0.0, tcol, ablate, prio, &grid, nullptr, nullptr, dt)));              \
+      } else if (NGv <= kGramRowSplitMaxNG) {                                                          \
         if (kpend > 0) PO_TRY((wgram_pc_launch_t<NGr, 3, 1>(c, d, pt, nv, n, ntiles, st, zt, kpend, b0, tcol, ablate, prio, &grid))); \
         else PO_TRY((wgram_pc_launch_t<NGr, 0, 1>(c, d, pt, nv, n, ntiles, st, zt, 0, 0.0, tcol, ablate, prio, &grid)));              \
       } else if (kpend > 0 && NGv == 16)  \
@@ -936,15 +997,17 @@
 
 static int wgram_one_launch(Ctx *c, const double *d, const double *const *V, int nv, int64_t n, double *W,
                             const double *const *S, double *const *Zout, int kpend, double b0, int preweighted_last,
-                            bool may_defer, const GramGroups *groups = nullptr, bool *groups_done = nullptr);
+                            bool may_defer, const GramGroups *groups = nullptr, bool *groups_done = nullptr,
+                            const GramDT *dt = nullptr);
 
 int k_wgram(Ctx *c, const double *d, const double *const *V, int nv, int64_t n, double *W,
             const double *const *S, double *const *Zout, int kpend, double b0, int preweighted_last, bool may_defer,
-            const GramGroups *groups, bool *groups_done) {
+            const GramGroups *groups, bool *groups_done, const GramDT *dt) {
   if (groups_done) *groups_done = false;
   if (nv <= 0) return PO_OK;
   if (nv <= kWgramMaxVecs)
-    return wgram_one_launch(c, d, V, nv, n, W, S, Zout, kpend, b0, preweighted_last, may_defer, groups, groups_done);
+    return wgram_one_launch(c, d, V, nv, n, W, S, Zout, kpend, b0, preweighted_last, may_defer, groups, groups_done,
+                            dt);
   if (kpend > 0 || preweighted_last) {
     set_error("wgram: a panel of %d columns is processed in blocks, which cannot form L-SR1 columns or carry a "
               "pre-weighted column", nv);
@@ -977,13 +1040,14 @@
 
 static int wgram_one_launch(Ctx *c, const double *d, const double *const *V, int nv, int64_t n, double *W,
                             const double *const *S, double *const *Zout, int kpend, double b0, int preweighted_last,
-                            bool may_defer, const GramGroups *groups, bool *groups_done) {
+                            bool may_defer, const GramGroups *groups, bool *groups_done, const GramDT *dt) {
   if (nv <= 0) return PO_OK;
   int grid = 0, nslots = 0;
   const bool defer = may_defer && c->batch_depth > 0;
   const bool timed = c->time_wgram != 0 && !defer;
   if (timed) PO_HIP(hipEventRecord(c->ev0, c->stream));
-  PO_TRY(k_wgram_launch(c, d, V, nv, n, &grid, &nslots, S, Zout, kpend, b0, preweighted_last, groups, groups_done));
+  PO_TRY(k_wgram_launch(c, d, V, nv, n, &grid, &nslots, S, Zout, kpend, b0, preweighted_last, groups, groups_done,
+                        dt));
   if (timed) PO_HIP(hipEventRecord(c->ev1, c->stream));
   auto blocks = std::make_shared<std::vector<double>>(nslots);
   PO_TRY(reduce_finish(c, grid, nslots, 0, 0, blocks->data(), !defer));
@@ -995,7 +1059,7 @@
     c->wgram_ms[w] += ms;
     c->wgram_count[w]++;
     c->wgram_cols[w] = nv;
-    c->wgram_bytes[w] += 8.0 * (double)n * (nv + 1 + 2 * kpend);
+    c->wgram_bytes[w] += 8.0 * (double)n * (nv + 1 + 2 * kpend + (dt ? 2 : 0));
   }
   auto unpack = [blocks, nv, W] {
     const int NG = wgram_groups(nv);
```

New measurement: 44.55, median of 6. +1.1%, better.
